# fedemagnani/optimization-solvers

Measured on AMD Instinct MI355X. Metric: BFGS iterations/sec on n-dim convex quadratic (f64) at 1/2/4/8 MI355X, higher is better.
Workload: dtype f64

## Files before the change

### include/qn_hip.h

```cpp
#ifndef QN_HIP_H
#define QN_HIP_H

#include <stddef.h>
#include <stdint.h>

#ifdef __cplusplus
extern "C" {
#endif

#define QN_ABI_VERSION 5

typedef enum {
    QN_OK = 0,
    QN_MAX_ITER_REACHED = 1,
    QN_OUT_OF_DOMAIN = 2,
    QN_ERROR_INPUT_PARAMS = 3,
    QN_ABNORMAL_TERMINATION = 4
} qn_status;

const char* qn_status_string(int status);
const char* qn_last_error_message(void);
int qn_abi_version(void);

typedef struct qn_context qn_context;
// ... 96 lines not shown

int qn_solver_create(qn_context* ctx, int method, double tol, const double* x0_host, size_t n, qn_solver** out);
void qn_solver_destroy(qn_solver* s);
int qn_solver_set_bounds(qn_solver* s, const double* lower_bound_host, const double* upper_bound_host);
int qn_solver_set_spg_lambdas(qn_solver* s, double lambda_min, double lambda_max);
int qn_solver_spg_lambda(qn_solver* s, double* out, int* is_some);
int qn_solver_newton_factorisations(qn_solver* s, size_t* out);
int qn_solver_set_lbfgs_memory(qn_solver* s, size_t m);
int qn_solver_lbfgs_state(qn_solver* s, size_t* m, size_t* stored, double* gamma, size_t* resets);
int qn_solver_set_inverse_p(qn_solver* s, const double* p_colmajor_host);
int qn_solver_get_inverse_p(qn_solver* s, double* out_colmajor_host);
int qn_solver_reset(qn_solver* s, const double* x0_host);

typedef void (*qn_callback_fn)(void* user, qn_solver* solver);

int qn_minimize(qn_solver* s, qn_linesearch* ls, const qn_oracle* oracle, size_t max_iter_solver,
                size_t max_iter_line_search, qn_callback_fn callback, void* callback_user);

int qn_compute_step_len(qn_context* ctx, qn_linesearch* ls, const double* x_k_host, double f_k, const double* g_k_host,
                        const double* direction_host, size_t n, const qn_oracle* oracle, size_t max_iter, double* step_out);

size_t qn_solver_n(const qn_solver* s);
size_t qn_solver_k(const qn_solver* s);
int qn_solver_set_k(qn_solver* s, size_t k);
double qn_solver_tol(const qn_solver* s);
int qn_solver_get_x(qn_solver* s, double* out_host);
int qn_solver_set_x(qn_solver* s, const double* x_host);
int qn_solver_s_norm(qn_solver* s, double* out, int* is_some);
int qn_solver_y_norm(qn_solver* s, double* out, int* is_some);
int qn_solver_next_iterate_too_close(qn_solver* s, int* out);
int qn_solver_gradient_next_iterate_too_close(qn_solver* s, int* out);
int qn_solver_decrement_squared(qn_solver* s, double* out, int* is_some);
int qn_solver_get_inv_hessian(qn_solver* s, double* out_colmajor_host, int all_ranks);
int qn_solver_set_inv_hessian(qn_solver* s, const double* h_colmajor_host);
int qn_solver_compute_direction(qn_solver* s, const double* g_host, double* d_host);
int qn_solver_secant_update(qn_solver* s, const double* s_host, const double* y_host);

#define QN_TRACE_LS_MODIFIED (1 << 30)
typedef struct {
    double f, gnorm, t, s_norm, y_norm;
    int32_t n_evals;
    int32_t ls_iters;
    int32_t ls_cases;
    int32_t updated;
} qn_trace_rec;
int qn_solver_set_trace(qn_solver* s, size_t cap, int with_x);
int qn_solver_get_trace(qn_solver* s, qn_trace_rec* out_host, size_t cap, size_t* len, double* x_trace_host);

typedef struct {
    uint64_t iterations;
    uint64_t oracle_calls;
    uint64_t oracle_evals;
    uint64_t h_passes;
    uint64_t h_bytes;
    uint64_t obj_bytes;
    uint64_t launches;
    uint64_t host_syncs;
    double   t_hpass_ms, t_eval_ms, t_ctl_ms, t_comm_ms;
    uint64_t n_hpass_timed, n_eval_timed, n_ctl_timed, n_comm_timed;
    uint64_t matrix_bytes_per_pass;
    uint64_t total_minimize_calls, total_iterations, total_oracle_calls, total_oracle_evals, total_h_passes, total_h_bytes,
        total_obj_bytes;
    uint32_t path;
    uint32_t _pad;
    double   t_hreduce_ms, t_ereduce_ms;
    uint64_t n_hreduce_timed, n_ereduce_timed;
    uint64_t total_xchg_vector, total_xchg_scalar;
    double   t_newton_ms;
    uint64_t n_newton_timed;
    uint64_t newton_lu_sync_timeouts;
} qn_stats;
#define QN_PATH_FUSED 1u
#define QN_PATH_SYM 2u
#define QN_PATH_SYM_GENERIC 4u
#define QN_PATH_PIPELINED 8u
#define QN_PATH_SYM2 16u
#define QN_PATH_TILES1 32u
#define QN_PATH_VECTOR 64u
#define QN_PATH_PNEWTON 128u
#define QN_PATH_RANK1 256u
#define QN_PATH_PNORM 512u
#define QN_PATH_LBFGS 1024u
int qn_solver_get_stats(qn_solver* s, qn_stats* out);
int qn_solver_set_profiling(qn_solver* s, int on);
int qn_solver_set_sync_mode(qn_solver* s, int sync);
int qn_solver_set_tiling(qn_solver* s, int rows_per_block, int col_splits);
typedef enum {
    QN_OPT_GENERIC_KERNELS = 1,
    QN_OPT_DEFERRED_UPDATE_STEP = 2,
    QN_OPT_SYMMETRIC_STORAGE = 3,
    QN_OPT_SECOND_GENERATION = 4,
    QN_OPT_FOLDED_ACCEPT_REDUCE = 5,
    QN_OPT_ROW_SLIVERS = 6,
    QN_OPT_EVAL_PAIR_INSTANCE = 7,
    QN_OPT_EVAL_MOVER_MULTIPLIER = 8,
    QN_OPT_TAIL_REDUCE = 9,
    QN_OPT_BOUNDED_SECOND_GENERATION = 10,
    QN_OPT_NEWTON_PIVOTED_LU = 11,
    QN_OPT_LU_PER_COLUMN_PANEL = 12,
    QN_OPT_LU_LOOKAHEAD = 13,
    QN_OPT_LU_ONE_LAUNCH_PANEL = 14,
    QN_OPT_LU_FORCE_WAIT_EXPIRY = 15,
    QN_OPT_CHUNKS_PER_TRIP = 16,
    QN_OPT_LU_SPLIT_ROLE_A = 17,
    QN_OPT_LU_SPLIT_MIN_ROWS = 18,
    QN_OPT_BTB_PROJECT_IN_EVAL = 19,
    QN_OPT_EVAL_ZIGZAG = 20,
    QN_OPT_TOUCH_H_ROWS = 21,
    QN_OPT_TOUCH_Q_ROWS = 22,
    QN_OPT_PNEWTON_REUSE_FACTOR = 23,
    QN_OPT_PNORM_NONTEMPORAL = 24,
    QN_OPT_PNORM_ROWS_PER_WAVE = 25,
    QN_OPT_LBFGS_UNIT_SCALING = 26
} qn_option;
int qn_solver_set_option(qn_solver* s, int option, int value);

int qn_dev_alloc(qn_context* ctx, size_t bytes, void** out_dev);
int qn_dev_free(qn_context* ctx, void* dev);
int qn_h2d(qn_context* ctx, void* dst_dev, const void* src_host, size_t bytes);
int qn_d2h(qn_context* ctx, void* dst_host, const void* src_dev, size_t bytes);
int qn_gemv(qn_context* ctx, const double* a_dev, size_t ld, size_t nrows, size_t ncols, const double* x_dev, double* y_dev);
int qn_rank2_update(qn_context* ctx, double* h_dev, size_t ld, size_t row0, size_t nrows, size_t n, const double* s_dev,
                    const double* u_dev, double c_ss, double c_su, double c_uu);
int qn_axpy(qn_context* ctx, size_t n, const double* x_dev, double t, const double* d_dev, double* out_dev);
int qn_dot(qn_context* ctx, size_t n, const double* a_dev, const double* b_dev, double* out_host);
int qn_nrm2(qn_context* ctx, size_t n, const double* a_dev, double* out_host);

#ifdef __cplusplus
}
#endif
#endif
```

### include/qn_solver.hpp

```cpp
#pragma once
#include <cmath>
#include <functional>
#include <optional>
#include <stdexcept>
#include <string>
#include <type_traits>
#include <utility>
#include <vector>

#include "qn_hip.h"

namespace optimization_solvers {

using Floating = double;
using DVector = std::vector<Floating>;

struct SolverError : std::runtime_error {
    enum Kind { MaxIterReached = QN_MAX_ITER_REACHED, OutOfDomain = QN_OUT_OF_DOMAIN, ErrorInputParams = QN_ERROR_INPUT_PARAMS,
                AbnormalTermination = QN_ABNORMAL_TERMINATION };
    Kind kind;
    explicit SolverError(int code, const std::string& detail = "")
        : std::runtime_error(std::string(qn_status_string(code)) + (detail.empty() ? "" : ": " + detail)), kind(static_cast<Kind>(code)) {}
};

// ... 142 lines not shown
    qn_linesearch s_;
    DVector lb_, ub_;
  public:
    BackTrackingB(Floating c1, Floating beta, DVector lower_bound, DVector upper_bound) : lb_(std::move(lower_bound)), ub_(std::move(upper_bound)) {
        qn_backtracking_b_new(&s_, c1, beta, lb_.data(), ub_.data());
    }
    BackTrackingB(const BackTrackingB&) = delete;
    qn_linesearch& ffi() { return s_; }
};

class Quadratic {
    qn_objective* h_ = nullptr;
    size_t n_;
  public:
    Quadratic(const DVector& q_rowmajor, const DVector& b, Context& ctx = Context::default_context()) : n_(b.size()) {
        check(qn_quadratic_create(ctx.handle(), n_, q_rowmajor.data(), b.data(), &h_));
    }
    Quadratic(const Quadratic&) = delete;
    ~Quadratic() { qn_objective_destroy(h_); }
    qn_objective* handle() const { return h_; }
    FuncEvalMultivariate operator()(const DVector& x) const {
        DVector g(n_);
        Floating f = 0;
        check(qn_objective_eval(h_, x.data(), &f, g.data()));
        return FuncEvalMultivariate(f, std::move(g));
    }
    DVector hessian(const DVector& x) const {
        DVector h(n_ * n_);
        check(qn_objective_hessian(h_, x.data(), h.data()));
        return h;
    }
};

class LogSumExp {
    qn_objective* h_ = nullptr;
    size_t n_;
  public:
    LogSumExp(const DVector& a_rowmajor, const DVector& c, size_t n, Floating mu, Context& ctx = Context::default_context()) : n_(n) {
        check(qn_logsumexp_create(ctx.handle(), c.size(), n, a_rowmajor.data(), c.data(), mu, &h_));
    }
    LogSumExp(const LogSumExp&) = delete;
    ~LogSumExp() { qn_objective_destroy(h_); }
    qn_objective* handle() const { return h_; }
    FuncEvalMultivariate operator()(const DVector& x) const {
        DVector g(n_);
        Floating f = 0;
        check(qn_objective_eval(h_, x.data(), &f, g.data()));
        return FuncEvalMultivariate(f, std::move(g));
    }
    DVector hessian(const DVector& x) const {
        DVector h(n_ * n_);
        check(qn_objective_hessian(h_, x.data(), h.data()));
        return h;
    }
};

template <int METHOD>
class LineSearchSolver {
    qn_solver* h_ = nullptr;
    size_t n_;
    mutable DVector x_cache_;
    mutable size_t k_cache_ = 0;
    mutable std::optional<Floating> opt_cache_[2];
  public:
    using Self = LineSearchSolver<METHOD>;
    LineSearchSolver(Floating tol, const DVector& x0, Context& ctx = Context::default_context()) : n_(x0.size()) {
        check(qn_solver_create(ctx.handle(), METHOD, tol, x0.data(), x0.size(), &h_));
    }
    qn_solver* handle() const { return h_; }
    static Self new_(Floating tol, const DVector& x0) { return Self(tol, x0); }
    LineSearchSolver(const Self&) = delete;
    LineSearchSolver(Self&& o) noexcept : h_(o.h_), n_(o.n_) { o.h_ = nullptr; }
    ~LineSearchSolver() { if (h_) qn_solver_destroy(h_); }

    const DVector& x() const { x_cache_.resize(n_); check(qn_solver_get_x(h_, x_cache_.data())); return x_cache_; }
    const DVector& xk() const { return x(); }
    const size_t& k() const { k_cache_ = qn_solver_k(h_); return k_cache_; }
    Floating tol() const { return qn_solver_tol(h_); }
    std::optional<Floating> s_norm() const { Floating v; int some; check(qn_solver_s_norm(h_, &v, &some)); return some ? std::optional<Floating>(v) : std::nullopt; }
    std::optional<Floating> y_norm() const { Floating v; int some; check(qn_solver_y_norm(h_, &v, &some)); return some ? std::optional<Floating>(v) : std::nullopt; }
    bool next_iterate_too_close() const { int v; check(qn_solver_next_iterate_too_close(h_, &v)); return v != 0; }
    bool gradient_next_iterate_too_close() const { int v; check(qn_solver_gradient_next_iterate_too_close(h_, &v)); return v != 0; }
    DVector approx_inv_hessian() const { DVector m(n_ * n_); check(qn_solver_get_inv_hessian(h_, m.data(), 1)); return m; }
    std::optional<Floating> decrement_squared() const { Floating v; int some; check(qn_solver_decrement_squared(h_, &v, &some)); return some ? std::optional<Floating>(v) : std::nullopt; }
    bool has_converged(const FuncEvalMultivariate& eval) const {
        if (METHOD == QN_NEWTON) {
            const std::optional<Floating> d = decrement_squared();
            return d ? *d * 0.5 < tol() : false;
        }
        if (METHOD == QN_GRADIENT_DESCENT || METHOD == QN_COORDINATE_DESCENT || METHOD == QN_PNORM_DESCENT) {
            Floating acc = -INFINITY;
            for (Floating v : eval.g()) acc = std::fmax(std::fabs(v), acc);
            return acc < tol();
        }
        if (next_iterate_too_close() || gradient_next_iterate_too_close()) return true;
        Floating s = 0;
        for (Floating v : eval.g()) s += v * v;
        return std::sqrt(s) < tol();
    }

    template <class LS, class Oracle, class = std::enable_if_t<!std::is_same_v<std::decay_t<Oracle>, Quadratic> && !std::is_same_v<std::decay_t<Oracle>, LogSumExp>>>
    Result minimize(LS& line_search, Oracle&& oracle, size_t max_iter_solver, size_t max_iter_line_search,
                    std::optional<std::function<void(const Self&)>> callback = std::nullopt) {
        using OracleT = std::remove_reference_t<Oracle>;
        struct Ctx { OracleT* o; size_t n; } octx{&oracle, n_};
        auto tramp = [](void* user, const double* x, size_t n, double* f, double* g) -> int {
            Ctx* c = static_cast<Ctx*>(user);
            DVector xv(x, x + n);
            FuncEvalMultivariate ev = (*c->o)(xv);
            *f = ev.f();
            for (size_t i = 0; i < n; ++i) g[i] = ev.g()[i];
            return 0;
        };
        struct Cb { Self* me; std::function<void(const Self&)>* f; } cb{this, callback ? &*callback : nullptr};
        auto cb_tramp = [](void* user, qn_solver*) { Cb* c = static_cast<Cb*>(user); (*c->f)(*c->me); };
        auto htramp = [](void* user, const double* x, size_t n, double* h) -> int {
            Ctx* c = static_cast<Ctx*>(user);
            DVector xv(x, x + n);
            FuncEvalMultivariate ev = (*c->o)(xv);
            if (!ev.hessian() || ev.hessian()->size() != n * n) return 1;
            for (size_t i = 0; i < n * n; ++i) h[i] = (*ev.hessian())[i];
            return 0;
        };
        qn_oracle o{};
        o.kind = QN_ORACLE_HOST;
        o.memoize = 0;
        o.host_fn = tramp;
        o.host_user = &octx;
        if (METHOD == QN_NEWTON || METHOD == QN_PROJECTED_NEWTON || METHOD == QN_SPECTRAL_PROJECTED_NEWTON) o.host_hessian_fn = htramp;
        const int st = qn_minimize(h_, &line_search.ffi(), &o, max_iter_solver, max_iter_line_search,
                                   callback ? static_cast<qn_callback_fn>(cb_tramp) : nullptr, &cb);
        return make_result(st);
    }

    template <class LS>
    Result minimize(LS& line_search, const Quadratic& objective, size_t max_iter_solver, size_t max_iter_line_search) {
        qn_oracle o{};
        o.kind = QN_ORACLE_OBJECTIVE;
        o.memoize = 1;
        o.objective = objective.handle();
        return make_result(qn_minimize(h_, &line_search.ffi(), &o, max_iter_solver, max_iter_line_search, nullptr, nullptr));
    }
    template <class LS>
    Result minimize(LS& line_search, const LogSumExp& objective, size_t max_iter_solver, size_t max_iter_line_search) {
        qn_oracle o{};
        o.kind = QN_ORACLE_OBJECTIVE;
        o.memoize = 1;
        o.objective = objective.handle();
        return make_result(qn_minimize(h_, &line_search.ffi(), &o, max_iter_solver, max_iter_line_search, nullptr, nullptr));
    }
};

using BFGS = LineSearchSolver<QN_BFGS>;
using DFP = LineSearchSolver<QN_DFP>;
using GradientDescent = LineSearchSolver<QN_GRADIENT_DESCENT>;
using Broyden = LineSearchSolver<QN_BROYDEN>;
using Newton = LineSearchSolver<QN_NEWTON>;

using CoordinateDescent = LineSearchSolver<QN_COORDINATE_DESCENT>;

class PnormDescent : public LineSearchSolver<QN_PNORM_DESCENT> {
  public:
    PnormDescent(Floating grad_tol, const DVector& x0, const DVector& inverse_p_colmajor, Context& ctx = Context::default_context())
        : LineSearchSolver<QN_PNORM_DESCENT>(grad_tol, x0, ctx) {
        if (inverse_p_colmajor.size() != x0.size() * x0.size()) throw SolverError(QN_ERROR_INPUT_PARAMS);
        check(qn_solver_set_inverse_p(this->handle(), inverse_p_colmajor.data()));
// ... 133 lines not shown
```

### optimization-solvers_amd/_abi.py

```python
import ctypes as C
import os

_HERE = os.path.dirname(os.path.abspath(__file__))
LIB_PATH = os.environ.get("QN_HIP_LIB") or os.path.join(_HERE, "lib", "libqn_hip.so")

OK, MAX_ITER_REACHED, OUT_OF_DOMAIN, ERROR_INPUT_PARAMS, ABNORMAL_TERMINATION = range(5)
LS_MORETHUENTE, LS_BACKTRACKING, LS_MORETHUENTE_B, LS_BACKTRACKING_B, LS_GLL_QUADRATIC = 0, 1, 2, 3, 4
LS_NO_SEARCH = 5
LS_STRONG_WOLFE = 6
ORACLE_HOST, ORACLE_DEVICE_FN, ORACLE_OBJECTIVE = 0, 1, 2
BFGS, DFP, GRADIENT_DESCENT, NEWTON, SR1, SPG, PROJECTED_GRADIENT, PROJECTED_NEWTON, SPECTRAL_PROJECTED_NEWTON = 0, 1, 2, 3, 4, 5, 6, 7, 8
BROYDEN = 9
COORDINATE_DESCENT, PNORM_DESCENT = 10, 11
LBFGS = 12
LBFGS_MAX_M = 32
UNIQUE_ID_BYTES = 128

dp = C.POINTER(C.c_double)


class LineSearchStruct(C.Structure):
    _fields_ = [("kind", C.c_int32), ("_pad", C.c_int32),
                ("c1", C.c_double), ("c2", C.c_double), ("t_min", C.c_double), ("t_max", C.c_double),
                ("delta_min", C.c_double), ("delta", C.c_double), ("delta_max", C.c_double),
# ... 38 lines not shown
PATH_FUSED, PATH_SYM, PATH_SYM_GENERIC, PATH_PIPELINED, PATH_SYM2, PATH_TILES1, PATH_VECTOR, PATH_PNEWTON = 1, 2, 4, 8, 16, 32, 64, 128
PATH_RANK1 = 256
PATH_PNORM = 512
PATH_LBFGS = 1024


SYMBOLS = [
    ("qn_status_string", C.c_char_p, [C.c_int]),
    ("qn_last_error_message", C.c_char_p, []),
    ("qn_abi_version", C.c_int, []),
    ("qn_device_count", C.c_int, [C.POINTER(C.c_int)]),
    ("qn_context_create", C.c_int, [C.c_int, C.POINTER(C.c_void_p)]),
    ("qn_comm_unique_id", C.c_int, [C.c_void_p]),
    ("qn_context_create_sharded", C.c_int, [C.c_int, C.c_int, C.c_int, C.c_void_p, C.POINTER(C.c_void_p)]),
    ("qn_context_create_sharded_host_exchange", C.c_int, [C.c_int, C.c_int, C.c_int, C.c_void_p, C.c_void_p, C.POINTER(C.c_void_p)]),
    ("qn_context_destroy", None, [C.c_void_p]),
    ("qn_partition", C.c_int, [C.c_size_t, C.c_int, C.POINTER(C.c_size_t), C.POINTER(C.c_size_t)]),
    ("qn_comm_selftest", C.c_int, [C.c_void_p]),
    ("qn_context_comm_check", C.c_int, [C.c_void_p]),
    ("qn_context_exchange_probe", C.c_int, [C.c_void_p, C.c_size_t, C.c_int, C.POINTER(C.c_double)]),
    ("qn_context_event_bracket_overhead", C.c_int, [C.c_void_p, C.c_int, C.POINTER(C.c_double)]),
    ("qn_context_synchronize", C.c_int, [C.c_void_p]),
    ("qn_context_rank", C.c_int, [C.c_void_p]),
    ("qn_context_world", C.c_int, [C.c_void_p]),
    ("qn_context_stream", C.c_void_p, [C.c_void_p]),
    ("qn_context_set_host_exchange_async", C.c_int, [C.c_void_p, C.c_int]),
    ("qn_context_set_trial_vector_exchange", C.c_int, [C.c_void_p, C.c_int]),
    ("qn_context_set_allreduce", C.c_int, [C.c_void_p, C.c_int]),
    ("qn_morethuente_default", None, [C.POINTER(LineSearchStruct)]),
    ("qn_morethuente_with_deltas", C.c_int, [C.POINTER(LineSearchStruct), C.c_double, C.c_double, C.c_double]),
    ("qn_morethuente_with_t_min", C.c_int, [C.POINTER(LineSearchStruct), C.c_double]),
    ("qn_morethuente_with_t_max", C.c_int, [C.POINTER(LineSearchStruct), C.c_double]),
    ("qn_morethuente_with_c1", C.c_int, [C.POINTER(LineSearchStruct), C.c_double]),
    ("qn_morethuente_with_c2", C.c_int, [C.POINTER(LineSearchStruct), C.c_double]),
    ("qn_backtracking_new", None, [C.POINTER(LineSearchStruct), C.c_double, C.c_double]),
    ("qn_morethuente_b_new", None, [C.POINTER(LineSearchStruct)]),
    ("qn_backtracking_b_new", None, [C.POINTER(LineSearchStruct), C.c_double, C.c_double, C.c_void_p, C.c_void_p]),
    ("qn_linesearch_with_lower_bound", None, [C.POINTER(LineSearchStruct), C.c_void_p]),
    ("qn_linesearch_with_upper_bound", None, [C.POINTER(LineSearchStruct), C.c_void_p]),
    ("qn_nosearch_new", None, [C.POINTER(LineSearchStruct)]),
    ("qn_gll_quadratic_new", None, [C.POINTER(LineSearchStruct), C.c_double, C.c_size_t]),
    ("qn_gll_quadratic_with_sigmas", None, [C.POINTER(LineSearchStruct), C.c_double, C.c_double]),
    ("qn_strong_wolfe_new", None, [C.POINTER(LineSearchStruct), C.c_double, C.c_double]),
    ("qn_strong_wolfe_with_xtol", C.c_int, [C.POINTER(LineSearchStruct), C.c_double]),
    ("qn_quadratic_create", C.c_int, [C.c_void_p, C.c_size_t, dp, dp, C.POINTER(C.c_void_p)]),
    ("qn_quadratic_create_synthetic", C.c_int, [C.c_void_p, C.c_size_t, C.c_uint64, dp, dp, C.POINTER(C.c_void_p)]),
    ("qn_logsumexp_create", C.c_int, [C.c_void_p, C.c_size_t, C.c_size_t, dp, dp, C.c_double, C.POINTER(C.c_void_p)]),
    ("qn_objective_destroy", None, [C.c_void_p]),
    ("qn_objective_eval", C.c_int, [C.c_void_p, dp, dp, dp]),
    ("qn_objective_get_rows", C.c_int, [C.c_void_p, C.c_size_t, C.c_size_t, dp]),
    ("qn_objective_hessian", C.c_int, [C.c_void_p, dp, dp]),
    ("qn_solver_create", C.c_int, [C.c_void_p, C.c_int, C.c_double, dp, C.c_size_t, C.POINTER(C.c_void_p)]),
    ("qn_solver_destroy", None, [C.c_void_p]),
    ("qn_solver_reset", C.c_int, [C.c_void_p, dp]),
    ("qn_solver_set_bounds", C.c_int, [C.c_void_p, dp, dp]),
    ("qn_solver_set_inverse_p", C.c_int, [C.c_void_p, dp]),
    ("qn_solver_get_inverse_p", C.c_int, [C.c_void_p, dp]),
    ("qn_solver_set_spg_lambdas", C.c_int, [C.c_void_p, C.c_double, C.c_double]),
    ("qn_solver_spg_lambda", C.c_int, [C.c_void_p, dp, C.POINTER(C.c_int)]),
    ("qn_solver_newton_factorisations", C.c_int, [C.c_void_p, C.POINTER(C.c_size_t)]),
    ("qn_solver_set_lbfgs_memory", C.c_int, [C.c_void_p, C.c_size_t]),
    ("qn_solver_lbfgs_state", C.c_int, [C.c_void_p, C.POINTER(C.c_size_t), C.POINTER(C.c_size_t), dp, C.POINTER(C.c_size_t)]),
    ("qn_minimize", C.c_int, [C.c_void_p, C.POINTER(LineSearchStruct), C.POINTER(OracleStruct), C.c_size_t, C.c_size_t, C.c_void_p, C.c_void_p]),
    ("qn_compute_step_len", C.c_int, [C.c_void_p, C.POINTER(LineSearchStruct), dp, C.c_double, dp, dp, C.c_size_t, C.POINTER(OracleStruct), C.c_size_t,
                             C.POINTER(C.c_double)]),
    ("qn_solver_n", C.c_size_t, [C.c_void_p]),
    ("qn_solver_k", C.c_size_t, [C.c_void_p]),
    ("qn_solver_set_k", C.c_int, [C.c_void_p, C.c_size_t]),
    ("qn_solver_tol", C.c_double, [C.c_void_p]),
    ("qn_solver_get_x", C.c_int, [C.c_void_p, dp]),
    ("qn_solver_set_x", C.c_int, [C.c_void_p, dp]),
    ("qn_solver_s_norm", C.c_int, [C.c_void_p, dp, C.POINTER(C.c_int)]),
    ("qn_solver_y_norm", C.c_int, [C.c_void_p, dp, C.POINTER(C.c_int)]),
    ("qn_solver_next_iterate_too_close", C.c_int, [C.c_void_p, C.POINTER(C.c_int)]),
    ("qn_solver_gradient_next_iterate_too_close", C.c_int, [C.c_void_p, C.POINTER(C.c_int)]),
    ("qn_solver_decrement_squared", C.c_int, [C.c_void_p, dp, C.POINTER(C.c_int)]),
    ("qn_solver_get_inv_hessian", C.c_int, [C.c_void_p, dp, C.c_int]),
    ("qn_solver_set_inv_hessian", C.c_int, [C.c_void_p, dp]),
    ("qn_solver_compute_direction", C.c_int, [C.c_void_p, dp, dp]),
    ("qn_solver_secant_update", C.c_int, [C.c_void_p, dp, dp]),
    ("qn_solver_set_trace", C.c_int, [C.c_void_p, C.c_size_t, C.c_int]),
    ("qn_solver_get_trace", C.c_int, [C.c_void_p, C.POINTER(TraceRec), C.c_size_t, C.POINTER(C.c_size_t), dp]),
    ("qn_solver_get_stats", C.c_int, [C.c_void_p, C.POINTER(Stats)]),
    ("qn_solver_set_profiling", C.c_int, [C.c_void_p, C.c_int]),
    ("qn_solver_set_sync_mode", C.c_int, [C.c_void_p, C.c_int]),
    ("qn_solver_set_tiling", C.c_int, [C.c_void_p, C.c_int, C.c_int]),
    ("qn_solver_set_option", C.c_int, [C.c_void_p, C.c_int, C.c_int]),
    ("qn_dev_alloc", C.c_int, [C.c_void_p, C.c_size_t, C.POINTER(C.c_void_p)]),
    ("qn_dev_free", C.c_int, [C.c_void_p, C.c_void_p]),
    ("qn_h2d", C.c_int, [C.c_void_p, C.c_void_p, C.c_void_p, C.c_size_t]),
    ("qn_d2h", C.c_int, [C.c_void_p, C.c_void_p, C.c_void_p, C.c_size_t]),
    ("qn_gemv", C.c_int, [C.c_void_p, C.c_void_p, C.c_size_t, C.c_size_t, C.c_size_t, C.c_void_p, C.c_void_p]),
    ("qn_rank2_update", C.c_int, [C.c_void_p, C.c_void_p, C.c_size_t, C.c_size_t, C.c_size_t, C.c_size_t, C.c_void_p, C.c_void_p,
                                  C.c_double, C.c_double, C.c_double]),
    ("qn_axpy", C.c_int, [C.c_void_p, C.c_size_t, C.c_void_p, C.c_double, C.c_void_p, C.c_void_p]),
    ("qn_dot", C.c_int, [C.c_void_p, C.c_size_t, C.c_void_p, C.c_void_p, dp]),
    ("qn_nrm2", C.c_int, [C.c_void_p, C.c_size_t, C.c_void_p, dp]),
]

_lib = None


def lib():
    global _lib
    if _lib is not None:
        return _lib
    if not os.path.exists(LIB_PATH):
        raise RuntimeError(
            f"{LIB_PATH} not found: build it first (python -c 'import __graft_entry__ as g; g.build()'). "
            "There is no CPU fallback for this path.")
    L = C.CDLL(LIB_PATH)
    for name, res, args in SYMBOLS:
        fn = getattr(L, name)
        fn.restype = res
        fn.argtypes = args
    _lib = L
    return L
```

### optimization-solvers_amd/csrc/qn_ctl.h

```cpp
#pragma once
#include <stdint.h>

enum QnPhase : int32_t {
    QN_PH_IDLE = 0,
    QN_PH_REQ_EVAL = 1,
    QN_PH_REQ_HPASS = 2,
    QN_PH_ITER_DONE = 3,
    QN_PH_DONE = 4,
    QN_PH_REQ_HPASS_EVAL = 7,
    QN_PH_REQ_VEC = 8,
    QN_PH_REQ_NEWTON = 6,
    QN_PH_REQ_DIR = 9,
    QN_PH_REQ_STEEP = 10
};

enum QnReqKind : int32_t { QN_REQ_X = 0 , QN_REQ_T = 1  };

enum QnState : int32_t {
    QN_ST_BEGIN = 0,
    QN_ST_LOOP_TOP,
    QN_ST_AFTER_EVALX,
    QN_ST_CHECK,
    QN_ST_AFTER_DIR,
    QN_ST_LS_BEGIN,
// ... 13 lines not shown
    QN_ST_AFTER_STEEP
};

#define QN_METHOD_BROYDEN 9
#define QN_METHOD_CD 10
#define QN_METHOD_PNORM 11
#define QN_LS_KIND_NOSEARCH 5
#define QN_LS_MODIFIED_BIT (1 << 30)

struct QnTraceRec {
    double f, gnorm, t, s_norm, y_norm;
    int32_t n_evals, ls_iters, ls_cases, updated;
};

struct QnCtl {
    double tol;
    int64_t max_iter, max_iter_ls;
    int32_t method, ls_kind, memoize, callback_mode;
    double mt_c1, mt_c2, mt_tmin, mt_tmax, mt_delta;
    double bt_c1, bt_beta;
    int64_t trace_cap;
    int32_t trace_x;
    int32_t small_n;

    int32_t phase, state, status, after_state;
    int64_t k;
    int32_t has_s_norm, has_y_norm;
    double s_norm, y_norm;
    double f_k;
    double gd0;
    double gnorm;
    double gg;
    int32_t gg_valid, xtrace_done;
    int32_t have_cur_eval;
    int32_t have_dir;

    int32_t fused, xc, sc, dir_mode, gd0_valid;
    int32_t no_defer;
    int32_t warm;
    int32_t defer_u;
    int32_t sym2;
    int32_t serviced;
    int32_t ev_par;
    int32_t ev_kind;
    double ev_t;
    double dir_ug, dir_sg;
    double st_gd0, st_yy, st_ys, st_gg, st_ss, st_dnf;
    double hp_yu, hp_ug, hp_sg;
    double hp_den;

    int32_t bounded, req_project, last_projected;
    int32_t ls_only;
    double mtb_cand;
    double bt_diff2;

    int32_t has_dec;
    int32_t s2_dir;
    double dec;

    int32_t req_kind, req_need_vectors;
    double req_t;
    int32_t hp_nrhs, hp_lazy;

    int32_t pending;
    int32_t spec_tiles;
    double c_ss, c_su, c_uu;

    double f_e, gd_e;
    int32_t last_valid, d_finite;
    double last_t, f_last, gd_last;

    int64_t ls_i;
    double t, tl, tu, ls_result;
    int32_t use_mod, conv;
    double phi_t_f, phi_t_g, psi_t_f, psi_t_g;
    double sel_f_tl, sel_g_tl, sel_f_t, sel_g_t;
    double ys;

    double tr_f, tr_gnorm;
    int32_t tr_n_evals, tr_ls_iters, tr_ls_cases, tr_ndigits, tr_updated;
    int32_t dir_ready;

    uint64_t n_oracle_calls, n_oracle_evals, n_hpasses, n_hpass_rw, n_iterations;
};
```

### optimization-solvers_amd/csrc/qn_ctl_step.hip.h

```cpp
#pragma once

#ifdef QN_CTL_STAMPS
#define QN_STAMP(id) do { if (tid == 0 && V.dbg) V.dbg[stamp_base + (id)] = wall_clock64(); } while (0)
#else
#define QN_STAMP(id) do { } while (0)
#endif

#define QN_TILE_IDX(base)                                        \
    int idx[4];                                                  \
    bool ok[4];                                                  \
    _Pragma("unroll") for (int u_ = 0; u_ < 4; ++u_) {           \
        const int i_ = (base) + u_ * tpb + tid;                  \
        ok[u_] = i_ < n_pad;                                     \
        idx[u_] = ok[u_] ? i_ : 0;                               \
    }

template <int NP>
__device__ __forceinline__ void ctl_sum_partials(const double* __restrict__ part, int world, int nblk, double* lds, int wave0 = 0) {
    const int lane = threadIdx.x & 63, wave = (int)(threadIdx.x >> 6) - wave0, nw = (int)(blockDim.x >> 6) - wave0;
    if (wave < 0) return;
    for (int k = wave; k < NP; k += nw) {
        const double acc = qn_partial_col_sum(part, world, nblk, NP, k, lane);
        if (lane == 0) lds[k] = acc;
    }
}

__device__ __forceinline__ void qn_keepalive(double v) { asm volatile("" ::"v"(v)); }

__device__ __forceinline__ bool qn_check_is_scalar(const QnCtl& c) {
    return c.method != 2 && c.method != QN_METHOD_CD && c.method != QN_METHOD_PNORM && (c.small_n || c.gg_valid || c.method == 3);
}


template <int LEAN>
__device__ __forceinline__ void qn_st_begin(QnCtl& c) {
    c.k = 0;
    if (!c.warm) { c.have_cur_eval = 0; c.have_dir = 0; c.last_valid = 0; c.gg_valid = 0; }
    else c.last_valid = 0;
    c.n_oracle_calls = 0; c.n_oracle_evals = 0; c.n_hpasses = 0; c.n_hpass_rw = 0; c.n_iterations = 0;
    c.status = -1;
    c.state = QN_ST_LOOP_TOP;
}

template <int LEAN>
__device__ __forceinline__ void qn_st_loop_top(QnCtl& c) {
    if (!(c.max_iter > c.k)) {
        c.status = 1;
        c.phase = QN_PH_DONE;
    } else {
        c.tr_n_evals = 0; c.tr_ls_iters = 0; c.tr_ls_cases = 0; c.tr_ndigits = 0; c.tr_updated = 0;
        c.ls_result = NAN;
        c.n_oracle_calls++;
        c.tr_n_evals++;
        if (c.memoize && c.have_cur_eval) {
            c.state = QN_ST_CHECK;
        } else {
            c.req_kind = QN_REQ_X; c.req_t = 0.0; c.req_need_vectors = 1;
            c.after_state = QN_ST_AFTER_EVALX;
            c.phase = QN_PH_REQ_EVAL;
        }
    }
}

template <int LEAN>
__device__ __forceinline__ bool qn_st_after_evalx(QnCtl& c) {
    if (!LEAN && !c.fused) return false;
    c.f_k = c.f_e;
    c.gg = c.st_gg; c.gg_valid = 1;
    c.have_cur_eval = c.memoize;
    c.have_dir = 0;
    c.state = QN_ST_CHECK;
    return true;
}

template <int LEAN>
__device__ __forceinline__ bool qn_st_after_dir(QnCtl& c) {
    if (!LEAN && !c.fused) return false;
    c.n_hpasses++;
    if (c.pending) c.n_hpass_rw++;
    c.pending = 0;
    c.dir_mode = 0;
    c.gd0_valid = 0; c.d_finite = 0; c.last_valid = 0;
    c.state = QN_ST_LS_BEGIN;
    if (LEAN == 2 && c.s2_dir) { c.dir_ready = 0; c.after_state = QN_ST_LS_BEGIN; c.phase = QN_PH_REQ_DIR; }
    return true;
}

template <int LEAN>
__device__ __forceinline__ bool qn_st_after_next(QnCtl& c) {
    if (!LEAN && !c.fused) return false;
    c.s_norm = sqrt(c.st_ss); c.has_s_norm = 1;
    c.y_norm = sqrt(c.st_yy); c.has_y_norm = 1;
    c.ys = c.st_ys;
    c.gg = c.st_gg; c.gg_valid = 1;
    c.f_k = c.f_e;
    c.xc ^= 1;
    c.have_cur_eval = c.memoize;
    c.have_dir = 0;
    c.last_valid = 0;
    if (c.s_norm < c.tol || c.y_norm < c.tol) {
        c.state = QN_ST_ITER_END;
    } else {
        c.hp_lazy = 1; c.hp_nrhs = 2;
        const double fk = c.f_k;
        const bool will_continue = (c.k + 1 < c.max_iter) && !(isnan(fk) || isinf(fk)) && !(sqrt(c.gg) < c.tol);
        if (!LEAN && will_continue && !c.callback_mode && !c.no_defer && !c.sym2) {
            c.defer_u = 1;
            c.tr_updated = 1;
            c.have_dir = 1; c.gd0_valid = 0; c.d_finite = 0;
            c.state = QN_ST_ITER_END;
        } else {
            c.after_state = QN_ST_AFTER_U;
            c.phase = QN_PH_REQ_HPASS;
        }
    }
    return true;
}

template <int LEAN>
__device__ __forceinline__ bool qn_st_after_u(QnCtl& c) {
    if (!LEAN && !c.fused) return false;
    const double yu = c.hp_yu;
    double c_ss, c_su, c_uu;
    qn_update_coeffs(c.method, c.ys, yu, c_ss, c_su, c_uu, c.hp_den);
    c.c_ss = c_ss; c.c_su = c_su; c.c_uu = c_uu;
    c.n_hpasses++;
    if (c.pending) c.n_hpass_rw++;
    c.pending = 1;
    c.sc ^= 1;
    c.dir_mode = 1; c.dir_ug = c.hp_ug; c.dir_sg = c.hp_sg;
    c.gd0_valid = 0; c.d_finite = 0;
    c.have_dir = 1;
    if (LEAN == 2) c.dir_ready = 0;
    c.tr_updated = 1;
    c.state = QN_ST_ITER_END;
    return true;
}

template <int LEAN>
__device__ __forceinline__ bool qn_st_check(QnCtl& c, const QnVecs& V, double* small_scratch) {
    const int n = V.n, n_pad = V.n_pad;
    if (!LEAN && !qn_check_is_scalar(c)) return false;
    if (!LEAN && c.method == 3) {
        c.gnorm = c.gg_valid ? sqrt(c.gg) : NAN; c.tr_f = c.f_k; c.tr_gnorm = c.gnorm;
        const double f = c.f_k;
        if (isnan(f) || isinf(f)) { c.status = 2; c.phase = QN_PH_DONE; }
        else if (c.has_dec && c.dec * 0.5 < c.tol) { c.status = 0; c.phase = QN_PH_DONE; }
        else { c.after_state = QN_ST_AFTER_NEWTON; c.phase = QN_PH_REQ_NEWTON; }
        return true;
    }
    double gnorm, gd0 = c.gd0;
    int d_finite = c.d_finite;
    if (!LEAN && c.small_n) {
        gnorm = sqrt(ref_dot(V.g, V.g, n));
        small_direction(V.H, n_pad, n, V.g, V.d, small_scratch, V.x, c.bounded ? V.lb : nullptr, c.bounded ? V.ub : nullptr);
        if (c.ls_kind == 2) {
            double cand = INFINITY;
            for (int i = 0; i < n; ++i) {
                const double di = V.d[i];
                double v = INFINITY;
                if (di > 0.0) v = (V.lub[i] - V.x[i]) / di; else if (di < 0.0) v = (V.llb[i] - V.x[i]) / di;
                cand = fmin(v, cand);
            }
            c.mtb_cand = cand;
        }
        gd0 = ref_dot(V.g, V.d, n);
        d_finite = 1;
        for (int i = 0; i < n; ++i) d_finite &= isfinite(V.d[i]) ? 1 : 0;
    } else {
        gnorm = sqrt(c.gg);
    }
    c.gnorm = gnorm; c.tr_f = c.f_k; c.tr_gnorm = gnorm;
    const double f = c.f_k;
    if (isnan(f) || isinf(f)) {
        c.status = 2; c.phase = QN_PH_DONE;
    } else if ((c.has_s_norm && c.s_norm < c.tol) || (c.has_y_norm && c.y_norm < c.tol) || (gnorm < c.tol)) {
        c.status = 0; c.phase = QN_PH_DONE;
    } else if (!LEAN && c.small_n) {
        c.gd0 = gd0; c.d_finite = d_finite; c.last_valid = 0;
        c.state = QN_ST_LS_BEGIN;
    } else if (c.have_dir) {
        c.state = QN_ST_LS_BEGIN;
        if (LEAN == 2 && c.s2_dir) {
            if (!c.dir_ready) { c.after_state = QN_ST_LS_BEGIN; c.phase = QN_PH_REQ_DIR; }
            else if (c.s2_dir & 2) c.mt_tmax = fmin(c.mt_tmax, c.mtb_cand);
        }
    } else {
        c.hp_nrhs = 1; c.hp_lazy = 0;
        c.after_state = QN_ST_AFTER_DIR;
        c.phase = QN_PH_REQ_HPASS;
    }
    return true;
}

template <int LEAN>
__device__ __forceinline__ void qn_st_ls_begin(QnCtl& c) {
    c.ls_i = 0;
    if (!LEAN && c.ls_kind == QN_LS_KIND_NOSEARCH) { c.ls_result = 1.0; c.state = QN_ST_AFTER_LS; return; }
    if (!LEAN && c.ls_kind == 2) c.mt_tmax = fmin(c.mt_tmax, c.mtb_cand);
    if (c.ls_kind == 0 || (!LEAN && c.ls_kind == 2)) {
        c.use_mod = 0; c.conv = 0;
        c.t = fmin(fmax(1.0, c.mt_tmin), c.mt_tmax);
        c.tl = c.mt_tmin; c.tu = c.mt_tmax;
        c.state = QN_ST_MT_LOOP;
    } else {
        c.t = 1.0;
        c.state = QN_ST_BT_LOOP;
    }
}

// ... 758 lines not shown
```

### optimization-solvers_amd/csrc/qn_host_launch.hip.h

```cpp
#pragma once
struct Run;
static int r1_enqueue_req(qn_solver* s);
static int steep_enqueue_req(qn_solver* s);
static int enqueue_newton(qn_solver* s, const qn_oracle* o, qn_objective* obj);

static int check_oracle(qn_context* c, size_t n, const qn_oracle* o, qn_objective** obj) {
    *obj = nullptr;
    if (o->kind == QN_ORACLE_HOST) return o->host_fn ? QN_OK : fail(QN_ERROR_INPUT_PARAMS, "host oracle is null");
    if (o->kind == QN_ORACLE_DEVICE_FN) return o->device_fn ? QN_OK : fail(QN_ERROR_INPUT_PARAMS, "device oracle is null");
    if (o->kind != QN_ORACLE_OBJECTIVE) return fail(QN_ERROR_INPUT_PARAMS, "unknown oracle kind");
    if (!o->objective) return fail(QN_ERROR_INPUT_PARAMS, "objective is null");
    if (o->objective->ctx != c || o->objective->n != n) return fail(QN_ERROR_INPUT_PARAMS, "objective does not match the solver");
    *obj = o->objective;
    return QN_OK;
}
static void stats_add_totals(qn_solver* s) {
    s->stats.total_minimize_calls++;
    s->stats.total_iterations += s->stats.iterations; s->stats.total_oracle_calls += s->stats.oracle_calls; s->stats.total_oracle_evals += s->stats.oracle_evals;
    s->stats.total_h_passes += s->stats.h_passes; s->stats.total_h_bytes += s->stats.h_bytes; s->stats.total_obj_bytes += s->stats.obj_bytes;
}
static int xchg_sum_or_gather(qn_context* c, double* buf, size_t cnt) { return c->use_allreduce ? exchange_sum(c, buf, cnt) : exchange(c, buf, cnt); }

struct Run {
    qn_solver* s;
// ... 256 lines not shown
                a.parity = (int)(r.s2_launches & 1);
                hipLaunchKernelGGL(s2sh_vsumt_kernel, dim3(a.nb), dim3(QN_S2_TPB), 0, c->stream, a);
                HIPCHK(hipGetLastError());
                s->stats.launches++;
            }
            ProfScope ps(s, KC_COMM);
            const XchgItem items[2] = {{half, cnt}, {s->symsh_xg, (size_t)s->T.n_pad}};
            c->n_xchg_scalar++;
            QNCHK(exchange_group(c, items, 2));
            return QN_OK;
        }
        ProfScope ps(s, KC_COMM);
        c->n_xchg_scalar++;
        QNCHK(xchg_sum_or_gather(c, half, cnt));
    }
    return QN_OK;
}
static int s2_do_vec(Run& r) {
    qn_solver* s = r.s;
    qn_context* c = s->ctx;
    if (r.s2.sh_world > 1 && c->trial_vector && !r.gobj) return s2_launch(r, QN_S2_VECD);
    if (r.s2.sh_world > 1) {
        QNCHK(s2_launch(r, QN_S2_VSUM));
        {
            ProfScope ps(s, KC_COMM);
            c->n_xchg_vector++;
            if (r.gobj) QNCHK(exchange(c, r.obj->lgall, (size_t)s->T.n_pad));
            else QNCHK(xchg_sum_or_gather(c, s->symsh_xg, (size_t)s->T.n_pad));
        }
        return s2_launch(r, QN_S2_VEC);
    }
    return s2_launch(r, r.s2.fold ? QN_S2_HTILE : QN_S2_VEC);
}
static int s2_do_hpass(Run& r, bool tiles) {
    qn_solver* s = r.s;
    qn_context* c = s->ctx;
    if (r.gobj && r.s2.sh_world == 1) {
        if (!tiles) return fail(QN_ABNORMAL_TERMINATION, "sym2 (generic objective): tiles marked done without their launch");
        QNCHK(s2_launch(r, QN_S2_GHT_A));
        QNCHK(s2g_enqueue_tiles(r));
        return s2_launch(r, QN_S2_HREDUCE);
    }
    if (tiles && r.tiles1) {
        QNCHK(s2_launch(r, QN_S2_GHT_A));
        QNCHK(s2g_enqueue_tiles(r));
    } else if (tiles) QNCHK(s2_launch(r, QN_S2_HTILE));
    if (r.s2.tred) return QN_OK;
    if (r.s2.sh_world > 1) {
        QNCHK(s2_launch(r, QN_S2_HSUM));
        ProfScope ps(s, KC_COMM);
        c->n_xchg_vector++;
        QNCHK(xchg_sum_or_gather(c, s->symsh_xg, 2 * (size_t)s->T.n_pad));
    }
    return s2_launch(r, QN_S2_HREDUCE);
}

static int s2_wait_report(Run& r, unsigned long long seq) {
    qn_solver* s = r.s;
    volatile unsigned long long* flag = s->hrep_flag;
    for (uint64_t spins = 0;; ++spins) {
        if (__atomic_load_n(flag, __ATOMIC_ACQUIRE) == seq) break;
        if ((spins & 0xfff) == 0xfff) {
            hipError_t e = hipStreamQuery(s->ctx->stream);
            if (e == hipSuccess) { if (__atomic_load_n(flag, __ATOMIC_ACQUIRE) == seq) break; return fail(QN_ABNORMAL_TERMINATION, "sym2: the batch ended without a report"); }
            if (e != hipErrorNotReady) return fail(QN_ABNORMAL_TERMINATION, std::string("sym2 batch: ") + hipGetErrorString(e));
        }
    }
    memcpy(s->hctl, s->hrep, sizeof(QnCtl));
    s->stats.host_syncs++;
    return QN_OK;
}

static int place_h(Run& r) {
    qn_solver* s = r.s;
    if (s->h_placed) return QN_OK;
    s->h_placed = true;
    const size_t np = s->T.n_pad, bytes = (size_t)s->T.rpr * np * sizeof(double);
    const char* sw = getenv("QN_H_PLACEMENT");
    if ((sw && atoi(sw) == 0) || s->ctx->world != 1 || bytes > ((size_t)330 << 20) || r.s2.fold) return QN_OK;
    hipStream_t st = s->ctx->stream;
    QnCtl* pc = s->hrep;
    memcpy(pc, s->hctl, sizeof(QnCtl));
    pc->phase = QN_PH_REQ_HPASS; pc->serviced = 0; pc->hp_nrhs = 1; pc->pending = 0; pc->after_state = QN_ST_AFTER_DIR; pc->sym2 = 1; pc->fused = 1;
    pc->spec_tiles = 0; pc->sc = 0; pc->xc = 0;
    PinnedBuf<QnCtl> pe;
    (void)pe.alloc(1, hipHostMallocMapped | hipHostMallocCoherent);
    if (pe) {
        memcpy(pe, s->hctl, sizeof(QnCtl));
        pe->phase = QN_PH_REQ_EVAL; pe->serviced = 0; pe->sym2 = 1; pe->fused = 1; pe->sc = 0; pe->xc = 0;
        pe->ev_kind = QN_REQ_T; pe->t = 1.0; pe->status = -1;
    }
    ScopedEvent e0, e1;
    if (hipEventCreate(&e0.e) != hipSuccess || hipEventCreate(&e1.e) != hipSuccess) { (void)hipGetLastError(); return QN_OK; }
    auto time_on = [&](double* H, float* out_us) -> int {
        QnS2Args a = r.s2;
        a.H = H; a.parity = 0; a.ctl_first = pc; a.rep_seq = 0;
        a.tred = 0;
        float t[6];
        for (int rep = 0; rep < 6; ++rep) {
            if (pe) {
                QnS2Args ae = a;
                ae.ctl_first = pe;
                for (int e = 0; e < 2; ++e) s2_launch_eval_plain(st, ae);
            }
            HIPCHK(hipEventRecord(e0.e, st));
            if (s->method == QN_BFGS) hipLaunchKernelGGL((s2_hpass_kernel<false, true, false>), dim3(a.G), dim3(QN_S2_TPB), 0, st, a);
            else hipLaunchKernelGGL((s2_hpass_kernel<false, false, false>), dim3(a.G), dim3(QN_S2_TPB), 0, st, a);
            HIPCHK(hipEventRecord(e1.e, st));
            HIPCHK(hipEventSynchronize(e1.e));
            float ms = 0.f;
            HIPCHK(hipEventElapsedTime(&ms, e0.e, e1.e));
            t[rep] = ms * 1e3f;
        }
        std::sort(t + 2, t + 6);
        *out_us = t[3];
        return QN_OK;
    };
    DevBuf<double> cand[2];
    struct Drain { hipStream_t st; ~Drain() { (void)hipStreamSynchronize(st); } } drained{st};
    float us[3] = {0.f, 0.f, 0.f};
    int ncand = 1, keep = 0;
    QNCHK(time_on(s->H, &us[0]));
    for (int k = 1; k < 3; ++k) {
        if (k == 2 && std::fabs(us[0] - us[1]) <= 0.06f * std::min(us[0], us[1])) break;
        if (cand[k - 1].alloc((size_t)s->T.rpr * np) != QN_OK) break;
        ++ncand;
        if (hipMemcpyAsync(cand[k - 1], s->H, bytes, hipMemcpyDeviceToDevice, st) != hipSuccess) return fail(QN_ABNORMAL_TERMINATION, "H placement: copy failed");
        QNCHK(time_on(cand[k - 1], &us[k]));
    }
    for (int k = 1; k < ncand; ++k)
        if (us[k] < 0.96f * us[keep]) keep = k;
    if (sw && atoi(sw) == 2) fprintf(stderr, "[qn] H placement: %d candidates, update kernel %.2f %.2f %.2f us, kept %d\n", ncand, us[0], us[1], us[2], keep);
    if (keep) {
        (void)hipStreamSynchronize(st);
        s->H = std::move(cand[keep - 1]);
        s->V.H = s->H;
        r.s2.H = s->H;
    }
    return QN_OK;
}

static int launch_ctl_mask(Run& r, int expect_mask) {
    qn_solver* s = r.s;
    ProfScope ps(s, KC_CTL);
    const bool hp = (expect_mask & ((1 << QN_PH_REQ_HPASS) | (1 << QN_PH_REQ_HPASS_EVAL))) != 0;
    const bool ev = (expect_mask & ((1 << QN_PH_REQ_EVAL) | (1 << QN_PH_REQ_HPASS_EVAL))) != 0;
    const dim3 blk(r.fused ? ((hp && ev) ? 768 : 576) : QN_CTL_TPB);
    QnVecs V = s->V;
    if (r.rank1) V.hcs = 1;
    if (r.oracle_tpl == QN_ORACLE_QUAD)
        hipLaunchKernelGGL(ctl_step_kernel<QN_ORACLE_QUAD>, dim3(1), blk, 0, s->ctx->stream, s->ctl, V, expect_mask);
    else
        hipLaunchKernelGGL(ctl_step_kernel<QN_ORACLE_GENERIC>, dim3(1), blk, 0, s->ctx->stream, s->ctl, V, expect_mask);
    s->stats.launches++;
    HIPCHK(hipGetLastError());
    return QN_OK;
}
static int launch_ctl(Run& r, int expect_phase) { return launch_ctl_mask(r, 1 << expect_phase); }

template <int R, int U>
static void launch_eval_fused(hipStream_t st, const QnEvalFusedArgs& a) {
    hipLaunchKernelGGL((quad_eval_fused_kernel<R, U>), dim3(a.T.rpr / R), dim3(QN_TPB), 0, st, a);
}
template <int R, int U>
static void launch_hpass_fused(hipStream_t st, const QnHPassFusedArgs& a) {
    hipLaunchKernelGGL((h_pass_fused_kernel<R, U>), dim3(a.T.rpr / R), dim3(QN_TPB), 0, st, a);
}
// ... 195 lines not shown
```

### optimization-solvers_amd/csrc/qn_host_minimize.hip.h

```cpp
#pragma once
static int vec_minimize(qn_solver* s, qn_linesearch* ls, const qn_oracle* o, size_t max_iter_solver, size_t max_iter_line_search,
                        qn_callback_fn callback, void* callback_user, int ls_only, double ls_f0);
static int vec_compute_step_len(qn_context* ctx, qn_linesearch* ls, const double* x_k_host, double f_k, const double* g_k_host,
                                const double* direction_host, size_t n, const qn_oracle* oracle, size_t max_iter, double* step_out);

static int plan_run(Run& r, qn_solver* s, qn_linesearch* ls, const qn_oracle* o, size_t max_iter_solver, size_t max_iter_line_search, double ls_f0) {
    qn_context* c = s->ctx;
    const qn_callback_fn callback = r.callback;
    const int ls_only = r.ls_only;
    if (ls->kind < QN_LS_MORETHUENTE || (ls->kind > QN_LS_BACKTRACKING_B && ls->kind != QN_LS_NO_SEARCH)) return fail(QN_ERROR_INPUT_PARAMS, "unknown line search");
    if (ls->kind == QN_LS_NO_SEARCH && s->method != QN_GRADIENT_DESCENT && s->method != QN_NEWTON && !steep_method(s->method))
        return fail(QN_ERROR_INPUT_PARAMS, "NoSearch pairs with GradientDescent, Newton, CoordinateDescent and PnormDescent only");
    if (s->method == QN_PNORM_DESCENT && !s->pnorm_set) return fail(QN_ERROR_INPUT_PARAMS, "PnormDescent: inverse_p has not been set (qn_solver_set_inverse_p)");
    if (steep_method(s->method)) QNCHK(steep_alloc(s));
    const bool ls_bounded = r.ls_bounded = ls->kind == QN_LS_MORETHUENTE_B || ls->kind == QN_LS_BACKTRACKING_B;
    if (ls_bounded || s->bounded) {
        QNCHK(bounds_alloc(s));
        if (ls_bounded) {
            QNCHK(bounds_upload(s, s->bounds_block + 2 * (size_t)s->T.n_pad, ls->lower_bound_host, -INFINITY));
            QNCHK(bounds_upload(s, s->bounds_block + 3 * (size_t)s->T.n_pad, ls->upper_bound_host, INFINITY));
        }
    }
    {
        std::vector<double> box;
        if (ls_bounded) {
            box.assign(2 * s->n, 0.0);
            for (size_t i = 0; i < s->n; ++i) { box[i] = ls->lower_bound_host ? ls->lower_bound_host[i] : -INFINITY; box[s->n + i] = ls->upper_bound_host ? ls->upper_bound_host[i] : INFINITY; }
        }
        s->ls_box_changed = ls->kind != s->last_ls_kind || box.size() != s->last_ls_box.size() ||
                            (!box.empty() && memcmp(box.data(), s->last_ls_box.data(), box.size() * sizeof(double)) != 0);
        s->last_ls_kind = ls->kind;
        s->last_ls_box.swap(box);
    }
    if (s->method == QN_NEWTON) {
        if (c->world > 1) return fail(QN_ERROR_INPUT_PARAMS, "Newton is single-GPU (SURVEY.md 8(f) row f2)");
        if (!(r.obj && (r.obj->kind == OBJ_QUADRATIC || r.obj->kind == OBJ_LOGSUMEXP)) && !(o->kind == QN_ORACLE_HOST && o->host_hessian_fn))
            return fail(QN_ERROR_INPUT_PARAMS, "Hessian not available in the oracle");
        QNCHK(newton_alloc(s));
    }

    QnCtl* h = s->hctl;
    h->tol = s->tol;
    h->max_iter = (int64_t)std::min<size_t>(max_iter_solver, (size_t)1 << 62);
    h->max_iter_ls = (int64_t)std::min<size_t>(max_iter_line_search, (size_t)1 << 62);
    h->method = s->method;
    h->ls_kind = ls->kind;
    h->memoize = o->memoize ? 1 : 0;
    h->callback_mode = callback ? 1 : 0;
    h->mt_c1 = ls->c1; h->mt_c2 = ls->c2; h->mt_tmin = ls->t_min; h->mt_tmax = ls->t_max; h->mt_delta = ls->delta;
    h->bt_c1 = ls->bt_c1; h->bt_beta = ls->bt_beta;
    h->trace_cap = (int64_t)s->trace_cap;
    h->trace_x = s->trace_x;
    h->bounded = s->bounded;
    h->req_project = 0; h->last_projected = 0; s->mtb_cand_keep = h->mtb_cand; h->mtb_cand = INFINITY;
    h->ls_only = ls_only;
    if (ls_only) { h->f_k = ls_f0; h->have_cur_eval = 0; h->have_dir = 0; h->last_valid = 0; }
    h->small_n = (s->n <= QN_SMALL_N && c->world == 1) ? 1 : 0;
    if (h->small_n && h->pending) QNCHK(flush_pending(s));
    const bool sym_base = s->T.n_pad >= 8 * QN_TB && !s->no_sym && !s->h_nonsym;
    const bool sym_ok = c->world == 1 && (s->T.n_pad % QN_TB) == 0 && sym_base;
    const bool symsh_ok = c->world > 1 && (s->T.rpr % QN_TB) == 0 && sym_base;
    const bool s2_shape = sym_ok && (size_t)s->T.n_pad == s->n && !s->no_sym2;
    const bool s2sh_shape = symsh_ok && (size_t)s->T.n_pad == s->n && !s->no_sym2 && c->world <= 64;
    const bool s2bnd_off = getenv("QN_S2_BND") && atoi(getenv("QN_S2_BND")) == 0;
    const bool s2_struct = !ls_only && s2_shape && r.obj && r.obj->q_symmetric && !s->no_s2bnd && !s2bnd_off;
    const bool s2b = (s->bounded || ls_bounded) && s2_struct;
    const bool sr1_s2 = s->method == QN_SR1 && s2_struct;
    r.fused = r.oracle_tpl == QN_ORACLE_QUAD && h->memoize && (s->method == QN_BFGS || s->method == QN_DFP || sr1_s2) && !callback && s->hcs == 1 &&
              s->qcs == 1 && !h->small_n && !s->no_fused && (!(s->bounded || ls_bounded) || s2b);
    r.gobj = r.obj && r.obj->kind == OBJ_LOGSUMEXP && r.obj->lse_kch && !r.obj->lse_two_pass && h->memoize && (s->method == QN_BFGS || s->method == QN_DFP) &&
             !callback && s->hcs == 1 && !h->small_n && !s->no_fused && !s->bounded && !ls_bounded && !ls_only &&
             (s2_shape || (s2sh_shape && (c->comm || c->host_xchg || c->host_async))) && !(getenv("QN_S2G") && atoi(getenv("QN_S2G")) == 0);
    if (r.gobj) r.fused = true;
    h->fused = r.fused ? 1 : 0;
    s->V.fused_hint = h->fused;
    r.sym = r.fused && (sym_ok || symsh_ok) && r.obj && (r.obj->q_symmetric || r.gobj);
    r.sym_generic = !r.fused && (sym_ok || symsh_ok) && s->H && s->hcs == 1 && (s->method == QN_BFGS || s->method == QN_DFP || s->method == QN_SR1);
    r.rank1 = s->method == QN_BROYDEN && !h->small_n;
    r.pnorm = s->method == QN_PNORM_DESCENT && !h->small_n;
    if (s->method == QN_BROYDEN && (r.fused || r.sym || r.sym_generic)) return fail(QN_ABNORMAL_TERMINATION, "Broyden on a symmetric-storage path");
    if ((r.sym || r.sym_generic) && c->world > 1) QNCHK(solver_alloc_symsh_lists(s));
    if (r.sym_generic) {
        if (c->world > 1) QNCHK(s->symsh_xg.ensure((size_t)c->world * 2 * s->T.n_pad, c->stream));
        const int nb = s->T.n_pad / QN_TB;
        QNCHK(s->sym_part.ensure((size_t)nb * nb * 2 * QN_TB, c->stream));
        s->sym_nb = nb;
    }
    r.sym2 = r.sym && (s2_shape || s2sh_shape);
    h->sym2 = r.sym2 ? 1 : 0;
    r.bnd = r.sym2 && (s->bounded || ls_bounded || s->method == QN_SR1);
    if ((s->bounded || ls_bounded) && r.fused && !r.bnd) return fail(QN_ABNORMAL_TERMINATION, "bounded run on a fused path that is not the second-generation one");
    if (s->method == QN_SR1 && r.fused && !r.sym2) return fail(QN_ABNORMAL_TERMINATION, "SR1 on a fused path that is not the second-generation one");
    h->s2_dir = r.bnd ? ((s->bounded ? 1 : 0) | (ls->kind == QN_LS_MORETHUENTE_B ? 2 : 0)) : 0;
    r.dirq = h->s2_dir != 0;
    r.btb = r.bnd && ls->kind == QN_LS_BACKTRACKING_B;
    r.proj = r.btb;
    if (r.bnd && ls->kind == QN_LS_MORETHUENTE_B) h->ls_kind = QN_LS_MORETHUENTE;
    {
        const size_t hhalf = c->world > 1 ? (size_t)s->T.rpr * s->T.n_pad * 8 / 2 : (size_t)s->T.n_pad * s->T.n_pad * 8 / 2;
        r.tiles1 = r.sym2 && !r.gobj && c->world > 1 && hhalf > ((size_t)320 << 20);
        if (r.sym2 && !r.gobj && getenv("QN_S2_GEN1_TILES")) r.tiles1 = atoi(getenv("QN_S2_GEN1_TILES")) != 0;
    }
    h->serviced = 0; h->ev_par = 0; h->ev_kind = QN_REQ_X; h->ev_t = 0.0; h->spec_tiles = 0;
    h->defer_u = 0;
    h->no_defer = s->no_defer;
    if (!r.fused) QNCHK(fused_export(s));
    if (!(r.sym || r.sym_generic) || (s->h_diag_stale && (!r.sym2 || (r.gobj && c->world == 1) || r.tiles1))) QNCHK(ensure_full_h(s));
    if (r.fused) {
        QNCHK(solver_alloc_fused(s, r.sym));
        s->V.F.pworld = r.sym ? 1 : c->world;
        if (r.sym && c->world > 1) QNCHK(s->symsh_xg.ensure((size_t)c->world * 2 * s->T.n_pad, c->stream));
        s->V.F.b = r.gobj ? nullptr : r.obj->b;
        if (!s->fused_live) {
            const size_t vb = (size_t)s->T.n_pad * sizeof(double);
            HIPCHK(hipMemcpyAsync(s->V.F.X0, s->V.x, vb, hipMemcpyDeviceToDevice, c->stream));
            if (h->pending) {
                HIPCHK(hipMemcpyAsync(s->V.F.S0, s->V.sp, vb, hipMemcpyDeviceToDevice, c->stream));
                HIPCHK(hipMemcpyAsync(s->V.F.UN, s->V.up, vb, hipMemcpyDeviceToDevice, c->stream));
            }
            h->xc = 0; h->sc = 0;
        }
        h->warm = (s->fused_live && s->warm_obj != 0 && s->warm_obj == r.obj->serial && h->memoize && h->pending && !ls_only) ? 1 : 0;
        if (!h->warm) { h->dir_mode = 0; h->gd0_valid = 0; h->dir_ready = 0; }
        if (!r.bnd || s->ls_box_changed) h->dir_ready = 0;
        if (r.bnd && h->dir_ready) h->mtb_cand = s->mtb_cand_keep;
    } else {
        h->warm = 0;
    }
    h->phase = QN_PH_IDLE;
    h->status = -1;
    const bool can_pipeline = (r.oracle_tpl == QN_ORACLE_QUAD || r.gobj) && !callback && !(c->world > 1 && !c->comm && !c->host_async);
    r.sync = s->method == QN_NEWTON || s->method == QN_BROYDEN || steep_method(s->method) || s->sync_mode == 1 || (s->sync_mode == -1 && !(can_pipeline && o->memoize)) || !can_pipeline;
    return QN_OK;
}

static void s2_cache_policy(size_t half, int* nt, int* ntq) {
    if (2 * half <= ((size_t)230 << 20)) { *nt = 0; *ntq = 0; }
    else if (half <= ((size_t)320 << 20)) { *nt = 0; *ntq = 1; }
    else { *nt = 1; *ntq = 1; }
}

static int plan_s2_args(Run& r) {
    qn_solver* s = r.s;
    qn_context* c = s->ctx;
    QNCHK(solver_alloc_sym2(s));
    QnS2Args& a = r.s2;
    a.Q = r.obj->Q; a.H = s->H; a.n = (int)s->n; a.np = s->T.n_pad; a.nb = s->s2_nb; a.G = s->s2_G;
    a.item_ij = s->s2_items; a.maxk = s->s2_maxk; a.inorder = s->s2_inorder; a.F = s->V.F; a.part = s->sym_part;
    a.wgS = s->s2_wgS; a.trows = s->s2_trows; a.ctl2 = s->s2_ctl; a.partE = s->s2_partE;
    a.gw = r.gobj ? s->T.n_pad / 64 : 0;
    a.gmu = r.gobj ? r.obj->mu : 0.0;
    if (r.gobj && c->world > 1) QNCHK(s->s2_gws.ensure(80, c->stream));
    a.gws = s->s2_gws;
    if (r.gobj) QNCHK(s->s2_wgV.ensure((size_t)2 * s->s2_trows * QN_S2_ROW, c->stream));
    a.wgV = s->s2_wgV;
    if (r.gobj && a.gw > s->s2_trows) return fail(QN_ABNORMAL_TERMINATION, "sym2 (generic objective): more combine workgroups than table rows");
    a.fold = (s->s2_maxk <= 3 && s->s2_nb <= 32 && s->fold) ? 1 : 0;
    a.sl_first = s->s2_sl_first; a.sl_per = s->s2_sl_per;
    a.pair = (a.sl_per != 0 && s->s2_maxk == 2 && s->s2_inorder == 2 * s->s2_G && !s->no_pair) ? 1 : 0;
    if (a.sl_per && !s->h_sliver_whole) { QNCHK(ensure_full_h(s)); s->h_sliver_whole = true; }
    a.trace = s->V.trace; a.xtrace = s->V.xtrace;
    a.sh_world = c->world; a.sh_rank = c->rank; a.sh_ioff = c->rank * (s->T.rpr / QN_TB);
    a.sh_nsum = c->use_allreduce ? 1 : c->world;
    a.evS = s->s2_evS; a.xg = s->symsh_xg; a.sl_off = s->s2_sl_off; a.sl_idx = s->s2_sl_idx;
    if (c->world > 1 || r.gobj) { a.fold = 0; a.pair = 0; }
    {
        a.ring = (a.pair && s->ring && s->s2_nb * (s->s2_nb - 1) / 2 >= s->s2_G) ? 1 : 0;
        a.zig = (a.ring && s->zig) ? 1 : 0;
    }
    a.projfold = (r.btb && a.pair && a.ring && !s->no_projfold) ? 1 : 0;
    if (a.projfold) r.proj = false;
    if (r.bnd) a.fold = 0;
    a.method = s->method;
    if (s->method == QN_SR1) a.fold = 0;
    a.lb = (r.bnd && s->bounded) ? s->V.lb : nullptr; a.ub = (r.bnd && s->bounded) ? s->V.ub : nullptr;
    a.llb = (r.bnd && r.ls_bounded) ? s->V.llb : nullptr; a.lub = (r.bnd && r.ls_bounded) ? s->V.lub : nullptr;
    if (r.tiles1) a.fold = 0;
    a.cnt = s->s2_cnt;
    a.cnt_stride = getenv("QN_S2_CNT_STRIDE") ? std::max(1, std::min(QN_S2_CNT_STRIDE, atoi(getenv("QN_S2_CNT_STRIDE")))) : QN_S2_CNT_STRIDE;
    const bool want_tred = getenv("QN_S2_TRED") ? atoi(getenv("QN_S2_TRED")) != 0 : s->tred;
    if (want_tred) QNCHK(s->s2_cnt.ensure((size_t)a.nb * QN_S2_CNT_STRIDE, c->stream));
    a.cnt = s->s2_cnt;
    a.tred = (c->world == 1 && !a.fold && !r.gobj && !r.tiles1 && s->s2_maxk <= QN_S2_TRED_MAXK && want_tred && s->method != QN_SR1) ? 1 : 0;
    {
        auto rows_ok = [](int v) { return v == 4 || v == 6 || v == 8 || v == 10 || v == 12 || v == 16; };
        const bool can = a.ring && !r.bnd && !a.fold && !a.tred && s->method != QN_SR1 && a.nb == 32 && a.G == 256;
        a.touch = (can && rows_ok(s->touch)) ? s->touch : 0;
        a.touchq = (can && rows_ok(s->touchq)) ? s->touchq : 0;
        a.touch_delay = std::max(0, std::min(512, s->touch_delay));
        a.touchq_delay = std::max(0, std::min(512, s->touchq_delay));
    }
    s2_cache_policy(c->world > 1 ? (size_t)s->T.rpr * s->T.n_pad * 8 / 2 : (size_t)s->T.n_pad * s->T.n_pad * 8 / 2, &a.nt, &a.ntq);
    if (getenv("QN_S2_NT")) a.nt = atoi(getenv("QN_S2_NT"));
    if (getenv("QN_S2_NTQ")) a.ntq = atoi(getenv("QN_S2_NTQ"));
    return QN_OK;
}

static int slots_needed(uint64_t evals, uint64_t iters, int cap) {
    return (int)std::min<uint64_t>((uint64_t)cap, std::max<uint64_t>(1, (evals + iters - 1) / iters));
}

static int pump_s2_sync(Run& r) {
    QnCtl* h = r.s->hctl;
    QNCHK(s2_launch(r, QN_S2_ADVANCE));
    for (;;) {
        QNCHK(s2_peek(r));
        const int ph = h->phase;
        if (ph == QN_PH_DONE) { r.status = h->status; return QN_OK; }
        const bool tiles_done = ph == QN_PH_REQ_HPASS && h->serviced == 1;
        if (h->serviced != 0 && !tiles_done) return fail(QN_ABNORMAL_TERMINATION, "sym2: request in an unexpected service state");
        if (ph == QN_PH_REQ_EVAL) QNCHK(s2_do_eval(r));
        else if (ph == QN_PH_REQ_VEC) QNCHK(s2_do_vec(r));
        else if (ph == QN_PH_REQ_DIR && r.bnd) QNCHK(s2_launch(r, QN_S2_DIR));
        else if (ph == QN_PH_REQ_HPASS) QNCHK(s2_do_hpass(r, !tiles_done));
        else return fail(QN_ABNORMAL_TERMINATION, "sym2: control block in an unexpected phase");
        QNCHK(s2_launch(r, QN_S2_ADVANCE));
    }
}

static int pump_s2_pipelined(Run& r) {
    qn_solver* s = r.s;
    qn_context* c = s->ctx;
    QnCtl* h = s->hctl;
    int slots = (r.ls->kind == QN_LS_MORETHUENTE) ? 2 : 4;
    const bool adaptive = r.s2.sh_world > 1 || r.gobj || r.bnd;
    if (adaptive) slots = s->s2_slots_hint ? s->s2_slots_hint : (r.gobj ? 1 : 2);
    bool first = true;
    uint64_t ev0 = 0, it0 = 0;
    unsigned long long seq = 0;
    for (;;) {
        if (!first) {
            QNCHK(s2_wait_report(r, seq));
            if (adaptive && h->n_iterations > it0) {
                uint64_t de = h->n_oracle_evals - ev0;
                if (it0 == 0 && !h->warm && de > 0) de -= 1;
                slots = slots_needed(de, h->n_iterations - it0, 4);
                s->s2_slots_hint = slots;
            }
            ev0 = h->n_oracle_evals; it0 = h->n_iterations;
            if (h->phase == QN_PH_DONE) { r.status = h->status; return QN_OK; }
        }
        int64_t remaining = h->max_iter - (first ? 0 : h->k);
        if (remaining < 1) remaining = 1;
        const int64_t periods = std::min<int64_t>(remaining + ((first && !h->warm) ? 1 : 0), 256);
        first = false;
        auto one_period = [&]() -> int {
            if (r.dirq) QNCHK(s2_launch(r, QN_S2_DIR));
            for (int e = 0; e < slots; ++e) QNCHK(s2_do_eval(r));
            if (r.btb) QNCHK(s2_launch(r, QN_S2_ADVANCE));
            if (!r.s2.fold && !(r.gobj && r.s2.sh_world == 1)) QNCHK(s2_do_vec(r));
            QNCHK(s2_do_hpass(r, true));
            return QN_OK;
        };
        int64_t p = 0;
        static const bool want_graph = getenv("QN_S2_GRAPH") && atoi(getenv("QN_S2_GRAPH")) != 0;
        if (want_graph && c->world == 1 && !r.gobj && !s->profiling && periods >= 3) {
            QNCHK(one_period()); ++p;
            const uint64_t l0 = r.s2_launches;
            if ((l0 & 1) != 0) { QNCHK(one_period()); ++p; }
            if (periods - p >= 2) {
                const uint64_t lbase = r.s2_launches, stat0 = s->stats.launches;
                const bool reuse = s->s2_graph_exec && memcmp(&s->s2_graph_args, &r.s2, sizeof(QnS2Args)) == 0 && s->s2_graph_slots == slots && s->s2_graph_bnd == (int)r.bnd;
                if (!reuse) {
                    if (s->s2_graph_exec) { (void)hipGraphExecDestroy(s->s2_graph_exec); s->s2_graph_exec = nullptr; }
                    hipGraph_t g = nullptr;
                    HIPCHK(hipStreamBeginCapture(c->stream, hipStreamCaptureModeThreadLocal));
                    int rc = one_period(); if (rc == QN_OK) rc = one_period();
                    const hipError_t e = hipStreamEndCapture(c->stream, &g);
                    if (rc != QN_OK) return rc;
                    HIPCHK(e);
                    HIPCHK(hipGraphInstantiate(&s->s2_graph_exec, g, nullptr, nullptr, 0));
                    (void)hipGraphDestroy(g);
                    s->s2_graph_args = r.s2; s->s2_graph_slots = slots; s->s2_graph_bnd = (int)r.bnd;
                    s->s2_graph_len = r.s2_launches - lbase; s->s2_graph_stat = s->stats.launches - stat0;
                    r.s2_launches = lbase; s->stats.launches = stat0;
                }
                if ((s->s2_graph_len & 1) == 0) {
// ... 14 lines not shown
static int pump_ctl_sync(Run& r) {
    qn_solver* s = r.s;
    QnCtl* h = s->hctl;
    QNCHK(launch_ctl(r, QN_PH_IDLE));
    for (;;) {
        QNCHK(peek_ctl(s));
        const int ph = h->phase;
        if (ph == QN_PH_DONE) { r.status = h->status; return QN_OK; }
        if (ph == QN_PH_REQ_EVAL) { QNCHK(enqueue_eval(r)); QNCHK(launch_ctl(r, QN_PH_REQ_EVAL)); }
        else if (ph == QN_PH_REQ_HPASS) { QNCHK(enqueue_hpass_req(r)); QNCHK(launch_ctl(r, QN_PH_REQ_HPASS)); }
        else if (ph == QN_PH_REQ_HPASS_EVAL) {
            QNCHK(enqueue_hpass_req(r)); QNCHK(enqueue_eval(r, 1)); QNCHK(launch_ctl(r, QN_PH_REQ_HPASS_EVAL));
        }
        else if (ph == QN_PH_REQ_NEWTON) { { ProfScope ps(s, KC_NEWTON); QNCHK(enqueue_newton(s, r.o, r.obj)); } QNCHK(launch_ctl(r, QN_PH_REQ_NEWTON)); }
        else if (ph == QN_PH_REQ_STEEP) { QNCHK(steep_enqueue_req(s)); QNCHK(launch_ctl(r, QN_PH_REQ_STEEP)); }
        else if (ph == QN_PH_ITER_DONE) { r.callback(r.callback_user, s); QNCHK(launch_ctl(r, QN_PH_ITER_DONE)); }
        else return fail(QN_ABNORMAL_TERMINATION, "control block in an unexpected phase");
    }
}

static int pump_ctl_pipelined(Run& r) {
    qn_solver* s = r.s;
    QnCtl* h = s->hctl;
    QNCHK(launch_ctl(r, QN_PH_IDLE));
    const int slots_max = (r.ls->kind == QN_LS_MORETHUENTE || r.ls->kind == QN_LS_MORETHUENTE_B) ? 2 : 4;
    int slots = slots_max;
    const bool adaptive = !r.fused;
    if (adaptive && s->gen_slots_hint) slots = std::min(slots_max, s->gen_slots_hint);
    uint64_t ev0 = 0, it0 = 0;
    bool first_batch = true;
    const int gd = s->method == QN_GRADIENT_DESCENT;
    for (;;) {
        QNCHK(peek_ctl(s));
        if (adaptive && !first_batch && h->n_iterations > it0) {
            uint64_t de = h->n_oracle_evals - ev0;
            if (it0 == 0 && de > 0) de -= 1;
            slots = slots_needed(de, h->n_iterations - it0, slots_max);
            s->gen_slots_hint = slots;
        }
        ev0 = h->n_oracle_evals; it0 = h->n_iterations;
        first_batch = false;
        if (h->phase == QN_PH_DONE) { r.status = h->status; return QN_OK; }
        int64_t remaining = h->max_iter - h->k;
        if (remaining < 1) remaining = 1;
        const int64_t periods = std::min<int64_t>(remaining, 256);
        const int first_mask = (1 << QN_PH_REQ_EVAL) | (1 << QN_PH_REQ_HPASS) | (1 << QN_PH_REQ_HPASS_EVAL);
        for (int64_t p = 0; p < periods; ++p) {
            if (r.fused) {
                QNCHK(enqueue_eval(r, 1)); QNCHK(launch_ctl_mask(r, first_mask));
                for (int e = 1; e < slots; ++e) { QNCHK(enqueue_eval(r, 0)); QNCHK(launch_ctl(r, QN_PH_REQ_EVAL)); }
                QNCHK(enqueue_hpass_req(r));
            } else {
                for (int e = 0; e < slots; ++e) { QNCHK(enqueue_eval(r)); QNCHK(launch_ctl(r, QN_PH_REQ_EVAL)); }
                if (!gd) { QNCHK(enqueue_hpass_req(r)); QNCHK(launch_ctl(r, QN_PH_REQ_HPASS)); }
            }
        }
    }
}

static void finish_stats(Run& r) {
    qn_solver* s = r.s;
    qn_context* c = s->ctx;
    QnCtl* h = s->hctl;
    if (r.fused) s->fused_live = true;
    s->warm_obj = (r.fused && r.status == QN_MAX_ITER_REACHED && h->memoize && h->have_cur_eval && h->have_dir) ? r.obj->serial : 0;
    if (r.ls->kind == QN_LS_MORETHUENTE_B) r.ls->t_max = h->mt_tmax;
    s->stats.iterations = h->n_iterations;
    s->stats.oracle_calls = h->n_oracle_calls;
    s->stats.oracle_evals = h->n_oracle_evals;
    s->stats.h_passes = h->n_hpasses;
    uint64_t shard = (uint64_t)s->T.rpr * (uint64_t)s->T.n_pad * 8ull;
    const uint64_t full_shard = shard;
    if (r.sym || r.sym_generic) shard = (uint64_t)s->sym_nb * (uint64_t)(s->sym_nb + 1) / 2ull * (uint64_t)QN_TB * QN_TB * 8ull;
    if ((r.sym || r.sym_generic) && c->world > 1) shard = (uint64_t)qn_symsh_ntiles(s->sym_nb, s->T.rpr / QN_TB, c->rank * (s->T.rpr / QN_TB)) * (uint64_t)QN_TB * QN_TB * 8ull;
    if (r.sym2 && !r.gobj && !r.tiles1)
        shard = (uint64_t)s->sym_nb * (uint64_t)(s->sym_nb - 1) / 2ull * (uint64_t)QN_TB * QN_TB * 8ull + (uint64_t)s->sym_nb * 73728ull;
    if (r.sym2 && c->world > 1 && !r.tiles1) {
        const uint64_t nbl = (uint64_t)(s->T.rpr / QN_TB);
        const uint64_t nt = (uint64_t)qn_symsh_ntiles(s->sym_nb, (int)nbl, c->rank * (int)nbl);
        shard = (nt - nbl) * (uint64_t)QN_TB * QN_TB * 8ull + nbl * 73728ull;
    }
    s->stats.h_bytes = (h->n_hpasses + h->n_hpass_rw) * shard;
    if (r.sym2) s->stats.h_bytes = 2 * h->n_hpasses * shard;
    s->stats.obj_bytes = (r.oracle_tpl == QN_ORACLE_QUAD) ? h->n_oracle_evals * (r.sym ? shard : full_shard) : 0;
    if (r.obj && r.obj->kind == OBJ_LOGSUMEXP)
        s->stats.obj_bytes = h->n_oracle_evals * (uint64_t)r.obj->TA.rpr * (uint64_t)r.obj->T.n_pad * 8ull * ((r.obj->lse_kch && !r.obj->lse_two_pass) ? 1ull : 2ull);
    s->stats.matrix_bytes_per_pass = shard;
    stats_add_totals(s);
    s->stats.total_xchg_vector += c->n_xchg_vector - r.xv0;
    s->stats.total_xchg_scalar += c->n_xchg_scalar - r.xs0;
    s->stats.path = (r.fused ? QN_PATH_FUSED : 0u) | (r.sym ? QN_PATH_SYM : 0u) | (r.sym_generic ? QN_PATH_SYM_GENERIC : 0u) |
                    (r.sync ? 0u : QN_PATH_PIPELINED) | (r.sym2 ? QN_PATH_SYM2 : 0u) | ((r.tiles1 || (r.gobj && c->world == 1)) ? QN_PATH_TILES1 : 0u) |
                    (r.rank1 ? QN_PATH_RANK1 : 0u) | (r.pnorm ? QN_PATH_PNORM : 0u);
}

static int minimize_impl(qn_solver* s, qn_linesearch* ls, const qn_oracle* o, size_t max_iter_solver, size_t max_iter_line_search,
                         qn_callback_fn callback, void* callback_user, int ls_only, double ls_f0) {
    if (!s || !ls || !o) return fail(QN_ERROR_INPUT_PARAMS, "null argument");
    if (vec_method(s->method)) return vec_minimize(s, ls, o, max_iter_solver, max_iter_line_search, callback, callback_user, ls_only, ls_f0);
    if (ls->kind == QN_LS_GLL_QUADRATIC) return fail(QN_ERROR_INPUT_PARAMS, "GLLQuadratic pairs with SPG / projected gradient only");
    qn_context* c = s->ctx;
    HIPCHK(hipSetDevice(c->device));
    Run r{s, o, nullptr, QN_ORACLE_GENERIC, false};
    r.ls = ls; r.callback = callback; r.callback_user = callback_user; r.ls_only = ls_only;
    r.xv0 = c->n_xchg_vector; r.xs0 = c->n_xchg_scalar;
    QNCHK(check_oracle(c, s->n, o, &r.obj));
    if (r.obj && r.obj->kind == OBJ_QUADRATIC) { r.oracle_tpl = QN_ORACLE_QUAD; s->V.b = r.obj->b; }
    else if (r.obj && r.obj->kind != OBJ_LOGSUMEXP) return fail(QN_ERROR_INPUT_PARAMS, "unsupported objective");
    QNCHK(plan_run(r, s, ls, o, max_iter_solver, max_iter_line_search, ls_f0));
    if (r.sym2) QNCHK(plan_s2_args(r));
    else QNCHK(poke_ctl(s));
    if (r.sym2 && !r.gobj) QNCHK(place_h(r));
    if (r.sym2) QNCHK(r.sync ? pump_s2_sync(r) : pump_s2_pipelined(r));
    else QNCHK(r.sync ? pump_ctl_sync(r) : pump_ctl_pipelined(r));
    finish_stats(r);
    if (c->host_async_failed) { c->host_async_failed = 0; return fail(QN_ABNORMAL_TERMINATION, "host exchange callback failed"); }
    if (r.status == QN_ABNORMAL_TERMINATION) return fail(r.status, "solver state machine aborted");
    return r.status;
}

extern "C" int qn_minimize(qn_solver* s, qn_linesearch* ls, const qn_oracle* o, size_t max_iter_solver,
                           size_t max_iter_line_search, qn_callback_fn callback, void* callback_user) {
    return minimize_impl(s, ls, o, max_iter_solver, max_iter_line_search, callback, callback_user, 0, 0.0);
}

extern "C" int qn_compute_step_len(qn_context* ctx, qn_linesearch* ls, const double* x_k_host, double f_k, const double* g_k_host,
                                   const double* direction_host, size_t n, const qn_oracle* oracle, size_t max_iter, double* step_out) {
    if (!ctx || !ls || !x_k_host || !g_k_host || !direction_host || !oracle || !step_out || n == 0)
        return fail(QN_ERROR_INPUT_PARAMS, "null argument");
    if (ls->kind == QN_LS_GLL_QUADRATIC) return vec_compute_step_len(ctx, ls, x_k_host, f_k, g_k_host, direction_host, n, oracle, max_iter, step_out);
    qn_solver* s = nullptr;
    QNCHK(qn_solver_create(ctx, QN_GRADIENT_DESCENT, 0.0, x_k_host, n, &s));
    int st = QN_OK;
    hipError_t e = hipMemcpyAsync(s->V.g, g_k_host, n * sizeof(double), hipMemcpyHostToDevice, ctx->stream);
    if (e == hipSuccess) e = hipMemcpyAsync(s->V.d, direction_host, n * sizeof(double), hipMemcpyHostToDevice, ctx->stream);
    if (e != hipSuccess) st = fail(QN_ABNORMAL_TERMINATION, std::string("compute_step_len upload: ") + hipGetErrorString(e));
    if (st == QN_OK) st = minimize_impl(s, ls, oracle, 1, max_iter, nullptr, nullptr, 1, f_k);
    if (st == QN_OK) *step_out = s->hctl->ls_result;
    qn_solver_destroy(s);
    return st;
}
```

### optimization-solvers_amd/csrc/qn_host_solver.hip.h

```cpp
#pragma once
enum { KC_HPASS = 0, KC_EVAL = 1, KC_CTL = 2, KC_COMM = 3, KC_HREDUCE = 4, KC_EREDUCE = 5, KC_NEWTON = 6 };
struct TimedEvent { hipEvent_t a, b; int cls; };
struct QnVecCtl;

struct qn_solver {
    qn_context* ctx = nullptr;
    int method = QN_BFGS;
    size_t n = 0;
    double tol = 0.0;
    QnTile T{};
    int R = 4, U = 1, hcs = 1, qcs = 1;
    DevBuf<double> H;
    DevBuf<double> vec_block;
    QnVecs V{};
    DevBuf<double> hp, q, xtrace; DevBuf<QnTraceRec> trace; DevBuf<unsigned long long> dbg;
    DevBuf<double> f_dev;
    DevBuf<double> newton_w, newton_x, newton_hsrc, newton_invl, newton_inv2;
    bool newton_big = false;
    DevBuf<double> sym_part;
    int sym_nb = 0;
    DevBuf<double> pnorm_P;
    bool pnorm_set = false;
    int pnorm_nt = -1, pnorm_rw = 0;
    DevBuf<double> steep_part;
    int steep_nshare = 0;
    DevBuf<double> r1_part;
    int r1_nb = 0;
    bool no_sym = false, h_nonsym = false;
    bool h_lower_stale = false;
    DevBuf<double> symsh_xg, symsh_gath;
    bool h_diag_stale = false;
    DevBuf<int> s2_items;
    int s2_G = 0, s2_nb = 0, s2_maxk = 0, s2_inorder = 0;
    int s2_sl_first = 0, s2_sl_per = 0, s2_sl_cfg = -1;
    bool no_sliver = false;
    bool no_pair = false;
    int ring = (getenv("QN_S2_RING") && atoi(getenv("QN_S2_RING")) == 0) ? 0 : 1;
    int zig = (getenv("QN_S2_ZIGZAG") && atoi(getenv("QN_S2_ZIGZAG")) == 0) ? 0 : 1;
    int touch = getenv("QN_S2_TOUCH") ? atoi(getenv("QN_S2_TOUCH")) : 8;
    int touchq = getenv("QN_S2_TOUCHQ") ? atoi(getenv("QN_S2_TOUCHQ")) : 6;
    int touch_delay = getenv("QN_S2_TOUCH_DELAY") ? atoi(getenv("QN_S2_TOUCH_DELAY")) : 32;
    int touchq_delay = getenv("QN_S2_TOUCHQ_DELAY") ? atoi(getenv("QN_S2_TOUCHQ_DELAY")) : 0;
    bool tred = false;
    DevBuf<int> s2_cnt;
    int gen_slots_hint = 0;
    DevBuf<double> s2_gws;
    DevBuf<double> s2_wgV;
    hipGraphExec_t s2_graph_exec = nullptr;
    QnS2Args s2_graph_args{}; int s2_graph_slots = 0, s2_graph_bnd = 0; uint64_t s2_graph_len = 0, s2_graph_stat = 0;
    int last_ls_kind = -1; std::vector<double> last_ls_box; bool ls_box_changed = false;
    double mtb_cand_keep = INFINITY;
    bool no_s2bnd = false;
    bool h_sliver_whole = false;
    DevBuf<double> s2_evS;
    DevBuf<int> s2_sl_off, s2_sl_idx;
    int s2_sl_nb = 0;
    bool h_placed = false;
    DevBuf<int> symsh_tiles;
    int s2_slots_hint = 0;
    DevBuf<double> s2_partE;
    DevBuf<double> s2_wgS;
    int s2_trows = 0;
    DevBuf<QnCtl> s2_ctl;
    bool no_sym2 = false;
    bool fold = false;
    bool fused_live = false;
    uint64_t warm_obj = 0;
    DevBuf<int> newton_fail;
    DevBuf<int> newton_piv, newton_perm;
    DevBuf<double> newton_panel;
    bool newton_lu_percol = false;
    std::vector<int> newton_piv_host;
    uint64_t newton_lu_runs = 0, newton_chol_runs = 0;
    int newton_lu_force_timeout = 0;
    int newton_lu_no_persist = 0;
    DevBuf<int> newton_sync;
    DevBuf<unsigned long long> newton_rec;
    bool no_projfold = getenv("QN_S2_PROJ_FOLD") && atoi(getenv("QN_S2_PROJ_FOLD")) == 0;
    int newton_lu_split = getenv("QN_LU_SPLIT") ? atoi(getenv("QN_LU_SPLIT")) : 4;
    int newton_lu_split_min = getenv("QN_LU_SPLIT_MIN") ? atoi(getenv("QN_LU_SPLIT_MIN")) : 4160;
    uint64_t newton_lu_sync_timeouts = 0;
    int newton_lu_timeout_fallback = 0;
    int newton_lu_no_la = 0;
    int newton_force_lu = 0;
    size_t newton_n64 = 0;
    std::vector<double> newton_hhost;
    DevBuf<QnVecCtl> vctl; PinnedBuf<QnVecCtl> hvctl;
    DevBuf<double> vpart;
    uint64_t pn_factor_serial = 0;
    int pn_reuse = 1;
    uint64_t pn_factorisations = 0;
    DevBuf<double> lb_ring, lb_part, lb_small;
    DevBuf<double> bounds_block;
    int bounded = 0;
    DevBuf<double> fused_block;
    DevBuf<double> fused_evp, fused_hpp;
    int fused_nblk = 0;
    DevBuf<QnCtl> ctl;
    PinnedBuf<unsigned char> hctl_block;
    QnCtl* hctl = nullptr;
    QnCtl* hrep = nullptr;
    unsigned long long* hrep_flag = nullptr;
    unsigned long long rep_seq = 0;
    PinnedBuf<double> hx, hg;
    size_t trace_cap = 0;
    int trace_x = 0;
    int sync_mode = -1;
    int no_fused = 0;
    int no_defer = 0;
    int profiling = 0;
    std::vector<TimedEvent> events;
    std::vector<hipEvent_t> event_pool;
    qn_stats stats{};
};

static hipEvent_t ev_get(qn_solver* s) {
    if (!s->event_pool.empty()) { hipEvent_t e = s->event_pool.back(); s->event_pool.pop_back(); return e; }
    hipEvent_t e = nullptr;
    (void)hipEventCreate(&e);
    return e;
}
struct ProfScope {
    qn_solver* s; int cls; hipEvent_t a = nullptr, b = nullptr;
    ProfScope(qn_solver* s_, int cls_) : s(s_), cls(cls_) {
        if (s->profiling && s->events.size() < 200000) { a = ev_get(s); b = ev_get(s); (void)hipEventRecord(a, s->ctx->stream); }
    }
    ~ProfScope() { if (a) { (void)hipEventRecord(b, s->ctx->stream); s->events.push_back({a, b, cls}); } }
};
static void prof_collect(qn_solver* s) {
    if (s->events.empty()) return;
    (void)hipStreamSynchronize(s->ctx->stream);
    std::vector<std::vector<float>> dur(8);
    std::vector<std::pair<int, float>> all;
    all.reserve(s->events.size());
    for (auto& e : s->events) {
        float ms = 0.f;
        const bool ok = hipEventElapsedTime(&ms, e.a, e.b) == hipSuccess;
        const int cls = (e.cls >= 0 && e.cls < 7) ? e.cls : 7;
        if (ok) { dur[cls].push_back(ms); all.push_back({e.cls, ms}); }
        s->event_pool.push_back(e.a);
        s->event_pool.push_back(e.b);
    }
    float floor_ms[8];
    for (int c = 0; c < 8; ++c) {
        floor_ms[c] = 0.f;
        if (dur[c].size() >= 8) {
            const size_t kth = dur[c].size() / 50;
            std::nth_element(dur[c].begin(), dur[c].begin() + kth, dur[c].end(), std::greater<float>());
            floor_ms[c] = 0.5f * dur[c][kth];
        }
    }
    for (auto& e : all) {
        const int cls = (e.first >= 0 && e.first < 7) ? e.first : 7;
        const float ms = e.second;
        if (ms < floor_ms[cls]) continue;
        switch (e.first) {
        case KC_HPASS: s->stats.t_hpass_ms += ms; s->stats.n_hpass_timed++; break;
        case KC_EVAL: s->stats.t_eval_ms += ms; s->stats.n_eval_timed++; break;
        case KC_CTL: s->stats.t_ctl_ms += ms; s->stats.n_ctl_timed++; break;
        case KC_HREDUCE: s->stats.t_hreduce_ms += ms; s->stats.n_hreduce_timed++; break;
        case KC_EREDUCE: s->stats.t_ereduce_ms += ms; s->stats.n_ereduce_timed++; break;
        case KC_NEWTON: s->stats.t_newton_ms += ms; s->stats.n_newton_timed++; break;
        default: s->stats.t_comm_ms += ms; s->stats.n_comm_timed++; break;
        }
    }
    s->events.clear();
}

static int solver_alloc_fused(qn_solver* s, bool sym) {
    const size_t np = s->T.n_pad;
    hipStream_t st = s->ctx->stream;
    QNCHK(s->fused_block.ensure(10 * np, st));
    const int nblk = sym ? (int)(np / QN_TB) : s->T.rpr / s->R;
    if (sym) {
        QNCHK(s->sym_part.ensure((size_t)nblk * nblk * 2 * QN_TB, st));
        s->sym_nb = nblk;
    }
    QNCHK(s->fused_evp.ensure((size_t)s->ctx->world * QN_NEVP * nblk, st));
    QNCHK(s->fused_hpp.ensure((size_t)s->ctx->world * QN_NHPP * nblk, st));
    s->fused_nblk = nblk;
    double* p = s->fused_block;
    QnFused& F = s->V.F;
    F.X0 = p; F.S0 = p + 2 * np; F.G = p + 4 * np; F.GT = p + 5 * np; F.Y = p + 6 * np;
    F.UN = p + 7 * np; F.UP = p + 8 * np; F.VV = p + 9 * np;
    F.evp = s->fused_evp; F.hpp = s->fused_hpp;
    F.nblk = nblk;
    return QN_OK;
}

static int solver_alloc_symsh_lists(qn_solver* s) {
    const int nb = s->T.n_pad / QN_TB;
    if (s->s2_sl_off && s->s2_sl_nb == nb) return QN_OK;
    const int nbl = s->T.rpr / QN_TB, ioff = s->ctx->rank * nbl;
    {
        std::vector<int> tiles;
        for (int il = 0; il < nbl; ++il)
            for (int k = 0, I = ioff + il; k < qn_symsh_cnt(I, nb); ++k) tiles.push_back((I << 16) | ((I + k) % nb));
        if (tiles.empty()) tiles.push_back(0);
        QNCHK(s->symsh_tiles.alloc(tiles.size()));
        HIPCHK(hipMemcpy(s->symsh_tiles, tiles.data(), tiles.size() * sizeof(int), hipMemcpyHostToDevice));
    }
    std::vector<int> off(nb + 1, 0), idx;
    for (int R = 0; R < nb; ++R) {
        const bool r_local = R >= ioff && R < ioff + nbl;
        for (int t = 0; t < nb; ++t) {
            const bool t_local = t >= ioff && t < ioff + nbl;
            if ((r_local && qn_symsh_owns(R, t, nb)) || (t_local && t != R && qn_symsh_owns(t, R, nb))) idx.push_back(t);
        }
        off[R + 1] = (int)idx.size();
    }
    if (idx.empty()) idx.push_back(0);
    QNCHK(s->s2_sl_off.alloc(off.size()));
    QNCHK(s->s2_sl_idx.alloc(idx.size()));
    HIPCHK(hipMemcpy(s->s2_sl_off, off.data(), off.size() * sizeof(int), hipMemcpyHostToDevice));
    HIPCHK(hipMemcpy(s->s2_sl_idx, idx.data(), idx.size() * sizeof(int), hipMemcpyHostToDevice));
    s->s2_sl_nb = nb;
    return QN_OK;
}

static int solver_alloc_sym2(qn_solver* s) {
    const int nb = s->T.n_pad / QN_TB;
    hipStream_t st = s->ctx->stream;
    const int world = s->ctx->world, rank = s->ctx->rank;
    const bool sharded = world > 1;
    const int cfg = (s->fold ? 1 : 0) | (s->no_sliver ? 2 : 0) | (sharded ? 4 : 0);
    if (s->s2_nb != nb || s->s2_sl_cfg != cfg) {
        s->s2_items.reset(); s->s2_wgS.reset(); s->s2_partE.reset(); s->s2_evS.reset(); s->s2_cnt.reset();
        s->s2_wgV.reset();
        if (s->s2_graph_exec) { (void)hipGraphExecDestroy(s->s2_graph_exec); s->s2_graph_exec = nullptr; }
        s->s2_nb = 0;
        const int nbl = s->T.rpr / QN_TB, ioff = rank * nbl;
        int nitems = nb * (nb + 1) / 2;
        int G = std::min(nitems, QN_S2_MAXG);
        if (sharded) {
            nitems = qn_symsh_ntiles(nb, nbl, ioff);
            int least = nitems;
            for (int r = 0; r < world; ++r) least = std::min(least, qn_symsh_ntiles(nb, nbl, r * nbl));
            G = std::min(least, QN_S2_MAXG);
            if (G < 1) return fail(QN_ABNORMAL_TERMINATION, "sym2: a rank without tiles");
        }
        std::vector<std::vector<int>> lists;
        int inorder = 0;
        auto deal = [&](int L) {
            lists.assign(G, std::vector<int>());
            std::vector<std::pair<double, int>> heap;
            for (int g = 0; g < G; ++g) heap.push_back({0.0, -g});
            std::make_heap(heap.begin(), heap.end());
            auto give = [&](int I, int J, double cost) {
                std::pop_heap(heap.begin(), heap.end());
                auto e = heap.back();
                lists[-e.second].push_back((I << 16) | J);
                e.first -= cost;
                heap.back() = e;
                std::push_heap(heap.begin(), heap.end());
            };
// ... 174 lines not shown
    HIPCHK(hipMemcpy(out, s->V.dbg, count * 8, hipMemcpyDeviceToHost));
    return QN_OK;
}
#endif

#ifdef QN_LU_STAMPS
extern "C" int qn_debug_lu_stamps(unsigned long long* out) {
    HIPCHK(hipDeviceSynchronize());
    HIPCHK(hipMemcpyFromSymbol(out, HIP_SYMBOL(qn_lu_dbg), sizeof(unsigned long long) * 64 * 16));
    return QN_OK;
}
#endif
extern "C" int qn_solver_set_profiling(qn_solver* s, int on) { s->profiling = on; return QN_OK; }
extern "C" int qn_solver_set_sync_mode(qn_solver* s, int sync) { s->sync_mode = sync; return QN_OK; }
extern "C" int qn_solver_set_option(qn_solver* s, int option, int value) {
    if (!s) return fail(QN_ERROR_INPUT_PARAMS, "null argument");
    const bool on = value != 0;
    switch (option) {
    case QN_OPT_GENERIC_KERNELS: s->no_fused = on ? 1 : 0; return QN_OK;
    case QN_OPT_DEFERRED_UPDATE_STEP: s->no_defer = on ? 0 : 1; return QN_OK;
    case QN_OPT_SYMMETRIC_STORAGE: s->no_sym = on ? 0 : 1; return QN_OK;
    case QN_OPT_SECOND_GENERATION: s->no_sym2 = on ? 0 : 1; return QN_OK;
    case QN_OPT_FOLDED_ACCEPT_REDUCE: s->fold = on ? 1 : 0; return QN_OK;
    case QN_OPT_ROW_SLIVERS: s->no_sliver = !on; return QN_OK;
    case QN_OPT_EVAL_PAIR_INSTANCE: s->no_pair = !on; return QN_OK;
    case QN_OPT_EVAL_MOVER_MULTIPLIER: s->ring = on ? 1 : 0; return QN_OK;
    case QN_OPT_TAIL_REDUCE: s->tred = on; return QN_OK;
    case QN_OPT_BOUNDED_SECOND_GENERATION: s->no_s2bnd = !on; return QN_OK;
    case QN_OPT_NEWTON_PIVOTED_LU: s->newton_force_lu = on ? 1 : 0; return QN_OK;
    case QN_OPT_LU_PER_COLUMN_PANEL: s->newton_lu_percol = on ? 1 : 0; return QN_OK;
    case QN_OPT_LU_LOOKAHEAD: s->newton_lu_no_la = on ? 0 : 1; return QN_OK;
    case QN_OPT_LU_ONE_LAUNCH_PANEL: s->newton_lu_no_persist = on ? 0 : 1; return QN_OK;
    case QN_OPT_LU_FORCE_WAIT_EXPIRY: s->newton_lu_force_timeout = on ? 1 : 0; return QN_OK;
    case QN_OPT_BTB_PROJECT_IN_EVAL: s->no_projfold = !on; return QN_OK;
    case QN_OPT_EVAL_ZIGZAG: s->zig = on ? 1 : 0; return QN_OK;
    case QN_OPT_PNEWTON_REUSE_FACTOR: s->pn_reuse = on ? 1 : 0; s->pn_factor_serial = 0; return QN_OK;
    case QN_OPT_LBFGS_UNIT_SCALING:
        if (s->method != QN_LBFGS) return fail(QN_ERROR_INPUT_PARAMS, "unit scaling belongs to an L-BFGS solver");
        return lbfgs_set_unit_scaling(s, on);
    case QN_OPT_PNORM_NONTEMPORAL:
        if (value < -1 || value > 1) return fail(QN_ERROR_INPUT_PARAMS, "non-temporal loads of inverse_p: 0 (plain), 1 (non-temporal) or -1 (by size)");
        s->pnorm_nt = value;
        return QN_OK;
    case QN_OPT_PNORM_ROWS_PER_WAVE:
        if (value != 0 && value != 2 && value != 4) return fail(QN_ERROR_INPUT_PARAMS, "rows per wave of the p-norm direction kernel: 2, 4 or 0 (by size)");
        s->pnorm_rw = value;
        return QN_OK;
    case QN_OPT_TOUCH_H_ROWS:
    case QN_OPT_TOUCH_Q_ROWS:
        if (value != 0 && value != 4 && value != 6 && value != 8 && value != 10 && value != 12 && value != 16) return fail(QN_ERROR_INPUT_PARAMS, "rows per wave to touch: 0, 4, 6, 8, 10, 12 or 16");
        (option == QN_OPT_TOUCH_H_ROWS ? s->touch : s->touchq) = value;
        return QN_OK;
    case QN_OPT_LU_SPLIT_ROLE_A:
        if (value != 0 && value != 1 && value != 2 && value != 4) return fail(QN_ERROR_INPUT_PARAMS, "role A runs as 1, 2 or 4 workgroups");
        s->newton_lu_split = value == 0 ? 1 : value;
        return QN_OK;
    case QN_OPT_LU_SPLIT_MIN_ROWS:
        if (value < 0) return fail(QN_ERROR_INPUT_PARAMS, "a number of rows");
        s->newton_lu_split_min = value;
        return QN_OK;
    case QN_OPT_CHUNKS_PER_TRIP:
        if (value != 1 && value != 2 && value != 4) return fail(QN_ERROR_INPUT_PARAMS, "chunks per trip must be 1, 2 or 4");
        s->U = value;
        return QN_OK;
    default: return fail(QN_ERROR_INPUT_PARAMS, "unknown option");
    }
}

extern "C" int qn_solver_set_tiling(qn_solver* s, int rows_per_block, int col_splits) {
    if (!s) return fail(QN_ERROR_INPUT_PARAMS, "null argument");
    if (rows_per_block != 0 && rows_per_block != 2 && rows_per_block != 4 && rows_per_block != 8 && rows_per_block != 16)
        return fail(QN_ERROR_INPUT_PARAMS, "rows_per_block must be 2, 4, 8 or 16 (diagnostics are named options: qn_solver_set_option)");
    if (col_splits < 0 || col_splits > 64) return fail(QN_ERROR_INPUT_PARAMS, "col_splits out of range");
    HIPCHK(hipSetDevice(s->ctx->device));
    if (rows_per_block) s->R = rows_per_block;
    if (col_splits) { s->hcs = col_splits; s->qcs = col_splits; }
    return solver_alloc_hp(s);
}

extern "C" size_t qn_solver_n(const qn_solver* s) { return s->n; }
extern "C" size_t qn_solver_k(const qn_solver* s) { return (size_t)s->hctl->k; }
extern "C" double qn_solver_tol(const qn_solver* s) { return s->tol; }

static int fused_export(qn_solver* s) {
    s->warm_obj = 0;
    if (!s->fused_live) return QN_OK;
    qn_context* c = s->ctx;
    const QnCtl* h = s->hctl;
    const size_t np = s->T.n_pad, vb = np * sizeof(double);
    HIPCHK(hipMemcpyAsync(s->V.x, s->V.F.X0 + (size_t)h->xc * np, vb, hipMemcpyDeviceToDevice, c->stream));
    if (h->pending) {
        HIPCHK(hipMemcpyAsync(s->V.sp, s->V.F.S0 + (size_t)h->sc * np, vb, hipMemcpyDeviceToDevice, c->stream));
        HIPCHK(hipMemcpyAsync(s->V.up, s->V.F.UN, vb, hipMemcpyDeviceToDevice, c->stream));
    }
    HIPCHK(hipStreamSynchronize(c->stream));
    s->fused_live = false;
    return QN_OK;
}

extern "C" int qn_solver_get_x(qn_solver* s, double* out) {
    HIPCHK(hipSetDevice(s->ctx->device));
    const double* src = s->fused_live ? s->V.F.X0 + (size_t)s->hctl->xc * (size_t)s->T.n_pad : s->V.x;
    HIPCHK(hipMemcpyAsync(out, src, s->n * sizeof(double), hipMemcpyDeviceToHost, s->ctx->stream));
    HIPCHK(hipStreamSynchronize(s->ctx->stream));
    return QN_OK;
}

static int poke_ctl(qn_solver* s) {
    HIPCHK(hipMemcpyAsync(s->ctl, s->hctl, sizeof(QnCtl), hipMemcpyHostToDevice, s->ctx->stream));
    HIPCHK(hipStreamSynchronize(s->ctx->stream));
    return QN_OK;
}
static int peek_ctl(qn_solver* s) {
    HIPCHK(hipMemcpyAsync(s->hctl, s->ctl, sizeof(QnCtl), hipMemcpyDeviceToHost, s->ctx->stream));
    HIPCHK(hipStreamSynchronize(s->ctx->stream));
    s->stats.host_syncs++;
    return QN_OK;
}

static int bounds_alloc(qn_solver* s) {
    if (s->bounds_block) return QN_OK;
    const size_t np = s->T.n_pad;
    QNCHK(s->bounds_block.alloc(4 * np));
    std::vector<double> init(4 * np);
    for (size_t i = 0; i < np; ++i) { init[i] = -INFINITY; init[np + i] = INFINITY; init[2 * np + i] = -INFINITY; init[3 * np + i] = INFINITY; }
    HIPCHK(hipMemcpy(s->bounds_block, init.data(), init.size() * sizeof(double), hipMemcpyHostToDevice));
    s->V.lb = s->bounds_block; s->V.ub = s->bounds_block + np; s->V.llb = s->bounds_block + 2 * np; s->V.lub = s->bounds_block + 3 * np;
    return QN_OK;
}
static int bounds_upload(qn_solver* s, double* dst, const double* src_host, double fill) {
    std::vector<double> v(s->T.n_pad, fill);
    if (src_host) memcpy(v.data(), src_host, s->n * sizeof(double));
    HIPCHK(hipMemcpy(dst, v.data(), v.size() * sizeof(double), hipMemcpyHostToDevice));
    return QN_OK;
}

extern "C" int qn_solver_set_bounds(qn_solver* s, const double* lb_host, const double* ub_host) {
    if (!s || !lb_host || !ub_host) return fail(QN_ERROR_INPUT_PARAMS, "null argument");
    if (s->method != QN_BFGS && s->method != QN_DFP && s->method != QN_SR1 && s->method != QN_BROYDEN && !vec_method(s->method))
        return fail(QN_ERROR_INPUT_PARAMS, "bounds need a BFGS / DFP / SR1 / Broyden / SPG / projected-gradient / L-BFGS solver");
    HIPCHK(hipSetDevice(s->ctx->device));
    QNCHK(bounds_alloc(s));
    QNCHK(bounds_upload(s, s->bounds_block, lb_host, -INFINITY));
    QNCHK(bounds_upload(s, s->bounds_block + s->T.n_pad, ub_host, INFINITY));
    std::vector<double> x(s->n);
    QNCHK(qn_solver_get_x(s, x.data()));
    for (size_t i = 0; i < s->n; ++i) x[i] = std::fmin(std::fmax(x[i], lb_host[i]), ub_host[i]);
    s->bounded = 1;
    return qn_solver_set_x(s, x.data());
}

extern "C" int qn_solver_reset(qn_solver* s, const double* x0_host) {
    if (!s || !x0_host) return fail(QN_ERROR_INPUT_PARAMS, "null argument");
    HIPCHK(hipSetDevice(s->ctx->device));
    hipStream_t st = s->ctx->stream;
    if (s->H) {
        hipLaunchKernelGGL(identity_fill_kernel, dim3(2048), dim3(256), 0, st, s->H, s->T);
        HIPCHK(hipGetLastError());
        s->h_lower_stale = false; s->h_diag_stale = false;
        s->h_nonsym = false;
    }
    s->fused_live = false; s->warm_obj = 0;
    HIPCHK(hipMemsetAsync(s->vec_block, 0, 9 * (size_t)s->T.n_pad * sizeof(double), st));
    std::vector<double> xp;
    if (vec_method(s->method) && s->bounded) {
        const size_t n = s->n;
        std::vector<double> lb(n), ub(n);
        HIPCHK(hipMemcpyAsync(lb.data(), s->bounds_block, n * sizeof(double), hipMemcpyDeviceToHost, st));
        HIPCHK(hipMemcpyAsync(ub.data(), s->bounds_block + s->T.n_pad, n * sizeof(double), hipMemcpyDeviceToHost, st));
// ... 179 lines not shown
    HIPCHK(hipSetDevice(c->device));
    QNCHK(flush_pending(s));
    const size_t np = s->T.n_pad, rpr = s->T.rpr;
    DevBuf<double> buf;
    QNCHK(buf.alloc_zero(2 * np, c->stream));
    HIPCHK(hipMemcpyAsync(buf, g_host, n * sizeof(double), hipMemcpyHostToDevice, c->stream));
    QNCHK(qn_gemv(c, s->H, np, rpr, n, buf, buf + np + (size_t)s->T.row_off));
    QNCHK(exchange(c, buf + np, rpr));
    HIPCHK(hipMemcpyAsync(d_host, buf + np, n * sizeof(double), hipMemcpyDeviceToHost, c->stream));
    HIPCHK(hipStreamSynchronize(c->stream));
    if (s->bounded) {
        std::vector<double> x(n), lb(n), ub(n);
        QNCHK(qn_solver_get_x(s, x.data()));
        HIPCHK(hipMemcpy(lb.data(), s->bounds_block, n * sizeof(double), hipMemcpyDeviceToHost));
        HIPCHK(hipMemcpy(ub.data(), s->bounds_block + np, n * sizeof(double), hipMemcpyDeviceToHost));
        for (size_t i = 0; i < n; ++i) {
            double t = x[i] - d_host[i];
            t = std::fmin(std::fmax(t, lb[i]), ub[i]);
            d_host[i] = t - x[i];
        }
        return QN_OK;
    }
    for (size_t i = 0; i < n; ++i) d_host[i] = -d_host[i];
    return QN_OK;
}

extern "C" int qn_solver_secant_update(qn_solver* s, const double* s_host, const double* y_host) {
    if (!s || !s_host || !y_host) return fail(QN_ERROR_INPUT_PARAMS, "null argument");
    if (s->method != QN_BROYDEN && ((s->method != QN_BFGS && s->method != QN_DFP) || s->bounded))
        return fail(QN_ERROR_INPUT_PARAMS, "secant update: BFGS, DFP and Broyden only");
    qn_context* c = s->ctx;
    HIPCHK(hipSetDevice(c->device));
    QNCHK(flush_pending(s));
    const size_t n = s->n, np = s->T.n_pad, rpr = s->T.rpr;
    double ss = 0.0, yy = 0.0, ys = 0.0;
    for (size_t i = 0; i < n; ++i) { ss += s_host[i] * s_host[i]; yy += y_host[i] * y_host[i]; ys += y_host[i] * s_host[i]; }
    QnCtl* h = s->hctl;
    h->has_s_norm = 1; h->s_norm = std::sqrt(ss);
    h->has_y_norm = 1; h->y_norm = std::sqrt(yy);
    h->have_dir = 0; h->have_cur_eval = 0;
    QNCHK(poke_ctl(s));
    if (h->s_norm < s->tol || h->y_norm < s->tol) return QN_OK;
    if (s->method == QN_BROYDEN) return r1_secant_update(s, s_host, y_host, ys);
    DevBuf<double> buf;
    QNCHK(buf.alloc_zero(3 * np, c->stream));
    std::vector<double> u(n);
    HIPCHK(hipMemcpyAsync(buf, s_host, n * sizeof(double), hipMemcpyHostToDevice, c->stream));
    HIPCHK(hipMemcpyAsync(buf + np, y_host, n * sizeof(double), hipMemcpyHostToDevice, c->stream));
    QNCHK(qn_gemv(c, s->H, np, rpr, n, buf + np, buf + 2 * np + (size_t)s->T.row_off));
    QNCHK(exchange(c, buf + 2 * np, rpr));
    HIPCHK(hipMemcpyAsync(u.data(), buf + 2 * np, n * sizeof(double), hipMemcpyDeviceToHost, c->stream));
    HIPCHK(hipStreamSynchronize(c->stream));
    double yu = 0.0;
    for (size_t i = 0; i < n; ++i) yu += y_host[i] * u[i];
    double c_ss, c_su, c_uu;
    if (s->method == QN_BFGS) { const double rho = 1.0 / ys; c_su = -rho; c_ss = rho * rho * yu + rho; c_uu = 0.0; }
    else { c_ss = 1.0 / ys; c_su = 0.0; c_uu = -1.0 / yu; }
    QNCHK(qn_rank2_update(c, s->H, np, (size_t)s->T.row_off, rpr, n, buf, buf + 2 * np, c_ss, c_su, c_uu));
    HIPCHK(hipStreamSynchronize(c->stream));
    return QN_OK;
}

extern "C" int qn_solver_set_inv_hessian(qn_solver* s, const double* h) {
    if (!s->H) return fail(QN_ERROR_INPUT_PARAMS, "gradient descent keeps no inverse Hessian");
    HIPCHK(hipSetDevice(s->ctx->device));
    const size_t n = s->n, np = s->T.n_pad;
    std::vector<double> rows((size_t)s->T.rpr * np, 0.0);
    for (size_t r = 0; r < (size_t)s->T.rpr; ++r) {
        const size_t i = (size_t)s->T.row_off + r;
        if (i >= n) break;
        for (size_t j = 0; j < n; ++j) rows[r * np + j] = h[i + j * n];
    }
    QNCHK(fused_export(s));
    HIPCHK(hipMemcpy(s->H, rows.data(), rows.size() * sizeof(double), hipMemcpyHostToDevice));
    s->h_lower_stale = false; s->h_diag_stale = false;
    s->h_nonsym = false;
    for (size_t i = 0; i < n && !s->h_nonsym; ++i)
        for (size_t j = i + 1; j < n; ++j)
            if (h[i + j * n] != h[j + i * n]) { s->h_nonsym = true; break; }
    s->hctl->pending = 0; s->hctl->have_dir = 0;
    return poke_ctl(s);
}

extern "C" int qn_solver_get_stats(qn_solver* s, qn_stats* out) {
    HIPCHK(hipSetDevice(s->ctx->device));
    prof_collect(s);
    *out = s->stats;
    return QN_OK;
}
```

### optimization-solvers_amd/csrc/qn_sym2.hip.h

```cpp
#pragma once
#include <type_traits>

#define QN_S2_TPB 512
#define QN_S2_WAVES 8
#define QN_S2_RPW 16
#define QN_S2_MAXG 256
#define QN_S2_NSE 6
#define QN_S2_NR 5
#define QN_S2_ROW 8
#define QN_S2SH_NEC 4
#define QN_S2SH_EB 4
#define QN_S2_CNT_STRIDE 1056
#define QN_S2_TRED_MAXK 31

enum { QN_S2_ADVANCE = 0, QN_S2_EVAL = 1, QN_S2_VEC = 2, QN_S2_HTILE = 3, QN_S2_HREDUCE = 4,
       QN_S2_VSUM = 5, QN_S2_HSUM = 6,
       QN_S2_GEVAL_A = 7, QN_S2_GCOMB = 8, QN_S2_GHT_A = 9,
       QN_S2_DIR = 10,
       QN_S2_PROJ = 11,
       QN_S2_VECD = 12 };

struct QnS2Args {
    const double* Q;
    double* H;
    int n, np, nb, G;
    const int* item_ij;
    int maxk;
    int inorder;
    QnFused F;
    double* part;
    double* partE;
    int pair;
    int fold;
    int tred;
    int method;
    int* cnt;
    int sl_first, sl_per;
    double* wgS;
    int trows;
    QnCtl* ctl2;
    QnTraceRec* trace;
    double* xtrace;
    int parity;
    const QnCtl* ctl_first;
    QnCtl* rep;
    unsigned long long* rep_flag;
    unsigned long long rep_seq;
    int nt;
    int ntq;
    int sh_world, sh_rank;
    int sh_ioff;
    int sh_nsum;
    double* evS;
    double* xg;
    const int* sl_off;
    const int* sl_idx;
    int cnt_stride;
    double* wgV;
    int gw;
    double gmu;
    double* gws;
    const double *lb, *ub;
    const double *llb, *lub;
    int ring;
    int projfold;
    int touch, touchq;
    int touch_delay, touchq_delay;
    int zig;
#ifdef QN_S2_STAMPS
    unsigned long long* dbg;
    int slot;
    int swz;
#endif
};
#ifdef QN_S2_STAMPS
#define QN_S2_WG(a) ((int)blockIdx.x ^ (a).swz)
#else
#define QN_S2_WG(a) ((int)blockIdx.x)
#endif
#ifdef QN_S2_STAMPS
#define QN_S2_STAMP(k) do { if (threadIdx.x == 0 && a.dbg && blockIdx.x < 256) a.dbg[(((size_t)(a.slot & 63)) * 256 + blockIdx.x) * 16 + (k)] = wall_clock64(); } while (0)
#define QN_S2_STAMP_T(k, t) do { if (threadIdx.x == (t) && a.dbg && blockIdx.x < 256) a.dbg[(((size_t)(a.slot & 63)) * 256 + blockIdx.x) * 16 + (k)] = wall_clock64(); } while (0)
#else
#define QN_S2_STAMP(k) do { } while (0)
#define QN_S2_STAMP_T(k, t) do { } while (0)
#endif

struct QnS2Lds {
    QnCtl c;
    double red[QN_S2_WAVES][8];
    int mine;
};

template <bool BND = false>
__device__ __forceinline__ void qn_s2_advance(QnCtl& c, const double* tot, const QnVecs& V, const bool leader, double* scratch, const bool resume) {
    const int ph = c.phase;
    bool run = resume;
    if (!resume) {
        if (ph == QN_PH_DONE) return;
        if (ph == QN_PH_IDLE) {
            c.serviced = 0;
            c.state = c.ls_only ? QN_ST_LS_ONLY : QN_ST_BEGIN;
            c.phase = QN_PH_RUNNING;
            run = true;
        } else {
            if (c.serviced != 2) return;
            c.serviced = 0;
            if (ph == QN_PH_REQ_EVAL) {
                const double f = 0.5 * tot[0] - tot[1];
                const double gd = tot[2] - tot[3];
                c.st_gd0 = tot[4]; c.st_dnf = tot[5];
                const bool proj = BND && c.req_project != 0;
                if (c.req_kind == QN_REQ_T && !c.gd0_valid && !proj) { c.gd0 = tot[4]; c.d_finite = tot[5] == 0.0; c.gd0_valid = 1; }
                c.f_e = f; c.gd_e = gd;
                c.n_oracle_evals++;
                c.ev_par ^= 1; c.ev_kind = c.req_kind; c.ev_t = c.req_t;
                if (c.req_kind == QN_REQ_T && !proj) { c.last_valid = 1; c.last_t = c.req_t; c.f_last = f; c.gd_last = gd; }
                else c.last_valid = 0;
                if (BND) c.last_projected = proj ? 1 : 0;
                if (c.req_need_vectors) { c.phase = QN_PH_REQ_VEC; return; }
                c.state = c.after_state;
            } else if (ph == QN_PH_REQ_VEC) {
                c.st_yy = tot[0]; c.st_ys = tot[1]; c.st_gg = tot[2]; c.st_ss = tot[3]; c.hp_sg = tot[4];
                c.state = c.after_state;
            } else if (ph == QN_PH_REQ_HPASS) {
                if (c.hp_nrhs == 2) { c.hp_yu = tot[0]; c.hp_ug = tot[1]; if (BND) c.hp_den = tot[2]; }
                c.state = c.after_state;
            } else if (BND && ph == QN_PH_REQ_DIR) {
                c.mtb_cand = tot[0];
                if (c.s2_dir & 2) c.mt_tmax = fmin(c.mt_tmax, c.mtb_cand);
                c.dir_mode = 0; c.dir_ready = 1;
                c.state = c.after_state;
            } else {
                return;
            }
            c.phase = QN_PH_RUNNING;
            run = true;
        }
    }
    if (run) ctl_scalar_run<BND ? 2 : 1>(c, V, scratch, leader);
    if (c.spec_tiles && c.phase != QN_PH_RUNNING && c.phase != QN_PH_REQ_VEC) {
        const int ran = c.spec_tiles;
        c.spec_tiles = 0;
        if (c.phase == QN_PH_REQ_HPASS && c.serviced == 0 && c.hp_nrhs == ran) c.serviced = 1;
        else if (c.pending) { c.pending = 0; c.n_hpasses++; c.n_hpass_rw++; }
    }
}

// ... 719 lines not shown
            e_u = a.F.UN[gi]; e_b = a.F.b[gi]; e_g = a.F.G[gi];
        }
    };
    if (wave == 7) {
#pragma unroll
        for (int k = 0; k < 4; ++k) cw[k] = qn_code_warm_issue(k * 64 + lane);
    }
    if (SHARD) { if (wave == 0) qn_s2_prologue_w0<(DECIDE ? QN_S2_VECD : QN_S2_VEC), true>(a, L, entries); else entries(); }
    else if (wave == 0) qn_s2_prologue_w0<QN_S2_VEC>(a, L, [&]() { qn_s2_slot_issue<1>(a.partE, a.nb, R, 0, S0); entries(); });
    else { qn_s2_slot_issue<1>(a.partE, a.nb, R, 0, S0); entries(); }
    __syncthreads();
    QN_S2_STAMP(2);
    qn_s2_ctl_out(a, L);
    qn_code_warm_done(cw[0] ^ cw[1] ^ cw[2] ^ cw[3], a.n < 0, a.wgS);
    if (!L.mine) return;
    const QnEvalReq q = qn_s2_eval_req<false>(L.c, true);
    double* __restrict__ xt = a.F.X0 + (size_t)(1 - q.xc) * np;
    double* __restrict__ sstage = a.F.S0 + (size_t)(1 - q.sc) * np;
    double qi = 0.0;
    if (!SHARD) qi = qn_s2_slot_sum<1>(a.partE, a.nb, R, 0, S0, qbuf);
    else if (tid < QN_TB) {
        const double* xp = a.xg + (size_t)R * QN_TB + tid;
        qi = xp[0];
        for (int r = 1; r < a.sh_nsum; ++r) qi = qi + xp[(size_t)r * np];
    }
    double p[8];
#pragma unroll
    for (int k = 0; k < 8; ++k) p[k] = 0.0;
    if (tid < QN_TB) {
        const int gi = R * QN_TB + tid;
        double di;
        const double xi = q.xc ? e_x1 : e_x0;
        const double xti = qn_s2_trial(q, xi, e_v, q.sc ? e_s1 : e_s0, e_u, di);
        const double bi = e_b, go = e_g;
        const double gti = qi - bi;
        const double yi = gti - go;
        const double si = xti - xi;
        a.F.GT[gi] = gti;
        a.F.Y[gi] = yi;
        xt[gi] = xti;
        sstage[gi] = si;
        p[0] = yi * yi; p[1] = yi * si; p[2] = gti * gti; p[3] = si * si; p[4] = si * gti;
    }
    if (wave < 2) {
        QnWaveFold<8, 32>::run(p, lane);
        if ((lane & 7) == 0) bred[wave][lane >> 3] = p[0];
    }
    __syncthreads();
    if (tid < QN_S2_NR) a.wgS[((size_t)a.parity * QN_S2_ROW + tid) * a.trows + R] = bred[0][tid] + bred[1][tid];
    QN_S2_STAMP(14);
}

template <bool SR1 = false>
__device__ __forceinline__ void qn_s2_hreduce_row(const QnS2Args& a, const int R, const int nrhs, const double tot0, const double tot1, double (*bred)[8],
                                                  const double gp, const double yv, const int half = -1, const double snew = 0.0) {
    const int tid = threadIdx.x, lane = tid & 63, wave = tid >> 6;
    if (half == 1) {
        if (tid < QN_TB && nrhs == 2) a.F.VV[R * QN_TB + tid] = tot1;
        return;
    }
    double p[8];
#pragma unroll
    for (int k = 0; k < 8; ++k) p[k] = 0.0;
    if (tid < QN_TB) {
        const int gi = R * QN_TB + tid;
        if (nrhs == 2) {
            a.F.UN[gi] = tot0;
            if (half < 0) a.F.VV[gi] = tot1;
            p[0] = yv * tot0;
            if (SR1) p[2] = (snew - tot0) * yv;
            p[1] = tot0 * gp;
        } else {
            a.F.VV[gi] = tot0;
        }
        a.F.G[gi] = gp;
    }
    if (wave < 2) {
        QnWaveFold<8, 32>::run(p, lane);
        if ((lane & 7) == 0) bred[wave][lane >> 3] = p[0];
    }
    __syncthreads();
    if (tid < (SR1 ? 3 : 2)) a.wgS[((size_t)a.parity * QN_S2_ROW + tid) * a.trows + R] = bred[0][tid] + bred[1][tid];
}
struct QnS2HReq {
    const double *sp, *up, *r0v, *gt;
    double c_ss, c_su, c_uu;
    bool pending;
};
struct QnS2HVec {
    double s_r, u_r, y0_r, y1_r;
    v2d s_c, u_c, a0, a1;
};
template <bool RHS = true>
__device__ __forceinline__ void qn_s2_hvec_load(const QnS2HReq& q, const unsigned ir, const unsigned jc, QnS2HVec& v) {
    v.s_r = q.sp[ir]; v.u_r = q.up[ir];
    v.s_c = ld2(q.sp + jc); v.u_c = ld2(q.up + jc);
    if (RHS) { v.y0_r = q.r0v[ir]; v.y1_r = q.gt[ir]; v.a0 = ld2(q.r0v + jc); v.a1 = ld2(q.gt + jc); }
}

#define QN_S2_FOLD_ITEMS 3
#define QN_S2_FOLD_BLOCKS (2 * QN_S2_FOLD_ITEMS)

template <bool NT, bool BFGS, bool FOLD, bool SHARD = false, bool TRED = false, bool SR1 = false>
__global__ __launch_bounds__(QN_S2_TPB, 2) void s2_hpass_kernel(const QnS2Args a) {
    static_assert(!(FOLD && SHARD), "the folded accept-reduce is a single-rank variant");
    static_assert(!(TRED && (FOLD || SHARD)), "the tail reduce is the single-rank kernel without the folded accept-reduce");
    static_assert(!(SR1 && (FOLD || SHARD || TRED || BFGS)), "SR1: the plain single-rank instance");
    __shared__ QnS2Lds L;
    __shared__ double colsum[2][QN_TB];
    __shared__ double colred[QN_S2_WAVES][2][QN_TB];
    __shared__ double fq[FOLD ? QN_S2_FOLD_BLOCKS : 1][4][QN_TB];
    __shared__ double fbg[FOLD ? QN_S2_FOLD_BLOCKS : 1][2][QN_TB];
    __shared__ double fv[FOLD ? QN_S2_FOLD_BLOCKS : 1][3][QN_TB];
    __shared__ double fred[2][8];
    const int tid = threadIdx.x, lane = tid & 63, wave = tid >> 6;
    const size_t np = (size_t)a.np;
    QN_S2_STAMP(0);
    int ij = qn_s2_first_item_of<SHARD>(a);
    const int ij1 = qn_s2_second_item(a);
    const int ij2 = (FOLD && ij1 >= 0 && a.maxk > 2) ? a.item_ij[(size_t)2 * a.G + blockIdx.x] : -1;
    int I = ij >> 16, J = ij & 0xffff;
    __shared__ v2d park0[QN_S2_RPW][64];
    QnS2HVec v0;
    double s1_r, y_r;
    v2d s1_c, y_c;
    auto vec_spec = [&]() {
        const int ir = I * QN_TB + wave * QN_S2_RPW + (lane & 15), jc = J * QN_TB + qn_s2_col(I == J, lane, wave);
        QnS2HReq spec;
        spec.sp = a.F.S0; spec.up = a.F.UN; spec.r0v = a.F.GT; spec.gt = a.F.GT;
        qn_s2_hvec_load<!FOLD>(spec, ir, jc, v0);
        s1_r = a.F.S0[np + ir]; s1_c = ld2(a.F.S0 + np + jc);
        if (!FOLD) { y_r = a.F.Y[ir]; y_c = ld2(a.F.Y + jc); }
    };
    if (wave == 0) qn_s2_prologue_w0<QN_S2_HTILE, SHARD>(a, L, vec_spec);
    int blk[QN_S2_FOLD_BLOCKS];
    {
        const int ijs[QN_S2_FOLD_ITEMS] = {ij, ij1 >= 0 ? ij1 : ij, ij2 >= 0 ? ij2 : ij};
#pragma unroll
        for (int k = 0; k < QN_S2_FOLD_ITEMS; ++k) { blk[2 * k] = ijs[k] >> 16; blk[2 * k + 1] = ijs[k] & 0xffff; }
    }
    double sv[QN_S2_FOLD_BLOCKS][8], sx[8], bg[QN_S2_FOLD_BLOCKS];
    if (FOLD && wave > 0) {
        const int per = (a.nb + 3) / 4;
        const int e = tid & (QN_TB - 1), qd = tid >> 7;
        const int k_lo = qd * per, k_hi = min(a.nb, k_lo + per);
#pragma unroll
        for (int b = 0; b < QN_S2_FOLD_BLOCKS; ++b) {
            const double* p = a.partE + ((size_t)blk[b] * a.nb) * QN_TB + e;
#pragma unroll
            for (int u = 0; u < 8; ++u) sv[b][u] = (k_lo + u < k_hi) ? p[(size_t)(k_lo + u) * QN_TB] : 0.0;
        }
        if (wave <= QN_S2_FOLD_BLOCKS) {
            const double* p = a.partE + ((size_t)blk[wave - 1] * a.nb) * QN_TB + lane;
#pragma unroll
            for (int u = 0; u < 8; ++u) sx[u] = (u < min(a.nb, per)) ? p[(size_t)u * QN_TB] : 0.0;
        }
        if (wave >= 4) {
            const double* src = (wave >= 6) ? a.F.G : a.F.b;
#pragma unroll
            for (int b = 0; b < QN_S2_FOLD_BLOCKS; ++b) bg[b] = src[blk[b] * QN_TB + e];
        }
    }
    v2d h[QN_S2_RPW];
    double* hbase = a.H + (size_t)(qn_s2_lrow<SHARD>(a, I) * QN_TB + wave * QN_S2_RPW) * np + (size_t)J * QN_TB + qn_s2_col(I == J, lane, wave);
    if (wave != 0) {
#pragma unroll
        for (int r = 0; r < QN_S2_RPW; ++r) h[r] = qn_sym_ld<NT>(hbase + (size_t)r * np);
        vec_spec();
        const double* q0 = a.H + (size_t)(qn_s2_lrow<SHARD>(a, I) * QN_TB) * np + (size_t)J * QN_TB + 2 * lane;
        const int r0 = (wave - 1) * 3;
        v2d t3[3];
#pragma unroll
        for (int k = 0; k < 3; ++k) t3[k] = qn_sym_ld<NT>(q0 + (size_t)min(r0 + k, QN_S2_RPW - 1) * np);
#pragma unroll
        for (int k = 0; k < 3; ++k)
            if (r0 + k < QN_S2_RPW) park0[r0 + k][lane] = t3[k];
    }
    if (FOLD && wave > 0) {
        const int e = tid & (QN_TB - 1), qd = tid >> 7;
#pragma unroll
        for (int b = 0; b < QN_S2_FOLD_BLOCKS; ++b) {
            double acc = 0.0;
#pragma unroll
            for (int u = 0; u < 8; ++u) acc = acc + sv[b][u];
            fq[b][qd][e] = acc;
        }
        if (wave <= QN_S2_FOLD_BLOCKS) {
            double acc = 0.0;
#pragma unroll
            for (int u = 0; u < 8; ++u) acc = acc + sx[u];
            fq[wave - 1][0][lane] = acc;
        }
        if (wave >= 4) {
#pragma unroll
            for (int b = 0; b < QN_S2_FOLD_BLOCKS; ++b) fbg[b][(wave - 4) >> 1][e] = bg[b];
        }
    }
    __syncthreads();
    qn_s2_ctl_out(a, L);
    const int mine = L.mine;
    if (!mine) return;
    QN_S2_STAMP(2);
    if (wave == 0) {
#pragma unroll
        for (int r = 0; r < QN_S2_RPW; ++r) h[r] = park0[r][lane];
    }
    const bool fold = FOLD && mine == 2;
    QnS2HReq q;
    bool nrhs2;
    {
        const QnCtl& c = L.c;
        q.pending = c.pending != 0;
        q.c_ss = c.c_ss; q.c_su = c.c_su; q.c_uu = c.c_uu;
        q.sp = a.F.S0 + (size_t)c.sc * np;
        q.up = a.F.UN;
        q.gt = a.F.GT;
        nrhs2 = fold ? (c.ev_kind == QN_REQ_T) : (c.hp_nrhs == 2);
        q.r0v = nrhs2 ? a.F.Y : a.F.GT;
        if (c.sc) { v0.s_r = s1_r; v0.s_c = s1_c; }
        if (!FOLD && nrhs2) { v0.y0_r = y_r; v0.a0 = y_c; }
    }
    if (FOLD) {
        if (tid < QN_TB) {
            if (fold) {
#pragma unroll
                for (int b = 0; b < QN_S2_FOLD_BLOCKS; ++b) {
                    const double qi = ((fq[b][0][tid] + fq[b][1][tid]) + fq[b][2][tid]) + fq[b][3][tid];
                    const double gti = qi - fbg[b][0][tid];
                    const double yi = gti - fbg[b][1][tid];
                    fv[b][0][tid] = nrhs2 ? yi : gti;
                    fv[b][1][tid] = gti;
                    fv[b][2][tid] = yi;
                }
            } else {
#pragma unroll
                for (int b = 0; b < QN_S2_FOLD_BLOCKS; ++b) {
                    const int gi = blk[b] * QN_TB + tid;
                    fv[b][0][tid] = q.r0v[gi];
                    fv[b][1][tid] = q.gt[gi];
                }
            }
        }
        __syncthreads();
        const int rr = wave * QN_S2_RPW + (lane & 15), cc = qn_s2_col(I == J, lane, wave);
        v0.y0_r = fv[0][0][rr]; v0.y1_r = fv[0][1][rr];
        v0.a0 = (v2d){fv[1][0][cc], fv[1][0][cc + 1]}; v0.a1 = (v2d){fv[1][1][cc], fv[1][1][cc + 1]};
    }
    const bool pend = q.pending;
    const double c_ss = pend ? q.c_ss : 0.0, c_su = pend ? q.c_su : 0.0, c_uu = pend ? q.c_uu : 0.0;
    const bool slv = !FOLD && !SHARD && a.sl_per != 0;
    auto sliver_ptr = [&]() {
        const QnS2Sliver sl = qn_s2_sliver(a, wave);
        unsigned r = sl.D * QN_TB + sl.row, c = sl.D * QN_TB + 2 * lane;
        asm volatile("" : "+v"(r), "+v"(c));
        return a.H + (size_t)r * np + c;
    };
    for (int it = 0;; ++it) {
        const bool diag = I == J;
        const double sr = pend ? v0.s_r : 0.0, ur = pend ? v0.u_r : 0.0;
        const double y0r = v0.y0_r, y1r = v0.y1_r;
        v2d sj = {0.0, 0.0}, uj = {0.0, 0.0};
        if (pend) { sj = v0.s_c; uj = v0.u_c; }
        v2d a0 = v0.a0, a1 = v0.a1;
        if (!qn_s2_row_on(diag, lane, wave)) { a0 = (v2d){0.0, 0.0}; a1 = (v2d){0.0, 0.0}; }
        int ijn = -1;
        if (it == 0) ijn = ij1;
        else if (FOLD) { if (it == 1) ijn = ij2; }
        else if (it + 1 < a.maxk) ijn = a.item_ij[(size_t)(it + 1) * a.G + blockIdx.x];
        const bool has_next = ijn >= 0;
        const int In = has_next ? (ijn >> 16) : I, Jn = has_next ? (ijn & 0xffff) : J;
        double* hnext = a.H + (size_t)(qn_s2_lrow<SHARD>(a, In) * QN_TB + wave * QN_S2_RPW) * np + (size_t)Jn * QN_TB + qn_s2_col(In == Jn, lane, wave);
        if (!has_next && slv) hnext = sliver_ptr();
        const size_t rstride = has_next ? np : 0;
        double c0x = 0.0, c0y = 0.0, c1x = 0.0, c1y = 0.0;
        double racc[QN_S2_RPW];
#pragma unroll
        for (int r = 0; r < QN_S2_RPW; ++r) {
            v2d hn = h[r];
            h[r] = qn_sym_ld<NT>(hnext + (size_t)r * rstride);
            const double si = qn_lane_bcast(sr, r), ui = qn_lane_bcast(ur, r);
            if (BFGS || SR1) {
                hn.x = hn.x + c_su * (si * uj.x + ui * sj.x);
                hn.y = hn.y + c_su * (si * uj.y + ui * sj.y);
            }
            hn.x = hn.x + c_ss * (si * sj.x);
            hn.y = hn.y + c_ss * (si * sj.y);
            if (!BFGS || SR1) {
                hn.x = hn.x + c_uu * (ui * uj.x);
                hn.y = hn.y + c_uu * (ui * uj.y);
            }
            qn_sym_st<NT>(hbase + (size_t)r * np, hn);
            const double y0 = qn_lane_bcast(y0r, r), y1 = qn_lane_bcast(y1r, r);
            double t0 = hn.x * a0.x;
            t0 = __builtin_fma(hn.y, a0.y, t0);
            double t1 = hn.x * a1.x;
            t1 = __builtin_fma(hn.y, a1.y, t1);
            {
                const auto rl = __builtin_amdgcn_permlane32_swap(__double2loint(t0), __double2loint(t1), false, false);
                const auto rh = __builtin_amdgcn_permlane32_swap(__double2hiint(t0), __double2hiint(t1), false, false);
                racc[r] = __hiloint2double(rh[0], rl[0]) + __hiloint2double(rh[1], rl[1]);
            }
            c0x = __builtin_fma(hn.x, y0, c0x);
            c0y = __builtin_fma(hn.y, y0, c0y);
            c1x = __builtin_fma(hn.x, y1, c1x);
            c1y = __builtin_fma(hn.y, y1, c1y);
        }
        if (!qn_s2_col_on(diag, lane, wave)) { c0x = 0.0; c0y = 0.0; c1x = 0.0; c1y = 0.0; }
        if (has_next) {
            const int irn = In * QN_TB + wave * QN_S2_RPW + (lane & 15), ccn = qn_s2_col(In == Jn, lane, wave);
            qn_s2_hvec_load<!FOLD>(q, irn, Jn * QN_TB + ccn, v0);
            if (FOLD) {
                const int rr = wave * QN_S2_RPW + (lane & 15), bI = 2 * (it + 1), bJ = bI + 1;
                v0.y0_r = fv[bI][0][rr]; v0.y1_r = fv[bI][1][rr];
                v0.a0 = (v2d){fv[bJ][0][ccn], fv[bJ][0][ccn + 1]}; v0.a1 = (v2d){fv[bJ][1][ccn], fv[bJ][1][ccn + 1]};
            }
        } else if (slv) {
            const QnS2Sliver sl = qn_s2_sliver(a, wave);
            unsigned r = sl.D * QN_TB + sl.row, c = sl.D * QN_TB + 2 * lane;
            asm volatile("" : "+v"(r), "+v"(c));
            qn_s2_hvec_load<true>(q, r, c, v0);
        }
        if (it == 0) { qn_keepalive(racc[0]); QN_S2_STAMP(3); QN_S2_STAMP_T(12, 448); }
        if (it == 1) { qn_keepalive(racc[0]); QN_S2_STAMP(6); QN_S2_STAMP_T(13, 448); }
        QnWaveFold<QN_S2_RPW, 16>::run(racc, lane);
        colred[wave][0][2 * lane] = c0x;
        colred[wave][0][2 * lane + 1] = c0y;
        colred[wave][1][2 * lane] = c1x;
        colred[wave][1][2 * lane + 1] = c1y;
        if ((lane & 1) == 0) {
            const int rhs = lane >> 5, rl = wave * QN_S2_RPW + ((lane >> 1) & 15);
            if (diag) colsum[rhs][rl] = racc[0];
            else qn_s2_slot_st<TRED>(a.part + (unsigned)(((I * a.nb + J) * 2 + rhs) * QN_TB + rl), racc[0]);
        }
        __syncthreads();
        if (tid < 2 * QN_TB) {
            const int crhs = tid / QN_TB, c = tid % QN_TB;
            double acc = colred[0][crhs][c];
#pragma unroll
            for (int w = 1; w < QN_S2_WAVES; ++w) acc = acc + colred[w][crhs][c];
            if (diag) qn_s2_slot_st<TRED>(a.part + (unsigned)(((I * a.nb + I) * 2 + crhs) * QN_TB + c), colsum[crhs][c] + acc);
            else qn_s2_slot_st<TRED>(a.part + (unsigned)(((J * a.nb + I) * 2 + crhs) * QN_TB + c), acc);
        }
        if (it == 0) QN_S2_STAMP(5);
        if (!has_next) break;
        I = In; J = Jn; hbase = hnext;
        __syncthreads();
    }
    if (slv) {
        v2d hn = h[0];
        const double si = pend ? v0.s_r : 0.0, ui = pend ? v0.u_r : 0.0;
        v2d sj = {0.0, 0.0}, uj = {0.0, 0.0};
        if (pend) { sj = v0.s_c; uj = v0.u_c; }
        if (BFGS || SR1) {
            hn.x = hn.x + c_su * (si * uj.x + ui * sj.x);
            hn.y = hn.y + c_su * (si * uj.y + ui * sj.y);
        }
        hn.x = hn.x + c_ss * (si * sj.x);
        hn.y = hn.y + c_ss * (si * sj.y);
        if (!BFGS || SR1) {
            hn.x = hn.x + c_uu * (ui * uj.x);
            hn.y = hn.y + c_uu * (ui * uj.y);
        }
        qn_sym_st<NT>(sliver_ptr(), hn);
        double t0 = hn.x * v0.a0.x;
        t0 = __builtin_fma(hn.y, v0.a0.y, t0);
        double t1 = hn.x * v0.a1.x;
        t1 = __builtin_fma(hn.y, v0.a1.y, t1);
        double tt[2] = {t0, t1};
        QnWaveFold<2, 32>::run(tt, lane);
        const QnS2Sliver sl = qn_s2_sliver(a, wave);
        if ((lane & 31) == 0) qn_s2_slot_st<TRED>(a.part + (unsigned)(((sl.D * a.nb + sl.D) * 2 + (lane >> 5)) * QN_TB + sl.row), tt[0]);
    }
    QN_S2_STAMP(15);
    if (TRED) {
        __shared__ int todo[2 * QN_S2_TRED_MAXK + 2];
        __shared__ double qbuf[3][QN_TB];
        asm volatile("s_waitcnt vmcnt(0)" ::: "memory");
        __syncthreads();
        QN_S2_STAMP(7);
        if (wave == 0) {
            const int k = lane >> 1;
            int R = -1;
            if (k < a.maxk) {
                const int ijk = k == 0 ? ij : (k == 1 ? ij1 : a.item_ij[(size_t)k * a.G + blockIdx.x]);
                if (ijk >= 0) {
                    const int Ik = ijk >> 16, Jk = ijk & 0xffff;
                    R = (lane & 1) ? (Jk != Ik ? Jk : -1) : Ik;
                }
            } else if (lane == 2 * a.maxk && slv) R = qn_s2_sliver(a, 0).D;
            bool last = false;
            if (R >= 0) {
                const int expect = (a.nb - 1) + ((a.sl_per != 0 && R >= a.sl_first) ? a.sl_per : 1);
                int* cp = a.cnt + (size_t)R * a.cnt_stride;
                last = __hip_atomic_fetch_add(cp, 1, __ATOMIC_RELAXED, __HIP_MEMORY_SCOPE_AGENT) + 1 == expect;
                if (last) __hip_atomic_store(cp, 0, __ATOMIC_RELAXED, __HIP_MEMORY_SCOPE_AGENT);
            }
            const unsigned long long m = __ballot(last);
            if (last) todo[1 + __popcll(m & ((1ull << lane) - 1ull))] = R;
            if (lane == 0) todo[0] = __popcll(m);
        }
        __syncthreads();
        QN_S2_STAMP(8);
        const int ntodo = todo[0];
        const int nrhs = L.c.hp_nrhs;
        for (int t = 0; t < ntodo; ++t) {
            const int R = todo[1 + t];
            QnS2Slots S0, S1;
            qn_s2_slot_issue<2, true>(a.part, a.nb, R, 0, S0);
            qn_s2_slot_issue<2, true>(a.part, a.nb, R, 1, S1);
            const double tot0 = qn_s2_slot_sum<2, true>(a.part, a.nb, R, 0, S0, qbuf);
            const double tot1 = (nrhs == 2) ? qn_s2_slot_sum<2, true>(a.part, a.nb, R, 1, S1, qbuf) : 0.0;
            double gp = 0.0, yv = 0.0;
            if (tid < QN_TB) { gp = a.F.GT[R * QN_TB + tid]; yv = a.F.Y[R * QN_TB + tid]; }
            qn_s2_hreduce_row(a, R, nrhs, tot0, tot1, fred, gp, yv);
            __syncthreads();
        }
        QN_S2_STAMP(14);
        return;
    }
    if (!fold) return;
    const QnEvalReq qe = qn_s2_eval_req<false>(L.c, true);
    const double* __restrict__ x = a.F.X0 + (size_t)qe.xc * np;
    double* __restrict__ xt = a.F.X0 + (size_t)(1 - qe.xc) * np;
    const double* __restrict__ spv = a.F.S0 + (size_t)qe.sc * np;
    double* __restrict__ sstage = a.F.S0 + (size_t)(1 - qe.sc) * np;
#pragma unroll 1
    for (int k = 0; k < QN_S2_FOLD_ITEMS; ++k) {
        const int ij_k = k == 0 ? ij : (k == 1 ? ij1 : ij2);
        if (ij_k < 0 || (ij_k >> 16) != (ij_k & 0xffff)) continue;
        const int R = ij_k >> 16;
        __syncthreads();
        if (tid < QN_TB) {
            const int gi = R * QN_TB + tid;
            const double gti = fv[2 * k][1][tid], yi = fv[2 * k][2][tid];
            double di;
            const double xi = x[gi];
            const double xti = qn_s2_trial(qe, xi, a.F.VV[gi], spv[gi], a.F.UN[gi], di);
            const double si = xti - xi;
            a.F.GT[gi] = gti;
            a.F.Y[gi] = yi;
            xt[gi] = xti;
            sstage[gi] = si;
            double p[8] = {yi * yi, yi * si, gti * gti, si * si, si * gti, 0.0, 0.0, 0.0};
            QnWaveFold<8, 32>::run(p, lane);
            if ((lane & 7) == 0) fred[wave][lane >> 3] = p[0];
        }
        __syncthreads();
        if (tid < QN_S2_NR) a.wgS[((size_t)a.parity * QN_S2_ROW + tid) * a.trows + R] = fred[0][tid] + fred[1][tid];
    }
}

template <bool SHARD = false, bool SR1 = false, int NBT = 0>
__global__ __launch_bounds__(QN_S2_TPB) void s2_hreduce_kernel(const QnS2Args a) {
    static_assert(!(SHARD && SR1), "SR1 runs on one rank");
    __shared__ QnS2Lds L;
    __shared__ double qbuf[3][QN_TB];
    __shared__ double bred[2][8];
    const int tid = threadIdx.x, wave = tid >> 6;
    const int R = SHARD ? (int)blockIdx.x : (int)(blockIdx.x >> 1), half = SHARD ? -1 : (int)(blockIdx.x & 1);
    if (NBT > 0 && __builtin_expect((int)blockIdx.x >= 2 * NBT, 0)) {
        const int b = (int)blockIdx.x - 2 * NBT;
        const int ij0 = qn_s2_item_of_index(b, NBT), ij1 = qn_s2_item_of_index(a.G + b, NBT);
        const bool flip = a.zig != 0 && ((a.parity ^ 1) & 1) != 0 && (ij1 >> 16) != (ij1 & 0xffff);
        for (int k = 0; k < a.touchq_delay; k += 8) __builtin_amdgcn_s_sleep(8);
        qn_s2_touch(a.Q, a, flip ? ij1 : ij0, a.touchq);
        return;
    }
    QnS2Slots S0;
    QN_S2_STAMP(0);
    double gp = 0.0, yv = 0.0, s0e = 0.0, s1e = 0.0;
    auto entries = [&]() {
        if (half != 1 && tid < QN_TB) {
            gp = a.F.GT[R * QN_TB + tid]; yv = a.F.Y[R * QN_TB + tid];
            if (SR1) { s0e = a.F.S0[R * QN_TB + tid]; s1e = a.F.S0[(size_t)a.np + R * QN_TB + tid]; }
        }
    };
    if (SHARD) { if (wave == 0) qn_s2_prologue_w0<QN_S2_HREDUCE, true>(a, L, entries); else entries(); }
    else if (wave == 0) qn_s2_prologue_w0<QN_S2_HREDUCE>(a, L, [&]() { qn_s2_slot_issue(a.part, a.nb, R, half, S0); entries(); });
    else { qn_s2_slot_issue(a.part, a.nb, R, half, S0); entries(); }
    __syncthreads();
    QN_S2_STAMP(2);
    qn_s2_ctl_out(a, L);
    if (!L.mine) return;
    const int nrhs = L.c.hp_nrhs;
    double tot0 = 0.0, tot1 = 0.0;
    if (!SHARD) {
        if (half == 1 && nrhs != 2) return;
        const double t = qn_s2_slot_sum(a.part, a.nb, R, half, S0, qbuf);
        if (half == 0) tot0 = t; else tot1 = t;
    } else if (tid < QN_TB) {
        const size_t np = (size_t)a.np;
        const double* xp = a.xg + (size_t)R * QN_TB + tid;
        tot0 = xp[0]; tot1 = xp[np];
        for (int r = 1; r < a.sh_nsum; ++r) { tot0 = tot0 + xp[(size_t)r * 2 * np]; tot1 = tot1 + xp[(size_t)r * 2 * np + np]; }
        if (nrhs != 2) tot1 = 0.0;
    }
    QN_S2_STAMP(13);
    qn_s2_hreduce_row<SR1>(a, R, nrhs, tot0, tot1, bred, gp, yv, half, L.c.sc ? s0e : s1e);
    QN_S2_STAMP(12);
}

template <bool WRITE>
__global__ __launch_bounds__(QN_S2_TPB, 2) void s2_place_probe_kernel(double* __restrict__ M, const int nb, const int np_, const int G, double* __restrict__ sink) {
    const int lane = threadIdx.x & 63, wave = threadIdx.x >> 6;
    const size_t np = (size_t)np_;
    const int nitems = nb * (nb + 1) / 2;
    double acc = 0.0;
#pragma unroll 1
    for (int k = 0; k < 2; ++k) {
        const int t = k * G + (int)blockIdx.x;
        if (t >= nitems) break;
        const int ij = qn_s2_item_of_index(t, nb);
        const int I = ij >> 16, J = ij & 0xffff;
        double* hb = M + (size_t)(I * QN_TB + wave * QN_S2_RPW) * np + (size_t)J * QN_TB + 2 * lane;
        v2d h[QN_S2_RPW];
#pragma unroll
        for (int r = 0; r < QN_S2_RPW; ++r) h[r] = ld2(hb + (size_t)r * np);
#pragma unroll
        for (int r = 0; r < QN_S2_RPW; ++r) {
            if (WRITE) {
                asm volatile("" : "+v"(h[r]));
                st2(hb + (size_t)r * np, h[r]);
            } else acc += h[r].x + h[r].y;
        }
    }
    if (!WRITE && acc == 12345.678) sink[blockIdx.x] = acc;
}

template <bool SHARD = false, bool GOBJ = false, int KIND = QN_S2_ADVANCE, bool BND = false>
__global__ __launch_bounds__(128) void s2_advance_kernel(const QnS2Args a) {
    __shared__ QnS2Lds L;
    if (threadIdx.x < 64) qn_s2_prologue_w0<KIND, SHARD, QnS2NoEarly, GOBJ, BND>(a, L);
    __syncthreads();
    qn_s2_ctl_out(a, L);
}

__global__ __launch_bounds__(QN_TB) void s2_dir_kernel(const QnS2Args a) {
    __shared__ QnS2Lds L;
    __shared__ double red[2];
    const int R = blockIdx.x, tid = threadIdx.x, lane = tid & 63, wave = tid >> 6;
    const int gi = R * QN_TB + tid;
    const size_t np = (size_t)a.np;
    double x0 = 0.0, x1 = 0.0, s0 = 0.0, s1 = 0.0, vv = 0.0, un = 0.0, lbi = -INFINITY, ubi = INFINITY, llbi = -INFINITY, lubi = INFINITY;
    auto entries = [&]() {
        x0 = a.F.X0[gi]; x1 = a.F.X0[np + gi]; s0 = a.F.S0[gi]; s1 = a.F.S0[np + gi]; vv = a.F.VV[gi]; un = a.F.UN[gi];
        if (a.lb) { lbi = a.lb[gi]; ubi = a.ub[gi]; }
        if (a.llb) { llbi = a.llb[gi]; lubi = a.lub[gi]; }
    };
    if (wave == 0) qn_s2_prologue_w0<QN_S2_DIR, false, decltype(entries)&, false, true>(a, L, entries);
    else entries();
    __syncthreads();
    qn_s2_ctl_out(a, L);
    if (!L.mine) return;
    const QnCtl& c = L.c;
    const double xi = c.xc ? x1 : x0, si = c.sc ? s1 : s0;
    const double al = c.c_su * c.dir_ug + c.c_ss * c.dir_sg, be = c.c_su * c.dir_sg + c.c_uu * c.dir_ug;
    const double w = c.dir_mode ? (vv + __builtin_fma(be, un, al * si)) : vv;
    double di = -w;
    if (c.s2_dir & 1) { double t = xi - w; t = fmin(fmax(t, lbi), ubi); di = t - xi; }
    a.F.VV[gi] = -di;
    double cand = INFINITY;
    if (c.s2_dir & 2) { if (di > 0.0) cand = (lubi - xi) / di; else if (di < 0.0) cand = (llbi - xi) / di; }
#pragma unroll
    for (int off = 32; off >= 1; off >>= 1) cand = fmin(cand, __shfl_xor(cand, off, 64));
    if (lane == 0) red[wave] = cand;
    __syncthreads();
    if (tid == 0) a.wgS[((size_t)a.parity * QN_S2_ROW + 0) * a.trows + R] = fmin(red[0], red[1]);
}

__global__ __launch_bounds__(QN_TB) void s2_proj_kernel(const QnS2Args a) {
    __shared__ QnS2Lds L;
// ... 43 lines not shown
```

### optimization-solvers_amd/solver.py

```python
import atexit
import ctypes as C
import weakref

import numpy as np

from . import _abi as A

_live = {"solver": weakref.WeakSet(), "objective": weakref.WeakSet(), "context": weakref.WeakSet()}


@atexit.register
def _close_all():
    for kind in ("solver", "objective", "context"):
        for obj in list(_live[kind]):
            try:
                obj.close()
            except Exception:
                pass


OPTIONS = {
    "generic_kernels": 1,
    "deferred_update_step": 2,
    "symmetric_storage": 3,
# ... 630 lines not shown
        x = _f64(x)
        _check(A.lib().qn_solver_set_x(self.h, _dp(x)))

    def k(self):
        return A.lib().qn_solver_k(self.h)

    def set_k(self, k):
        _check(A.lib().qn_solver_set_k(self.h, int(k)))

    def identity(self):
        return np.eye(self.n)

    def tol(self):
        return A.lib().qn_solver_tol(self.h)

    def _opt(self, fn):
        v, some = C.c_double(), C.c_int()
        _check(fn(self.h, C.byref(v), C.byref(some)))
        return v.value if some.value else None

    def s_norm(self):
        return self._opt(A.lib().qn_solver_s_norm)

    def y_norm(self):
        return self._opt(A.lib().qn_solver_y_norm)

    def next_iterate_too_close(self):
        v = C.c_int()
        _check(A.lib().qn_solver_next_iterate_too_close(self.h, C.byref(v)))
        return bool(v.value)

    def gradient_next_iterate_too_close(self):
        v = C.c_int()
        _check(A.lib().qn_solver_gradient_next_iterate_too_close(self.h, C.byref(v)))
        return bool(v.value)

    def has_converged(self, eval_x_k):
        if self.next_iterate_too_close() or self.gradient_next_iterate_too_close():
            return True
        g = eval_x_k.g() if isinstance(eval_x_k, FuncEvalMultivariate) else eval_x_k[1]
        return float(np.sqrt(np.dot(g, g))) < self.tol()

    def approx_inv_hessian(self, all_ranks=True):
        out = np.zeros((self.n, self.n), order="F")
        _check(A.lib().qn_solver_get_inv_hessian(self.h, out.ctypes.data_as(A.dp), 1 if all_ranks else 0))
        return np.ascontiguousarray(out)

    def compute_direction(self, eval_x_k):
        g = _f64(eval_x_k.g() if isinstance(eval_x_k, FuncEvalMultivariate) else eval_x_k[1])
        if g.size != self.n:
            raise ErrorInputParams("gradient has the wrong dimension")
        d = np.empty(self.n)
        _check(A.lib().qn_solver_compute_direction(self.h, g.ctypes.data_as(A.dp), d.ctypes.data_as(A.dp)))
        return d

    def secant_update(self, s, y):
        s, y = _f64(s), _f64(y)
        if s.size != self.n or y.size != self.n:
            raise ErrorInputParams("s / y have the wrong dimension")
        _check(A.lib().qn_solver_secant_update(self.h, s.ctypes.data_as(A.dp), y.ctypes.data_as(A.dp)))

    def set_approx_inv_hessian(self, h):
        a = np.asfortranarray(h, dtype=np.float64)
        _check(A.lib().qn_solver_set_inv_hessian(self.h, a.ctypes.data_as(A.dp)))

    def set_trace(self, cap, with_x=False):
        self._trace_cap = cap
        self._trace_x = with_x
        _check(A.lib().qn_solver_set_trace(self.h, cap, 1 if with_x else 0))

    def trace(self):
        cap = self._trace_cap
        recs = (A.TraceRec * max(cap, 1))()
        ln = C.c_size_t()
        xs = np.zeros((max(cap, 1), self.n)) if getattr(self, "_trace_x", False) else None
        _check(A.lib().qn_solver_get_trace(self.h, recs, cap, C.byref(ln), _dp(xs) if xs is not None else None))
        out = [dict(f=r.f, gnorm=r.gnorm, t=r.t, s_norm=r.s_norm, y_norm=r.y_norm, n_evals=r.n_evals, ls_iters=r.ls_iters,
                    ls_cases=r.ls_cases, updated=r.updated) for r in recs[:ln.value]]
        return out, (xs[:ln.value] if xs is not None else None)

    def stats(self):
        st = A.Stats()
        _check(A.lib().qn_solver_get_stats(self.h, C.byref(st)))
        return {k: getattr(st, k) for k, _ in A.Stats._fields_}

    def set_profiling(self, on):
        _check(A.lib().qn_solver_set_profiling(self.h, 1 if on else 0))

    def set_sync_mode(self, sync):
        _check(A.lib().qn_solver_set_sync_mode(self.h, int(sync)))

    def set_tiling(self, rows_per_block=0, col_splits=0):
        _check(A.lib().qn_solver_set_tiling(self.h, rows_per_block, col_splits))

    def set_option(self, option, value=1):
        if isinstance(option, str):
            option = OPTIONS[option]
        _check(A.lib().qn_solver_set_option(self.h, int(option), int(value)))

    def configure(self, what, value=0):
        if isinstance(what, str):
            self.set_option(what, value)
        else:
            self.set_tiling(what, value)


class BFGS(_SolverBase):
    METHOD = A.BFGS


class DFP(_SolverBase):
    METHOD = A.DFP


class Broyden(_SolverBase):
    METHOD = A.BROYDEN


class GradientDescent(_SolverBase):
    METHOD = A.GRADIENT_DESCENT

    def has_converged(self, eval_x_k):
        g = eval_x_k.g() if isinstance(eval_x_k, FuncEvalMultivariate) else eval_x_k[1]
        return float(np.max(np.abs(g))) < self.tol()


class CoordinateDescent(GradientDescent):
    METHOD = A.COORDINATE_DESCENT

    def grad_tol(self):
        return self.tol()


class PnormDescent(GradientDescent):
    METHOD = A.PNORM_DESCENT

    def __init__(self, grad_tol, x0, inverse_p, ctx=None):
        super().__init__(grad_tol, x0, ctx)
        if inverse_p is not None:
            self.set_inverse_p(inverse_p)

    def set_inverse_p(self, inverse_p):
        p = np.asfortranarray(inverse_p, dtype=np.float64)
        if p.shape != (self.n, self.n):
            raise ErrorInputParams("inverse_p must be n x n")
        _check(A.lib().qn_solver_set_inverse_p(self.h, p.ctypes.data_as(A.dp)))

    @classmethod
    def new(cls, grad_tol, x0, inverse_p, ctx=None):
        return cls(grad_tol, x0, inverse_p, ctx)

    def grad_tol(self):
        return self.tol()

    def inverse_p(self):
        out = np.zeros((self.n, self.n), order="F")
        _check(A.lib().qn_solver_get_inverse_p(self.h, out.ctypes.data_as(A.dp)))
        return np.ascontiguousarray(out)


class _BoundedBase(_SolverBase):

    def __init__(self, tol, x0, lower_bound, upper_bound, ctx=None):
        super().__init__(tol, x0, ctx)
        self._lb, self._ub = _f64(lower_bound), _f64(upper_bound)
        _check(A.lib().qn_solver_set_bounds(self.h, _dp(self._lb), _dp(self._ub)))

# ... 205 lines not shown
```

### rust/src/ffi.rs

```rust
#![allow(non_camel_case_types)]
use std::os::raw::{c_char, c_int, c_void};

pub const QN_ABI_VERSION: c_int = 5;

pub const QN_OK: c_int = 0;
pub const QN_MAX_ITER_REACHED: c_int = 1;
pub const QN_OUT_OF_DOMAIN: c_int = 2;
pub const QN_ERROR_INPUT_PARAMS: c_int = 3;
pub const QN_ABNORMAL_TERMINATION: c_int = 4;

pub const QN_LS_MORETHUENTE: i32 = 0;
pub const QN_LS_BACKTRACKING: i32 = 1;
pub const QN_LS_MORETHUENTE_B: i32 = 2;
pub const QN_LS_BACKTRACKING_B: i32 = 3;
pub const QN_LS_GLL_QUADRATIC: i32 = 4;
pub const QN_LS_NO_SEARCH: i32 = 5;
pub const QN_LS_STRONG_WOLFE: i32 = 6;

pub const QN_ORACLE_HOST: i32 = 0;
pub const QN_ORACLE_DEVICE_FN: i32 = 1;
pub const QN_ORACLE_OBJECTIVE: i32 = 2;

pub const QN_BFGS: c_int = 0;
pub const QN_DFP: c_int = 1;
// ... 147 lines not shown
}

extern "C" {
    pub fn qn_status_string(status: c_int) -> *const c_char;
    pub fn qn_last_error_message() -> *const c_char;
    pub fn qn_abi_version() -> c_int;

    pub fn qn_device_count(out: *mut c_int) -> c_int;
    pub fn qn_context_create(device: c_int, out: *mut *mut qn_context) -> c_int;
    pub fn qn_comm_unique_id(out_128_bytes: *mut c_void) -> c_int;
    pub fn qn_context_create_sharded(device: c_int, rank: c_int, world: c_int, unique_id: *const c_void, out: *mut *mut qn_context) -> c_int;
    pub fn qn_context_create_sharded_host_exchange(device: c_int, rank: c_int, world: c_int, fn_: qn_host_allgather_fn, user: *mut c_void, out: *mut *mut qn_context) -> c_int;
    pub fn qn_context_set_allreduce(ctx: *mut qn_context, on: c_int) -> c_int;
    pub fn qn_context_set_host_exchange_async(ctx: *mut qn_context, on: c_int) -> c_int;
    pub fn qn_context_set_trial_vector_exchange(ctx: *mut qn_context, on: c_int) -> c_int;
    pub fn qn_context_destroy(ctx: *mut qn_context);
    pub fn qn_partition(n: usize, world: c_int, rows_per_rank: *mut usize, n_pad: *mut usize) -> c_int;
    pub fn qn_comm_selftest(ctx: *mut qn_context) -> c_int;
    pub fn qn_context_comm_check(ctx: *mut qn_context) -> c_int;
    pub fn qn_context_exchange_probe(ctx: *mut qn_context, count: usize, reps: c_int, out_us: *mut f64) -> c_int;
    pub fn qn_context_event_bracket_overhead(ctx: *mut qn_context, reps: c_int, out_ms: *mut f64) -> c_int;
    pub fn qn_context_synchronize(ctx: *mut qn_context) -> c_int;
    pub fn qn_context_rank(ctx: *const qn_context) -> c_int;
    pub fn qn_context_world(ctx: *const qn_context) -> c_int;
    pub fn qn_context_stream(ctx: *mut qn_context) -> *mut c_void;

    pub fn qn_morethuente_default(ls: *mut qn_linesearch);
    pub fn qn_morethuente_with_deltas(ls: *mut qn_linesearch, dmin: f64, d: f64, dmax: f64) -> c_int;
    pub fn qn_morethuente_with_t_min(ls: *mut qn_linesearch, t_min: f64) -> c_int;
    pub fn qn_morethuente_with_t_max(ls: *mut qn_linesearch, t_max: f64) -> c_int;
    pub fn qn_morethuente_with_c1(ls: *mut qn_linesearch, c1: f64) -> c_int;
    pub fn qn_morethuente_with_c2(ls: *mut qn_linesearch, c2: f64) -> c_int;
    pub fn qn_backtracking_new(ls: *mut qn_linesearch, c1: f64, beta: f64);
    pub fn qn_morethuente_b_new(ls: *mut qn_linesearch);
    pub fn qn_backtracking_b_new(ls: *mut qn_linesearch, c1: f64, beta: f64, lower_bound_host: *const f64, upper_bound_host: *const f64);
    pub fn qn_linesearch_with_lower_bound(ls: *mut qn_linesearch, lower_bound_host: *const f64);
    pub fn qn_linesearch_with_upper_bound(ls: *mut qn_linesearch, upper_bound_host: *const f64);
    pub fn qn_nosearch_new(ls: *mut qn_linesearch);
    pub fn qn_gll_quadratic_new(ls: *mut qn_linesearch, c1: f64, m: usize);
    pub fn qn_gll_quadratic_with_sigmas(ls: *mut qn_linesearch, sigma1: f64, sigma2: f64);
    pub fn qn_strong_wolfe_new(ls: *mut qn_linesearch, c1: f64, c2: f64);
    pub fn qn_strong_wolfe_with_xtol(ls: *mut qn_linesearch, xtol: f64) -> c_int;

    pub fn qn_quadratic_create(ctx: *mut qn_context, n: usize, q_rowmajor_host: *const f64, b_host: *const f64, out: *mut *mut qn_objective) -> c_int;
    pub fn qn_quadratic_create_synthetic(ctx: *mut qn_context, n: usize, seed: u64, diag_host: *const f64, b_host: *const f64, out: *mut *mut qn_objective) -> c_int;
    pub fn qn_logsumexp_create(ctx: *mut qn_context, m: usize, n: usize, a_rowmajor_host: *const f64, c_host: *const f64, mu: f64, out: *mut *mut qn_objective) -> c_int;
    pub fn qn_objective_destroy(obj: *mut qn_objective);
    pub fn qn_objective_eval(obj: *mut qn_objective, x_host: *const f64, f: *mut f64, g_host: *mut f64) -> c_int;
    pub fn qn_objective_get_rows(obj: *mut qn_objective, row0: usize, nrows: usize, out_host: *mut f64) -> c_int;
    pub fn qn_objective_hessian(obj: *mut qn_objective, x_host: *const f64, h_colmajor_host: *mut f64) -> c_int;

    pub fn qn_solver_create(ctx: *mut qn_context, method: c_int, tol: f64, x0_host: *const f64, n: usize, out: *mut *mut qn_solver) -> c_int;
    pub fn qn_solver_destroy(s: *mut qn_solver);
    pub fn qn_solver_set_bounds(s: *mut qn_solver, lower_bound_host: *const f64, upper_bound_host: *const f64) -> c_int;
    pub fn qn_solver_set_inverse_p(s: *mut qn_solver, p_colmajor_host: *const f64) -> c_int;
    pub fn qn_solver_get_inverse_p(s: *mut qn_solver, out_colmajor_host: *mut f64) -> c_int;
    pub fn qn_solver_set_spg_lambdas(s: *mut qn_solver, lambda_min: f64, lambda_max: f64) -> c_int;
    pub fn qn_solver_spg_lambda(s: *mut qn_solver, out: *mut f64, is_some: *mut c_int) -> c_int;
    pub fn qn_solver_newton_factorisations(s: *mut qn_solver, out: *mut usize) -> c_int;
    pub fn qn_solver_set_lbfgs_memory(s: *mut qn_solver, m: usize) -> c_int;
    pub fn qn_solver_lbfgs_state(s: *mut qn_solver, m: *mut usize, stored: *mut usize, gamma: *mut f64, resets: *mut usize) -> c_int;
    pub fn qn_solver_reset(s: *mut qn_solver, x0_host: *const f64) -> c_int;
    pub fn qn_minimize(s: *mut qn_solver, ls: *mut qn_linesearch, oracle: *const qn_oracle, max_iter_solver: usize, max_iter_line_search: usize, callback: qn_callback_fn, callback_user: *mut c_void) -> c_int;
    pub fn qn_compute_step_len(ctx: *mut qn_context, ls: *mut qn_linesearch, x_k_host: *const f64, f_k: f64, g_k_host: *const f64, direction_host: *const f64, n: usize, oracle: *const qn_oracle, max_iter: usize, step_out: *mut f64) -> c_int;
    pub fn qn_solver_n(s: *const qn_solver) -> usize;
    pub fn qn_solver_k(s: *const qn_solver) -> usize;
    pub fn qn_solver_set_k(s: *mut qn_solver, k: usize) -> c_int;
    pub fn qn_solver_tol(s: *const qn_solver) -> f64;
    pub fn qn_solver_get_x(s: *mut qn_solver, out_host: *mut f64) -> c_int;
    pub fn qn_solver_set_x(s: *mut qn_solver, x_host: *const f64) -> c_int;
    pub fn qn_solver_s_norm(s: *mut qn_solver, out: *mut f64, is_some: *mut c_int) -> c_int;
    pub fn qn_solver_y_norm(s: *mut qn_solver, out: *mut f64, is_some: *mut c_int) -> c_int;
    pub fn qn_solver_next_iterate_too_close(s: *mut qn_solver, out: *mut c_int) -> c_int;
    pub fn qn_solver_gradient_next_iterate_too_close(s: *mut qn_solver, out: *mut c_int) -> c_int;
    pub fn qn_solver_decrement_squared(s: *mut qn_solver, out: *mut f64, is_some: *mut c_int) -> c_int;
    pub fn qn_solver_get_inv_hessian(s: *mut qn_solver, out_colmajor_host: *mut f64, all_ranks: c_int) -> c_int;
    pub fn qn_solver_set_inv_hessian(s: *mut qn_solver, h_colmajor_host: *const f64) -> c_int;
    pub fn qn_solver_compute_direction(s: *mut qn_solver, g_host: *const f64, d_host: *mut f64) -> c_int;
    pub fn qn_solver_secant_update(s: *mut qn_solver, s_host: *const f64, y_host: *const f64) -> c_int;

    pub fn qn_solver_set_trace(s: *mut qn_solver, cap: usize, with_x: c_int) -> c_int;
    pub fn qn_solver_get_trace(s: *mut qn_solver, out_host: *mut qn_trace_rec, cap: usize, len: *mut usize, x_trace_host: *mut f64) -> c_int;
    pub fn qn_solver_get_stats(s: *mut qn_solver, out: *mut qn_stats) -> c_int;
    pub fn qn_solver_set_profiling(s: *mut qn_solver, on: c_int) -> c_int;
    pub fn qn_solver_set_sync_mode(s: *mut qn_solver, sync: c_int) -> c_int;
    pub fn qn_solver_set_tiling(s: *mut qn_solver, rows_per_block: c_int, col_splits: c_int) -> c_int;
    pub fn qn_solver_set_option(s: *mut qn_solver, option: c_int, value: c_int) -> c_int;

    pub fn qn_dev_alloc(ctx: *mut qn_context, bytes: usize, out_dev: *mut *mut c_void) -> c_int;
    pub fn qn_dev_free(ctx: *mut qn_context, dev: *mut c_void) -> c_int;
    pub fn qn_h2d(ctx: *mut qn_context, dst_dev: *mut c_void, src_host: *const c_void, bytes: usize) -> c_int;
    pub fn qn_d2h(ctx: *mut qn_context, dst_host: *mut c_void, src_dev: *const c_void, bytes: usize) -> c_int;
    pub fn qn_gemv(ctx: *mut qn_context, a_dev: *const f64, ld: usize, nrows: usize, ncols: usize, x_dev: *const f64, y_dev: *mut f64) -> c_int;
    pub fn qn_rank2_update(ctx: *mut qn_context, h_dev: *mut f64, ld: usize, row0: usize, nrows: usize, n: usize, s_dev: *const f64, u_dev: *const f64, c_ss: f64, c_su: f64, c_uu: f64) -> c_int;
    pub fn qn_axpy(ctx: *mut qn_context, n: usize, x_dev: *const f64, t: f64, d_dev: *const f64, out_dev: *mut f64) -> c_int;
    pub fn qn_dot(ctx: *mut qn_context, n: usize, a_dev: *const f64, b_dev: *const f64, out_host: *mut f64) -> c_int;
    pub fn qn_nrm2(ctx: *mut qn_context, n: usize, a_dev: *const f64, out_host: *mut f64) -> c_int;
}
```

### rust/src/lib.rs

```rust
pub mod ffi;

use ffi::*;
use nalgebra::{DMatrix, DVector};
use optimization_solvers::{
    ComputeDirection, CurvatureCondition, Floating, FuncEvalMultivariate, HasBounds, LineSearch, LineSearchSolver, MoreThuente,
    SolverError, SufficientDecreaseCondition,
};
use std::ffi::CStr;
use std::os::raw::{c_int, c_void};
use std::sync::OnceLock;

fn status_to_result(code: c_int) -> Result<(), SolverError> {
    match code {
        QN_OK => Ok(()),
        QN_MAX_ITER_REACHED => Err(SolverError::MaxIterReached),
        QN_OUT_OF_DOMAIN => Err(SolverError::OutOfDomain),
        QN_ERROR_INPUT_PARAMS => Err(SolverError::ErrorInputParams),
        _ => Err(SolverError::AbnormalTermination),
    }
}

pub fn last_error() -> String {
    unsafe { CStr::from_ptr(qn_last_error_message()).to_string_lossy().into_owned() }
}
// ... 701 lines not shown
            }
            fn set_lower_bound(&mut self, lower_bound: DVector<Floating>) {
                let ub = self.core.ub.clone();
                self.core.set_bounds(lower_bound, ub).expect("qn_solver_set_bounds");
            }
            fn set_upper_bound(&mut self, upper_bound: DVector<Floating>) {
                let lb = self.core.lb.clone();
                self.core.set_bounds(lb, upper_bound).expect("qn_solver_set_bounds");
            }
        }
    };
}
bounded_first_order!(GpuProjectedGradientDescent);
bounded_first_order!(GpuSpectralProjectedGradient);
bounded_first_order!(GpuProjectedNewton);
bounded_first_order!(GpuSpectralProjectedNewton);
bounded_first_order!(GpuProjectedLbfgs);
bounded_first_order!(GpuBroydenB);

macro_rules! newton_factorisations {
    ($name:ident) => {
        impl $name {
            pub fn newton_factorisations(&self) -> usize {
                let mut v = 0usize;
                unsafe { qn_solver_newton_factorisations(self.core.h, &mut v) };
                v
            }
        }
    };
}
newton_factorisations!(GpuProjectedNewton);
newton_factorisations!(GpuSpectralProjectedNewton);

impl GpuProjectedNewton {
    pub fn s_norm(&self) -> Option<Floating> {
        self.core.option(qn_solver_s_norm)
    }
    pub fn y_norm(&self) -> Option<Floating> {
        self.core.option(qn_solver_y_norm)
    }
    pub fn next_iterate_too_close(&self) -> bool {
        self.core.flag(qn_solver_next_iterate_too_close)
    }
    pub fn gradient_next_iterate_too_close(&self) -> bool {
        self.core.flag(qn_solver_gradient_next_iterate_too_close)
    }
}

impl GpuSpectralProjectedNewton {
    pub fn with_lambdas(self, lambda_min: Floating, lambda_max: Floating) -> Self {
        assert_eq!(unsafe { qn_solver_set_spg_lambdas(self.core.h, lambda_min, lambda_max) }, QN_OK, "{}", last_error());
        self
    }
    pub fn lambda(&self) -> Option<Floating> {
        self.core.option(qn_solver_spg_lambda)
    }
}

impl GpuSpectralProjectedGradient {
    pub fn with_lambdas(self, lambda_min: Floating, lambda_max: Floating) -> Self {
        assert_eq!(unsafe { qn_solver_set_spg_lambdas(self.core.h, lambda_min, lambda_max) }, QN_OK, "{}", last_error());
        self
    }
    pub fn lambda(&self) -> Option<Floating> {
        self.core.option(qn_solver_spg_lambda)
    }
}

macro_rules! quasi_newton_getters {
    ($name:ident) => {
        impl $name {
            pub fn s_norm(&self) -> Option<Floating> {
                self.core.option(qn_solver_s_norm)
            }
            pub fn y_norm(&self) -> Option<Floating> {
                self.core.option(qn_solver_y_norm)
            }
            pub fn next_iterate_too_close(&self) -> bool {
                self.core.flag(qn_solver_next_iterate_too_close)
            }
            pub fn gradient_next_iterate_too_close(&self) -> bool {
                self.core.flag(qn_solver_gradient_next_iterate_too_close)
            }
            pub fn approx_inv_hessian(&self) -> DMatrix<Floating> {
                self.core.approx_inv_hessian()
            }
            pub fn identity(&self) -> DMatrix<Floating> {
                DMatrix::identity(self.core.n, self.core.n)
            }
        }
    };
}
quasi_newton_getters!(GpuBFGS);
quasi_newton_getters!(GpuDFP);
```

Measured before the change: 13700.

## Defer inverse-Hessian store to every other pass by carrying two pending rank-2 updates

Lets the symmetric fused BFGS/DFP pass hold two pending rank-2 updates. Every other pass applies the older update in registers but suppresses its H stores through a zero-size buffer resource, so H is written only on alternate iterations. The previous s and u vectors are saved to a spare slot so the next pass can apply both updates. A collapse kernel flushes a leftover pending update on export or when the path changes. It also adds a counter and API for store passes. The cost is extra vector loads, more arithmetic per element and more complexity; it applies only to single-rank, non-folded, non-SR1 runs.

```diff
diff --git a/include/qn_hip.h b/include/qn_hip.h
--- a/include/qn_hip.h
+++ b/include/qn_hip.h
@@ -202,6 +202,7 @@
 #define QN_PATH_PNORM 512u
 #define QN_PATH_LBFGS 1024u
 int qn_solver_get_stats(qn_solver* s, qn_stats* out);
+int qn_solver_h_store_passes(qn_solver* s, size_t* out);
 int qn_solver_set_profiling(qn_solver* s, int on);
 int qn_solver_set_sync_mode(qn_solver* s, int sync);
 int qn_solver_set_tiling(qn_solver* s, int rows_per_block, int col_splits);
diff --git a/include/qn_solver.hpp b/include/qn_solver.hpp
--- a/include/qn_solver.hpp
+++ b/include/qn_solver.hpp
@@ -248,6 +248,7 @@
     bool next_iterate_too_close() const { int v; check(qn_solver_next_iterate_too_close(h_, &v)); return v != 0; }
     bool gradient_next_iterate_too_close() const { int v; check(qn_solver_gradient_next_iterate_too_close(h_, &v)); return v != 0; }
     DVector approx_inv_hessian() const { DVector m(n_ * n_); check(qn_solver_get_inv_hessian(h_, m.data(), 1)); return m; }
+    size_t h_store_passes() const { size_t v = 0; check(qn_solver_h_store_passes(h_, &v)); return v; }
     std::optional<Floating> decrement_squared() const { Floating v; int some; check(qn_solver_decrement_squared(h_, &v, &some)); return some ? std::optional<Floating>(v) : std::nullopt; }
     bool has_converged(const FuncEvalMultivariate& eval) const {
         if (METHOD == QN_NEWTON) {
diff --git a/optimization-solvers_amd/_abi.py b/optimization-solvers_amd/_abi.py
--- a/optimization-solvers_amd/_abi.py
+++ b/optimization-solvers_amd/_abi.py
@@ -144,6 +144,7 @@
     ("qn_solver_set_trace", C.c_int, [C.c_void_p, C.c_size_t, C.c_int]),
     ("qn_solver_get_trace", C.c_int, [C.c_void_p, C.POINTER(TraceRec), C.c_size_t, C.POINTER(C.c_size_t), dp]),
     ("qn_solver_get_stats", C.c_int, [C.c_void_p, C.POINTER(Stats)]),
+    ("qn_solver_h_store_passes", C.c_int, [C.c_void_p, C.POINTER(C.c_size_t)]),
     ("qn_solver_set_profiling", C.c_int, [C.c_void_p, C.c_int]),
     ("qn_solver_set_sync_mode", C.c_int, [C.c_void_p, C.c_int]),
     ("qn_solver_set_tiling", C.c_int, [C.c_void_p, C.c_int, C.c_int]),
diff --git a/optimization-solvers_amd/csrc/qn_ctl.h b/optimization-solvers_amd/csrc/qn_ctl.h
--- a/optimization-solvers_amd/csrc/qn_ctl.h
+++ b/optimization-solvers_amd/csrc/qn_ctl.h
@@ -119,4 +119,9 @@
     int32_t dir_ready;
 
     uint64_t n_oracle_calls, n_oracle_evals, n_hpasses, n_hpass_rw, n_iterations;
+
+    int32_t pend2;
+    int32_t defer_max;
+    double c2_ss, c2_su, c2_uu;
 };
+#define QN_CTL_PASS_KEEPS_H(c) ((c).defer_max == 2 && (c).hp_nrhs == 2 && (c).pending != 0 && (c).pend2 == 0)
diff --git a/optimization-solvers_amd/csrc/qn_ctl_step.hip.h b/optimization-solvers_amd/csrc/qn_ctl_step.hip.h
--- a/optimization-solvers_amd/csrc/qn_ctl_step.hip.h
+++ b/optimization-solvers_amd/csrc/qn_ctl_step.hip.h
@@ -78,7 +78,7 @@
     if (!LEAN && !c.fused) return false;
     c.n_hpasses++;
     if (c.pending) c.n_hpass_rw++;
-    c.pending = 0;
+    c.pending = 0; c.pend2 = 0;
     c.dir_mode = 0;
     c.gd0_valid = 0; c.d_finite = 0; c.last_valid = 0;
     c.state = QN_ST_LS_BEGIN;
@@ -123,9 +123,10 @@
     const double yu = c.hp_yu;
     double c_ss, c_su, c_uu;
     qn_update_coeffs(c.method, c.ys, yu, c_ss, c_su, c_uu, c.hp_den);
+    if (QN_CTL_PASS_KEEPS_H(c)) { c.pend2 = 1; c.c2_ss = c.c_ss; c.c2_su = c.c_su; c.c2_uu = c.c_uu; }
+    else { if (c.pending) c.n_hpass_rw++; c.pend2 = 0; }
     c.c_ss = c_ss; c.c_su = c_su; c.c_uu = c_uu;
     c.n_hpasses++;
-    if (c.pending) c.n_hpass_rw++;
     c.pending = 1;
     c.sc ^= 1;
     c.dir_mode = 1; c.dir_ug = c.hp_ug; c.dir_sg = c.hp_sg;
diff --git a/optimization-solvers_amd/csrc/qn_host_launch.hip.h b/optimization-solvers_amd/csrc/qn_host_launch.hip.h
--- a/optimization-solvers_amd/csrc/qn_host_launch.hip.h
+++ b/optimization-solvers_amd/csrc/qn_host_launch.hip.h
@@ -362,7 +362,7 @@
     QnCtl* pc = s->hrep;
     memcpy(pc, s->hctl, sizeof(QnCtl));
     pc->phase = QN_PH_REQ_HPASS; pc->serviced = 0; pc->hp_nrhs = 1; pc->pending = 0; pc->after_state = QN_ST_AFTER_DIR; pc->sym2 = 1; pc->fused = 1;
-    pc->spec_tiles = 0; pc->sc = 0; pc->xc = 0;
+    pc->spec_tiles = 0; pc->sc = 0; pc->xc = 0; pc->pend2 = 0; pc->defer_max = 1;
     PinnedBuf<QnCtl> pe;
     (void)pe.alloc(1, hipHostMallocMapped | hipHostMallocCoherent);
     if (pe) {
diff --git a/optimization-solvers_amd/csrc/qn_host_minimize.hip.h b/optimization-solvers_amd/csrc/qn_host_minimize.hip.h
--- a/optimization-solvers_amd/csrc/qn_host_minimize.hip.h
+++ b/optimization-solvers_amd/csrc/qn_host_minimize.hip.h
@@ -104,6 +104,8 @@
     h->serviced = 0; h->ev_par = 0; h->ev_kind = QN_REQ_X; h->ev_t = 0.0; h->spec_tiles = 0;
     h->defer_u = 0;
     h->no_defer = s->no_defer;
+    h->defer_max = 1;
+    if (h->pend2 && !r.sym2) QNCHK(s2_collapse_pending(s));
     if (!r.fused) QNCHK(fused_export(s));
     if (!(r.sym || r.sym_generic) || (s->h_diag_stale && (!r.sym2 || (r.gobj && c->world == 1) || r.tiles1))) QNCHK(ensure_full_h(s));
     if (r.fused) {
@@ -193,6 +195,14 @@
     s2_cache_policy(c->world > 1 ? (size_t)s->T.rpr * s->T.n_pad * 8 / 2 : (size_t)s->T.n_pad * s->T.n_pad * 8 / 2, &a.nt, &a.ntq);
     if (getenv("QN_S2_NT")) a.nt = atoi(getenv("QN_S2_NT"));
     if (getenv("QN_S2_NTQ")) a.ntq = atoi(getenv("QN_S2_NTQ"));
+    a.sold = s->fused_block + (size_t)10 * s->T.n_pad;
+    {
+        const bool plain = c->world == 1 && !r.gobj && !r.tiles1 && !a.fold && !a.tred && s->method != QN_SR1;
+        const bool depth1 = getenv("QN_S2_DEFER_DEPTH") && atoi(getenv("QN_S2_DEFER_DEPTH")) == 1;
+        QnCtl* h = s->hctl;
+        h->defer_max = (plain && !depth1) ? 2 : 1;
+        if (h->pend2 && !plain) QNCHK(s2_collapse_pending(s));
+    }
     return QN_OK;
 }
 
@@ -373,6 +383,8 @@
     }
     s->stats.h_bytes = (h->n_hpasses + h->n_hpass_rw) * shard;
     if (r.sym2) s->stats.h_bytes = 2 * h->n_hpasses * shard;
+    s->h_store_passes = h->n_hpass_rw;
+    if (r.sym2 && h->pend2) s->d2_args = r.s2;
     s->stats.obj_bytes = (r.oracle_tpl == QN_ORACLE_QUAD) ? h->n_oracle_evals * (r.sym ? shard : full_shard) : 0;
     if (r.obj && r.obj->kind == OBJ_LOGSUMEXP)
         s->stats.obj_bytes = h->n_oracle_evals * (uint64_t)r.obj->TA.rpr * (uint64_t)r.obj->T.n_pad * 8ull * ((r.obj->lse_kch && !r.obj->lse_two_pass) ? 1ull : 2ull);
diff --git a/optimization-solvers_amd/csrc/qn_host_solver.hip.h b/optimization-solvers_amd/csrc/qn_host_solver.hip.h
--- a/optimization-solvers_amd/csrc/qn_host_solver.hip.h
+++ b/optimization-solvers_amd/csrc/qn_host_solver.hip.h
@@ -94,6 +94,8 @@
     DevBuf<double> bounds_block;
     int bounded = 0;
     DevBuf<double> fused_block;
+    QnS2Args d2_args{};
+    uint64_t h_store_passes = 0;
     DevBuf<double> fused_evp, fused_hpp;
     int fused_nblk = 0;
     DevBuf<QnCtl> ctl;
@@ -170,7 +172,7 @@
 static int solver_alloc_fused(qn_solver* s, bool sym) {
     const size_t np = s->T.n_pad;
     hipStream_t st = s->ctx->stream;
-    QNCHK(s->fused_block.ensure(10 * np, st));
+    QNCHK(s->fused_block.ensure(11 * np, st));
     const int nblk = sym ? (int)(np / QN_TB) : s->T.rpr / s->R;
     if (sym) {
         QNCHK(s->sym_part.ensure((size_t)nblk * nblk * 2 * QN_TB, st));
@@ -511,9 +513,37 @@
 extern "C" size_t qn_solver_k(const qn_solver* s) { return (size_t)s->hctl->k; }
 extern "C" double qn_solver_tol(const qn_solver* s) { return s->tol; }
 
+static int s2_collapse_pending(qn_solver* s) {
+    QnCtl* h = s->hctl;
+    if (!h->pend2) return QN_OK;
+    if (!s->fused_live || !s->d2_args.sold || s->d2_args.H != s->H) return fail(QN_ABNORMAL_TERMINATION, "two updates pending outside the path that defers them");
+    hipStream_t st = s->ctx->stream;
+    QnCtl* pc = s->hrep;
+    memcpy(pc, h, sizeof(QnCtl));
+    pc->phase = QN_PH_REQ_HPASS; pc->serviced = 0; pc->hp_nrhs = 1; pc->pending = 0; pc->pend2 = 1; pc->defer_max = 1;
+    pc->after_state = QN_ST_AFTER_DIR; pc->sym2 = 1; pc->fused = 1; pc->spec_tiles = 0;
+    QnS2Args a = s->d2_args;
+    a.parity = 0; a.ctl_first = pc; a.rep = nullptr; a.rep_flag = nullptr; a.rep_seq = 0; a.tred = 0; a.fold = 0;
+    if (s->method == QN_BFGS) {
+        if (a.nt) hipLaunchKernelGGL((s2_hpass_kernel<true, true, false>), dim3(a.G), dim3(QN_S2_TPB), 0, st, a);
+        else hipLaunchKernelGGL((s2_hpass_kernel<false, true, false>), dim3(a.G), dim3(QN_S2_TPB), 0, st, a);
+    } else {
+        if (a.nt) hipLaunchKernelGGL((s2_hpass_kernel<true, false, false>), dim3(a.G), dim3(QN_S2_TPB), 0, st, a);
+        else hipLaunchKernelGGL((s2_hpass_kernel<false, false, false>), dim3(a.G), dim3(QN_S2_TPB), 0, st, a);
+    }
+    HIPCHK(hipGetLastError());
+    HIPCHK(hipStreamSynchronize(st));
+    s->stats.launches++;
+    s->h_lower_stale = true; s->h_diag_stale = true;
+    s->h_sliver_whole = a.sl_per != 0;
+    h->pend2 = 0;
+    return QN_OK;
+}
+
 static int fused_export(qn_solver* s) {
     s->warm_obj = 0;
     if (!s->fused_live) return QN_OK;
+    QNCHK(s2_collapse_pending(s));
     qn_context* c = s->ctx;
     const QnCtl* h = s->hctl;
     const size_t np = s->T.n_pad, vb = np * sizeof(double);
@@ -859,6 +889,12 @@
     return poke_ctl(s);
 }
 
+extern "C" int qn_solver_h_store_passes(qn_solver* s, size_t* out) {
+    if (!s || !out) return fail(QN_ERROR_INPUT_PARAMS, "null argument");
+    *out = (size_t)s->h_store_passes;
+    return QN_OK;
+}
+
 extern "C" int qn_solver_get_stats(qn_solver* s, qn_stats* out) {
     HIPCHK(hipSetDevice(s->ctx->device));
     prof_collect(s);
diff --git a/optimization-solvers_amd/csrc/qn_sym2.hip.h b/optimization-solvers_amd/csrc/qn_sym2.hip.h
--- a/optimization-solvers_amd/csrc/qn_sym2.hip.h
+++ b/optimization-solvers_amd/csrc/qn_sym2.hip.h
@@ -64,6 +64,7 @@
     const double *llb, *lub;
     int ring;
     int projfold;
+    double* sold;
     int touch, touchq;
     int touch_delay, touchq_delay;
     int zig;
@@ -949,19 +950,33 @@
     __syncthreads();
     if (tid < (SR1 ? 3 : 2)) a.wgS[((size_t)a.parity * QN_S2_ROW + tid) * a.trows + R] = bred[0][tid] + bred[1][tid];
 }
+typedef unsigned qn_v4u __attribute__((ext_vector_type(4)));
+__device__ __forceinline__ __amdgpu_buffer_rsrc_t qn_s2_tile_rsrc(double* H, const int row0, const int col0, const size_t np, const bool on) {
+    const unsigned long long base = (unsigned long long)(H + (size_t)row0 * np + col0);
+    const unsigned lo = __builtin_amdgcn_readfirstlane((unsigned)base), hi = __builtin_amdgcn_readfirstlane((unsigned)(base >> 32));
+    const unsigned bytes = __builtin_amdgcn_readfirstlane(on ? (unsigned)(QN_TB * np * 8) : 0u);
+    return __builtin_amdgcn_make_buffer_rsrc((void*)(((unsigned long long)hi << 32) | lo), 0, (int)bytes, 0x00020000);
+}
+template <bool NT> __device__ __forceinline__ void qn_s2_tile_st(const __amdgpu_buffer_rsrc_t rs, const unsigned voff, const unsigned soff, const v2d v) {
+    __builtin_amdgcn_raw_buffer_store_b128(__builtin_bit_cast(qn_v4u, v), rs, (int)voff, (int)soff, NT ? 2 : 0);
+}
 struct QnS2HReq {
     const double *sp, *up, *r0v, *gt;
     double c_ss, c_su, c_uu;
     bool pending;
+    const double *so, *uo;
 };
 struct QnS2HVec {
     double s_r, u_r, y0_r, y1_r;
     v2d s_c, u_c, a0, a1;
+    double so_r, uo_r;
+    v2d so_c, uo_c;
 };
-template <bool RHS = true>
+template <bool RHS = true, bool D2 = false>
 __device__ __forceinline__ void qn_s2_hvec_load(const QnS2HReq& q, const unsigned ir, const unsigned jc, QnS2HVec& v) {
     v.s_r = q.sp[ir]; v.u_r = q.up[ir];
     v.s_c = ld2(q.sp + jc); v.u_c = ld2(q.up + jc);
+    if (D2) { v.so_r = q.so[ir]; v.uo_r = q.uo[ir]; v.so_c = ld2(q.so + jc); v.uo_c = ld2(q.uo + jc); }
     if (RHS) { v.y0_r = q.r0v[ir]; v.y1_r = q.gt[ir]; v.a0 = ld2(q.r0v + jc); v.a1 = ld2(q.gt + jc); }
 }
 
@@ -973,7 +988,9 @@
     static_assert(!(FOLD && SHARD), "the folded accept-reduce is a single-rank variant");
     static_assert(!(TRED && (FOLD || SHARD)), "the tail reduce is the single-rank kernel without the folded accept-reduce");
     static_assert(!(SR1 && (FOLD || SHARD || TRED || BFGS)), "SR1: the plain single-rank instance");
+    constexpr bool D2 = !FOLD && !SHARD && !TRED && !SR1;
     __shared__ QnS2Lds L;
+    __shared__ double park_o[D2 ? 6 : 1][64];
     __shared__ double colsum[2][QN_TB];
     __shared__ double colred[QN_S2_WAVES][2][QN_TB];
     __shared__ double fq[FOLD ? QN_S2_FOLD_BLOCKS : 1][4][QN_TB];
@@ -995,7 +1012,9 @@
         const int ir = I * QN_TB + wave * QN_S2_RPW + (lane & 15), jc = J * QN_TB + qn_s2_col(I == J, lane, wave);
         QnS2HReq spec;
         spec.sp = a.F.S0; spec.up = a.F.UN; spec.r0v = a.F.GT; spec.gt = a.F.GT;
-        qn_s2_hvec_load<!FOLD>(spec, ir, jc, v0);
+        spec.so = a.sold; spec.uo = a.F.UP;
+        if (D2 && wave != 0) qn_s2_hvec_load<!FOLD, D2>(spec, ir, jc, v0);
+        else qn_s2_hvec_load<!FOLD>(spec, ir, jc, v0);
         s1_r = a.F.S0[np + ir]; s1_c = ld2(a.F.S0 + np + jc);
         if (!FOLD) { y_r = a.F.Y[ir]; y_c = ld2(a.F.Y + jc); }
     };
@@ -1034,6 +1053,13 @@
 #pragma unroll
         for (int r = 0; r < QN_S2_RPW; ++r) h[r] = qn_sym_ld<NT>(hbase + (size_t)r * np);
         vec_spec();
+        double w0o[D2 ? 6 : 1];
+        if (D2 && wave == 1) {
+            const int ir0 = I * QN_TB + (lane & 15), jc0 = J * QN_TB + qn_s2_col(I == J, lane, 0);
+            const v2d so0 = ld2(a.sold + jc0), uo0 = ld2(a.F.UP + jc0);
+            w0o[0] = a.sold[ir0]; w0o[D2 ? 1 : 0] = a.F.UP[ir0];
+            w0o[D2 ? 2 : 0] = so0.x; w0o[D2 ? 3 : 0] = so0.y; w0o[D2 ? 4 : 0] = uo0.x; w0o[D2 ? 5 : 0] = uo0.y;
+        }
         const double* q0 = a.H + (size_t)(qn_s2_lrow<SHARD>(a, I) * QN_TB) * np + (size_t)J * QN_TB + 2 * lane;
         const int r0 = (wave - 1) * 3;
         v2d t3[3];
@@ -1042,6 +1068,10 @@
 #pragma unroll
         for (int k = 0; k < 3; ++k)
             if (r0 + k < QN_S2_RPW) park0[r0 + k][lane] = t3[k];
+        if (D2 && wave == 1) {
+#pragma unroll
+            for (int k = 0; k < (D2 ? 6 : 1); ++k) park_o[k][lane] = w0o[k];
+        }
     }
     if (FOLD && wave > 0) {
         const int e = tid & (QN_TB - 1), qd = tid >> 7;
@@ -1071,13 +1101,25 @@
     if (wave == 0) {
 #pragma unroll
         for (int r = 0; r < QN_S2_RPW; ++r) h[r] = park0[r][lane];
+        if (D2) {
+            v0.so_r = park_o[0][lane]; v0.uo_r = park_o[D2 ? 1 : 0][lane];
+            v0.so_c = (v2d){park_o[D2 ? 2 : 0][lane], park_o[D2 ? 3 : 0][lane]}; v0.uo_c = (v2d){park_o[D2 ? 4 : 0][lane], park_o[D2 ? 5 : 0][lane]};
+        }
     }
     const bool fold = FOLD && mine == 2;
     QnS2HReq q;
     bool nrhs2;
+    bool pend2 = false, keep_h = false;
+    double c2_ss = 0.0, c2_su = 0.0, c2_uu = 0.0;
     {
         const QnCtl& c = L.c;
         q.pending = c.pending != 0;
+        q.so = a.sold; q.uo = a.F.UP;
+        if (D2) {
+            pend2 = c.pend2 != 0;
+            keep_h = QN_CTL_PASS_KEEPS_H(c);
+            if (pend2) { c2_ss = c.c2_ss; c2_su = c.c2_su; c2_uu = c.c2_uu; }
+        }
         q.c_ss = c.c_ss; q.c_su = c.c_su; q.c_uu = c.c_uu;
         q.sp = a.F.S0 + (size_t)c.sc * np;
         q.up = a.F.UN;
@@ -1122,12 +1164,19 @@
         asm volatile("" : "+v"(r), "+v"(c));
         return a.H + (size_t)r * np + c;
     };
+    const bool st_on = !keep_h;
+    const unsigned npb = (unsigned)np * 8u;
+    __amdgpu_buffer_rsrc_t rs = qn_s2_tile_rsrc(a.H, D2 ? I * QN_TB : 0, D2 ? J * QN_TB : 0, np, st_on);
+    unsigned voff = (unsigned)(wave * QN_S2_RPW) * npb + (unsigned)qn_s2_col(I == J, lane, wave) * 8u;
     for (int it = 0;; ++it) {
         const bool diag = I == J;
         const double sr = pend ? v0.s_r : 0.0, ur = pend ? v0.u_r : 0.0;
         const double y0r = v0.y0_r, y1r = v0.y1_r;
         v2d sj = {0.0, 0.0}, uj = {0.0, 0.0};
         if (pend) { sj = v0.s_c; uj = v0.u_c; }
+        double sor = 0.0, uor = 0.0;
+        v2d soj = {0.0, 0.0}, uoj = {0.0, 0.0};
+        if (D2 && pend2) { sor = v0.so_r; uor = v0.uo_r; soj = v0.so_c; uoj = v0.uo_c; }
         v2d a0 = v0.a0, a1 = v0.a1;
         if (!qn_s2_row_on(diag, lane, wave)) { a0 = (v2d){0.0, 0.0}; a1 = (v2d){0.0, 0.0}; }
         int ijn = -1;
@@ -1145,6 +1194,19 @@
         for (int r = 0; r < QN_S2_RPW; ++r) {
             v2d hn = h[r];
             h[r] = qn_sym_ld<NT>(hnext + (size_t)r * rstride);
+            if (D2) {
+                const double si = qn_lane_bcast(sor, r), ui = qn_lane_bcast(uor, r);
+                if (BFGS) {
+                    hn.x = hn.x + c2_su * (si * uoj.x + ui * soj.x);
+                    hn.y = hn.y + c2_su * (si * uoj.y + ui * soj.y);
+                }
+                hn.x = hn.x + c2_ss * (si * soj.x);
+                hn.y = hn.y + c2_ss * (si * soj.y);
+                if (!BFGS) {
+                    hn.x = hn.x + c2_uu * (ui * uoj.x);
+                    hn.y = hn.y + c2_uu * (ui * uoj.y);
+                }
+            }
             const double si = qn_lane_bcast(sr, r), ui = qn_lane_bcast(ur, r);
             if (BFGS || SR1) {
                 hn.x = hn.x + c_su * (si * uj.x + ui * sj.x);
@@ -1156,7 +1218,8 @@
                 hn.x = hn.x + c_uu * (ui * uj.x);
                 hn.y = hn.y + c_uu * (ui * uj.y);
             }
-            qn_sym_st<NT>(hbase + (size_t)r * np, hn);
+            if (D2) qn_s2_tile_st<NT>(rs, voff, (unsigned)r * npb, hn);
+            else qn_sym_st<NT>(hbase + (size_t)r * np, hn);
             const double y0 = qn_lane_bcast(y0r, r), y1 = qn_lane_bcast(y1r, r);
             double t0 = hn.x * a0.x;
             t0 = __builtin_fma(hn.y, a0.y, t0);
@@ -1175,7 +1238,7 @@
         if (!qn_s2_col_on(diag, lane, wave)) { c0x = 0.0; c0y = 0.0; c1x = 0.0; c1y = 0.0; }
         if (has_next) {
             const int irn = In * QN_TB + wave * QN_S2_RPW + (lane & 15), ccn = qn_s2_col(In == Jn, lane, wave);
-            qn_s2_hvec_load<!FOLD>(q, irn, Jn * QN_TB + ccn, v0);
+            qn_s2_hvec_load<!FOLD, D2>(q, irn, Jn * QN_TB + ccn, v0);
             if (FOLD) {
                 const int rr = wave * QN_S2_RPW + (lane & 15), bI = 2 * (it + 1), bJ = bI + 1;
                 v0.y0_r = fv[bI][0][rr]; v0.y1_r = fv[bI][1][rr];
@@ -1185,7 +1248,7 @@
             const QnS2Sliver sl = qn_s2_sliver(a, wave);
             unsigned r = sl.D * QN_TB + sl.row, c = sl.D * QN_TB + 2 * lane;
             asm volatile("" : "+v"(r), "+v"(c));
-            qn_s2_hvec_load<true>(q, r, c, v0);
+            qn_s2_hvec_load<true, D2>(q, r, c, v0);
         }
         if (it == 0) { qn_keepalive(racc[0]); QN_S2_STAMP(3); QN_S2_STAMP_T(12, 448); }
         if (it == 1) { qn_keepalive(racc[0]); QN_S2_STAMP(6); QN_S2_STAMP_T(13, 448); }
@@ -1211,6 +1274,7 @@
         if (it == 0) QN_S2_STAMP(5);
         if (!has_next) break;
         I = In; J = Jn; hbase = hnext;
+        if (D2) { rs = qn_s2_tile_rsrc(a.H, I * QN_TB, J * QN_TB, np, st_on); voff = (unsigned)(wave * QN_S2_RPW) * npb + (unsigned)qn_s2_col(I == J, lane, wave) * 8u; }
         __syncthreads();
     }
     if (slv) {
@@ -1218,6 +1282,21 @@
         const double si = pend ? v0.s_r : 0.0, ui = pend ? v0.u_r : 0.0;
         v2d sj = {0.0, 0.0}, uj = {0.0, 0.0};
         if (pend) { sj = v0.s_c; uj = v0.u_c; }
+        if (D2) {
+            const double so = pend2 ? v0.so_r : 0.0, uo = pend2 ? v0.uo_r : 0.0;
+            v2d soj = {0.0, 0.0}, uoj = {0.0, 0.0};
+            if (pend2) { soj = v0.so_c; uoj = v0.uo_c; }
+            if (BFGS) {
+                hn.x = hn.x + c2_su * (so * uoj.x + uo * soj.x);
+                hn.y = hn.y + c2_su * (so * uoj.y + uo * soj.y);
+            }
+            hn.x = hn.x + c2_ss * (so * soj.x);
+            hn.y = hn.y + c2_ss * (so * soj.y);
+            if (!BFGS) {
+                hn.x = hn.x + c2_uu * (uo * uoj.x);
+                hn.y = hn.y + c2_uu * (uo * uoj.y);
+            }
+        }
         if (BFGS || SR1) {
             hn.x = hn.x + c_su * (si * uj.x + ui * sj.x);
             hn.y = hn.y + c_su * (si * uj.y + ui * sj.y);
@@ -1228,7 +1307,12 @@
             hn.x = hn.x + c_uu * (ui * uj.x);
             hn.y = hn.y + c_uu * (ui * uj.y);
         }
-        qn_sym_st<NT>(sliver_ptr(), hn);
+        if (D2) {
+            const QnS2Sliver sl = qn_s2_sliver(a, wave);
+            unsigned so = (unsigned)sl.row * npb + (unsigned)lane * 16u;
+            asm volatile("" : "+v"(so));
+            qn_s2_tile_st<NT>(qn_s2_tile_rsrc(a.H, sl.D * QN_TB, sl.D * QN_TB, np, st_on), so, 0u, hn);
+        } else qn_sym_st<NT>(sliver_ptr(), hn);
         double t0 = hn.x * v0.a0.x;
         t0 = __builtin_fma(hn.y, v0.a0.y, t0);
         double t1 = hn.x * v0.a1.x;
@@ -1335,11 +1419,13 @@
     }
     QnS2Slots S0;
     QN_S2_STAMP(0);
-    double gp = 0.0, yv = 0.0, s0e = 0.0, s1e = 0.0;
+    double gp = 0.0, yv = 0.0, s0e = 0.0, s1e = 0.0, uoe = 0.0;
+    constexpr bool D2 = !SHARD && !SR1;
     auto entries = [&]() {
         if (half != 1 && tid < QN_TB) {
             gp = a.F.GT[R * QN_TB + tid]; yv = a.F.Y[R * QN_TB + tid];
             if (SR1) { s0e = a.F.S0[R * QN_TB + tid]; s1e = a.F.S0[(size_t)a.np + R * QN_TB + tid]; }
+            if (D2) uoe = a.F.UN[R * QN_TB + tid];
         }
     };
     if (SHARD) { if (wave == 0) qn_s2_prologue_w0<QN_S2_HREDUCE, true>(a, L, entries); else entries(); }
@@ -1350,10 +1436,15 @@
     qn_s2_ctl_out(a, L);
     if (!L.mine) return;
     const int nrhs = L.c.hp_nrhs;
+    const bool keep_h = D2 && a.sold && QN_CTL_PASS_KEEPS_H(L.c);
+    if (keep_h && half == 0 && tid < QN_TB) a.F.UP[R * QN_TB + tid] = uoe;
+    double spe = 0.0;
+    if (keep_h && half == 1 && tid < QN_TB) spe = a.F.S0[(size_t)L.c.sc * (size_t)a.np + R * QN_TB + tid];
     double tot0 = 0.0, tot1 = 0.0;
     if (!SHARD) {
         if (half == 1 && nrhs != 2) return;
         const double t = qn_s2_slot_sum(a.part, a.nb, R, half, S0, qbuf);
+        if (keep_h && half == 1 && tid < QN_TB) a.sold[R * QN_TB + tid] = spe;
         if (half == 0) tot0 = t; else tot1 = t;
     } else if (tid < QN_TB) {
         const size_t np = (size_t)a.np;
diff --git a/optimization-solvers_amd/solver.py b/optimization-solvers_amd/solver.py
--- a/optimization-solvers_amd/solver.py
+++ b/optimization-solvers_amd/solver.py
@@ -736,7 +736,11 @@
     def stats(self):
         st = A.Stats()
         _check(A.lib().qn_solver_get_stats(self.h, C.byref(st)))
-        return {k: getattr(st, k) for k, _ in A.Stats._fields_}
+        out = {k: getattr(st, k) for k, _ in A.Stats._fields_}
+        v = C.c_size_t()
+        _check(A.lib().qn_solver_h_store_passes(self.h, C.byref(v)))
+        out["h_store_passes"] = v.value
+        return out
 
     def set_profiling(self, on):
         _check(A.lib().qn_solver_set_profiling(self.h, 1 if on else 0))
diff --git a/rust/src/ffi.rs b/rust/src/ffi.rs
--- a/rust/src/ffi.rs
+++ b/rust/src/ffi.rs
@@ -253,6 +253,7 @@
     pub fn qn_solver_set_trace(s: *mut qn_solver, cap: usize, with_x: c_int) -> c_int;
     pub fn qn_solver_get_trace(s: *mut qn_solver, out_host: *mut qn_trace_rec, cap: usize, len: *mut usize, x_trace_host: *mut f64) -> c_int;
     pub fn qn_solver_get_stats(s: *mut qn_solver, out: *mut qn_stats) -> c_int;
+    pub fn qn_solver_h_store_passes(s: *mut qn_solver, out: *mut usize) -> c_int;
     pub fn qn_solver_set_profiling(s: *mut qn_solver, on: c_int) -> c_int;
     pub fn qn_solver_set_sync_mode(s: *mut qn_solver, sync: c_int) -> c_int;
     pub fn qn_solver_set_tiling(s: *mut qn_solver, rows_per_block: c_int, col_splits: c_int) -> c_int;
diff --git a/rust/src/lib.rs b/rust/src/lib.rs
--- a/rust/src/lib.rs
+++ b/rust/src/lib.rs
@@ -807,6 +807,11 @@
             pub fn gradient_next_iterate_too_close(&self) -> bool {
                 self.core.flag(qn_solver_gradient_next_iterate_too_close)
             }
+            pub fn h_store_passes(&self) -> usize {
+                let mut v = 0usize;
+                unsafe { qn_solver_h_store_passes(self.core.h, &mut v) };
+                v
+            }
             pub fn approx_inv_hessian(&self) -> DMatrix<Floating> {
                 self.core.approx_inv_hessian()
             }
```

Result: no change. 13820, median of 6 (+0.9%).
